# biirving/meant

Hardware: AMD Instinct MI355X
Metric: samples/sec fwd+bwd, MEANT lag=12 d=768 (higher is better)
Workload: dtype bf16; 1 GPU; full MEANT (tweet+image) fwd+CE+bwd, lag=12, d=768, 12 heads, seq=512, 224x224 p=16, E=1, vocab 64001 (BASELINE.json configs[2]/[3]); batch_per_gpu=128, global_batch=128, parallelism=dp1, micro_batches=1, train_mode_dropout=True, activation_checkpointing=False, norm_linear_fold=False, grad_allreduce=False

## Files before the change

### include/meant_hip.h

```cpp
#ifndef MEANT_HIP_H
#define MEANT_HIP_H

#include <stddef.h>
#include <stdint.h>

#ifdef __cplusplus
extern "C" {
#endif

enum meant_dtype { MEANT_F32 = 0, MEANT_BF16 = 1 };
enum meant_raw_dtype { MEANT_RAW_F32 = 0, MEANT_RAW_BF16 = 1, MEANT_RAW_F64 = 2, MEANT_RAW_U8 = 3 };

enum meant_status {
  MEANT_OK = 0,
  MEANT_ERR_ARG = -1,
  MEANT_ERR_UNSUPPORTED = -2,
  MEANT_ERR_LAUNCH = -3,
  MEANT_ERR_WORKSPACE = -4
};

enum meant_epilogue {
  MEANT_EPI_NONE = 0,
  MEANT_EPI_GELU = 1,
  MEANT_EPI_RESIDUAL = 2,
  MEANT_EPI_SIGMOID = 4
};

int meant_version(void);
const char* meant_last_error(void);
int meant_num_cus(void);

int meant_set_option(const char* name, int value);
int meant_get_option(const char* name, int* value);
int64_t meant_route_count(const char* route);
void meant_route_reset(void);
int64_t meant_debug_nt_steals(void);

int meant_rmsnorm_fwd(const void* x, const float* scale, void* y, float* rinv, int64_t rows, int64_t d,
                      float eps, float drop_p, uint64_t seed, int dtype, void* stream);
size_t meant_rmsnorm_bwd_ws(int64_t rows, int64_t d);
int meant_rmsnorm_bwd(const void* dy, const void* x, const float* scale, const float* rinv, void* dx,
                      float* dscale, int64_t rows, int64_t d, float eps, float drop_p, uint64_t seed,
                      const void* dres, const void* gelu_pre, int dtype, void* workspace, size_t workspace_bytes,
                      void* stream);

int meant_rmsnorm_partial_fwd(const void* x, const float* scale, const float* offset, void* y, float* rinv, int64_t rows,
                              int64_t d, int64_t d_part, float eps, int dtype, void* stream);
int meant_rmsnorm_partial_bwd(const void* dy, const void* x, const float* scale, const float* rinv, void* dx, float* dscale,
                              float* doffset, int64_t rows, int64_t d, int64_t d_part, float eps, int dtype, void* workspace,
                              size_t workspace_bytes, void* stream);

int meant_rmsnorm_pooled_ok(int64_t rows, int64_t d, int64_t group_rows);
int meant_rmsnorm_fwd_pooled(const void* x, const float* scale, void* y, float* rinv, float* pooled, int64_t rows,
                             int64_t d, int64_t group_rows, int pool_input, int gelu_input, float eps, float drop_p,
                             uint64_t seed, int dtype, void* stream);
int meant_rmsnorm_bwd_pooled(const void* dy, int dy_pooled, const void* x, const float* scale, const float* rinv,
                             void* dx, float* dscale, int64_t rows, int64_t d, int64_t group_rows, float eps,
                             float drop_p, uint64_t seed, const void* dres, int dres_pooled, const void* gelu_pre,
                             int dtype, void* workspace, size_t workspace_bytes, void* stream);

int meant_rmsnorm_stats(const void* x, float* rinv, int64_t rows, int64_t d, float eps, int dtype, void* stream);
int meant_rmsnorm_bwd_chain(const void* dy, int dy_pooled, const void* x, const float* scale, const float* rinv,
                            void* dx_scaled, float* dscale, int64_t rows, int64_t d, int64_t group_rows, float eps,
                            float drop_p, uint64_t seed, const void* gelu_pre, const float* up_rinv, const float* up_bias,
                            float up_eps, int64_t up_d, float* kcoef, float* dbias_up, int dtype, void* workspace, size_t workspace_bytes,
                            void* stream);
int meant_colscale(const float* w, const float* g, float* out, int64_t N, int64_t K, void* stream);
int meant_colscale_bwd(const float* dwp, const float* w, const float* g, float* dw, float* dg, int64_t N, int64_t K,
                       void* stream);

int meant_layernorm_fwd(const void* x, const float* gamma, const float* beta, void* y, float* stats,
                        int64_t rows, int64_t d, float eps, int dtype, void* stream);
int meant_layernorm_bwd(const void* dy, const void* x, const float* gamma, const float* stats, void* dx,
                        float* dgamma, float* dbeta, int64_t rows, int64_t d, int dtype, void* workspace,
                        size_t workspace_bytes, void* stream);

int meant_linear_fwd(const void* x, int64_t ldx, const void* w, const float* bias, const void* residual,
                     int64_t ldr, void* y, int64_t ldy, void* preact, int64_t M, int64_t N, int64_t K,
                     int epilogue, int dtype, void* stream);
int meant_qkv_proj_fwd(const void* x, int64_t ldx, const void* w, const float* bias, void* qkv, int64_t M,
                       int64_t K, int64_t S, int H, int Dh, int R, const float* qa, const float* qb,
                       const float* ka, const float* kb, int dtype, void* stream);
int meant_linear_fwd_rowscale(const void* x, int64_t ldx, const void* w, const float* bias, const float* row_scale,
                              const void* residual, int64_t ldr, void* y, int64_t ldy, void* preact, int64_t M, int64_t N,
                              int64_t K, int epilogue, int dtype, void* stream);
int meant_linear_bwd_dx_norm(const void* dy_scaled, int64_t lddy, const void* wT, const void* x, int64_t ldx,
                             const float* coef, const void* dres, int64_t lddres, const float* dres_pooled,
                             int64_t group_rows, void* dx, int64_t lddx, int64_t M, int64_t N, int64_t K, int dtype,
                             void* stream);
int meant_linear_bwd_dx(const void* dy, int64_t lddy, const void* wT, void* dx, int64_t lddx, int64_t M,
                        int64_t N, int64_t K, int dtype, void* stream);
size_t meant_linear_bwd_dw_ws(int64_t M, int64_t N, int64_t K, int dtype);
int meant_linear_bwd_dw(const void* dy, int64_t lddy, const void* x, int64_t ldx, float* dw, float* dbias,
                        int64_t M, int64_t N, int64_t K, int dtype, void* workspace, size_t workspace_bytes,
                        void* stream);

int meant_gemm_f32_strided(const float* A, const float* B, float* C, int64_t M, int64_t N, int64_t K,
                           int64_t nb1, int64_t nb2, const int64_t* sA ,
                           const int64_t* sB , const int64_t* sC , float alpha,
                           int accumulate, void* stream);

int meant_rotary_qk(void* qkv, int64_t T, int64_t S, int H, int Dh, int R, const float* qa, const float* qb,
                    const float* ka, const float* kb, int transpose, int dtype, void* stream);

size_t meant_attn_ws(int64_t G, int64_t S, int H, int Dh, int dtype);
size_t meant_attn_fwd_ws(int64_t G, int64_t S, int H, int Dh, int dtype);
int meant_attn_fwd(const void* qkv, void* o, float* lse, const float* key_mask, int64_t G, int64_t S, int H,
                   int Dh, float scale, int causal, int dtype, void* workspace, size_t workspace_bytes,
                   void* stream);
size_t meant_attn_drop_ws(int64_t G, int64_t S, int H, int Dh, int dtype);
int meant_attn_drop_fwd(const void* qkv, void* o, float* lse, const float* key_mask, int64_t G, int64_t S, int H, int Dh,
                        float scale, int causal, float drop_p, uint64_t seed, int dtype, void* workspace,
                        size_t workspace_bytes, void* stream);
int meant_attn_drop_bwd(const void* qkv, const void* o, const void* do_, const float* lse, const float* key_mask, void* dqkv,
                        int64_t G, int64_t S, int H, int Dh, float scale, int causal, float drop_p, uint64_t seed,
                        int dtype, void* workspace, size_t workspace_bytes, void* stream);
int meant_attn_bwd(const void* qkv, const void* o, const void* do_, const float* lse, const float* key_mask,
                   void* dqkv, int64_t G, int64_t S, int H, int Dh, float scale, int causal, const float* qa,
                   const float* qb, const float* ka, const float* kb, int R, int dtype, void* workspace,
                   size_t workspace_bytes, void* stream);

int meant_gather_rows(const void* src, const int32_t* idx, const void* fill, void* dst, int64_t n, int64_t W, int dtype,
                      void* stream);
int meant_gather_rows_rot(const void* src, const int32_t* idx, void* dst, int64_t n, int64_t S, int H, int Dh, int R,
                          const float* qa, const float* qb, const float* ka, const float* kb, int dtype, void* stream);
int meant_group_scatter(const void* ddst, const int32_t* index, void* dsrc, int64_t B, int64_t L, int64_t G, int64_t S,
                        int64_t W, int dtype, void* stream);
int meant_attn_cls_fwd(const void* qkv, void* out, int64_t ld_out, float* stats, const float* key_mask, int64_t B, int64_t L,
                       int H, int Dh, float scale, int dtype, void* stream);
int meant_attn_cls_bwd(const void* qkv, const void* out, int64_t ld_out, const void* dout, int64_t ld_dout,
                       const float* stats, const float* key_mask, void* dqkv, int64_t B, int64_t L, int H, int Dh,
                       float scale, int dtype, void* stream);

int meant_token_shift(const void* x, void* y, int64_t B, int64_t frames, int64_t n, int64_t d, int transpose, int dtype,
                      void* stream);
int meant_dropout(const void* x, void* y, int64_t n, float p, uint64_t seed, int dtype, void* stream);

int meant_temporal_attn_fwd(const void* q, const void* kv, void* o, float* p, int64_t B, int L, int H, int Dh,
                            float scale, int dtype, void* stream);
int meant_temporal_attn_bwd(const void* q, const void* kv, const float* p, const void* do_, void* dq, void* dkv,
                            int64_t B, int L, int H, int Dh, float scale, int dtype, void* stream);

int meant_patchify(const void* images, int images_dtype, void* patches, int64_t G, int C, int Hh, int Ww, int p,
                   int dtype, void* stream);

int meant_patchify_raw(const void* images, int raw_dtype, float mean, float inv_std, void* patches, int64_t G, int C,
                       int Hh, int Ww, int p, int dtype, void* stream);

int meant_meanpool_fwd(const void* x, void* out, int64_t ld_out, int64_t col_off, int64_t G, int64_t S, int64_t d,
                       int dtype, int out_dtype, void* stream);
int meant_meanpool_bwd(const void* dout, int64_t ld_out, int64_t col_off, void* dx, int64_t G, int64_t S, int64_t d,
                       int dtype, int out_dtype, void* stream);

int meant_add_rowvec(const void* x, const float* v, void* y, int64_t rows, int64_t d, int64_t period, int dtype,
                     void* stream);
int meant_add_rowvec_bwd(const void* dy, float* dv, int64_t rows, int64_t d, int64_t period, int dtype, void* stream);
int meant_gelu_bwd(const void* dy, const void* pre, void* dx, int64_t n, int dtype, void* stream);
int meant_sigmoid_bwd(const void* dy, const void* y, void* dx, int64_t n, int dtype, void* stream);
int meant_geglu_fwd(const void* h, void* y, int64_t rows, int64_t w, int dtype, void* stream);
int meant_geglu_bwd(const void* h, const void* dy, void* dh, int64_t rows, int64_t w, int dtype, void* stream);
int meant_add(const void* a, const void* b, void* y, int64_t n, int dtype, void* stream);
int meant_cast(const void* src, int dtype_src, void* dst, int dtype_dst, int64_t n, void* stream);
int meant_transpose2d(const void* src, int dtype_src, void* dst, int dtype_dst, int64_t rows, int64_t cols,
                      void* stream);
int meant_pad_copy2d(const void* src, int64_t ld_src, int64_t cols_src, int dtype_src, void* dst, int64_t ld_dst,
                     int64_t cols_dst, int dtype_dst, int64_t rows, void* stream);
int meant_embedding_fwd(const float* table, const int64_t* ids, void* out, int64_t n, int64_t d, int64_t V, int dtype,
                        void* stream);
int meant_embedding_bwd(const void* dout, const int64_t* ids, float* dtable, int64_t n, int64_t d, int64_t V, int dtype,
                        void* stream);
int meant_embedding_bwd_sorted(const void* dout, const int64_t* sorted_ids, const int64_t* order, float* dtable,
                               int64_t n, int64_t d, int64_t V, int dtype, void* stream);
int meant_embedding_bwd_sorted_range(const void* dout, const int64_t* sorted_ids, const int64_t* order, float* dtable,
                                     int64_t n, int64_t d, int64_t V, int64_t id_lo, int64_t id_hi, int dtype, void* stream);
size_t meant_sort_ids_ws(int64_t n, int64_t V);
int meant_sort_ids(const int64_t* ids, int64_t n, int64_t V, int64_t* sorted_ids, int64_t* order, void* workspace,
                   size_t workspace_bytes, void* stream);
size_t meant_embedding_bwd_seg_ws(int64_t n, int64_t d);
int meant_embedding_bwd_seg(const void* dout, const int64_t* sorted_ids, const int64_t* order, float* dtable, int64_t n,
                            int64_t d, int64_t V, int64_t id_lo, int64_t id_hi, int dtype, void* workspace,
                            size_t workspace_bytes, void* stream);

int meant_ce_probs(const float* probs, const int64_t* target, float* loss_accum, float* dprobs, int64_t B, int C,
                   void* stream);
int meant_softmax_ce_fwd(const void* logits, int64_t ld, const int64_t* target, int64_t T, int64_t V, int64_t ignore_index,
                         float* row_loss, float* lse, int dtype, void* stream);
int meant_softmax_ce_bwd(const void* logits, int64_t ld, const int64_t* target, const float* lse, int64_t T, int64_t V,
                         int64_t ignore_index, const float* gscale, void* dlogits, int dtype, void* stream);
size_t meant_select_rows_ws(int64_t T);
int meant_select_rows(const int64_t* target, int64_t T, int64_t V, int64_t ignore_index, int32_t* idx, int32_t* inv,
                      int64_t* target_sel, int32_t* count, void* workspace, size_t workspace_bytes, void* stream);
int meant_sumsq_f32(const float* x, int64_t n, float* out_accum, void* stream);
int meant_adamw_f32(float* p, const float* g, float* m, float* v, int64_t n, float lr, float beta1, float beta2,
                    float eps, float weight_decay, int64_t step, const float* sumsq, float max_norm,
                    float grad_scale, void* stream);

#ifdef __cplusplus
}
#endif
#endif
```

### meant_amd/_lib.py

```python
from __future__ import annotations

import ctypes as C
import os

import torch

_HERE = os.path.dirname(os.path.abspath(__file__))
LIB_PATH = os.environ.get("MEANT_LIB_PATH") or os.path.join(_HERE, "libmeant_hip.so")

F32, BF16 = 0, 1
RAW_F32, RAW_BF16, RAW_F64, RAW_U8 = 0, 1, 2, 3
EPI_NONE, EPI_GELU, EPI_RESIDUAL, EPI_SIGMOID = 0, 1, 2, 4

_p, _i, _i64, _f, _u64, _sz = C.c_void_p, C.c_int, C.c_int64, C.c_float, C.c_uint64, C.c_size_t

SIGNATURES = {
    "meant_version": (_i, []),
    "meant_last_error": (C.c_char_p, []),
    "meant_num_cus": (_i, []),
    "meant_rmsnorm_fwd": (_i, [_p, _p, _p, _p, _i64, _i64, _f, _f, _u64, _i, _p]),
    "meant_rmsnorm_bwd_ws": (_sz, [_i64, _i64]),
    "meant_rmsnorm_bwd": (_i, [_p, _p, _p, _p, _p, _p, _i64, _i64, _f, _f, _u64, _p, _p, _i, _p, _sz, _p]),
    "meant_rmsnorm_pooled_ok": (_i, [_i64, _i64, _i64]),
    "meant_rmsnorm_fwd_pooled": (_i, [_p, _p, _p, _p, _p, _i64, _i64, _i64, _i, _i, _f, _f, _u64, _i, _p]),
    "meant_rmsnorm_bwd_pooled": (_i, [_p, _i, _p, _p, _p, _p, _p, _i64, _i64, _i64, _f, _f, _u64, _p, _i, _p, _i, _p, _sz, _p]),
    "meant_layernorm_fwd": (_i, [_p, _p, _p, _p, _p, _i64, _i64, _f, _i, _p]),
    "meant_layernorm_bwd": (_i, [_p, _p, _p, _p, _p, _p, _p, _i64, _i64, _i, _p, _sz, _p]),
    "meant_linear_fwd": (_i, [_p, _i64, _p, _p, _p, _i64, _p, _i64, _p, _i64, _i64, _i64, _i, _i, _p]),
    "meant_linear_bwd_dx": (_i, [_p, _i64, _p, _p, _i64, _i64, _i64, _i64, _i, _p]),
    "meant_linear_bwd_dw_ws": (_sz, [_i64, _i64, _i64, _i]),
    "meant_linear_bwd_dw": (_i, [_p, _i64, _p, _i64, _p, _p, _i64, _i64, _i64, _i, _p, _sz, _p]),
    "meant_set_option": (_i, [C.c_char_p, _i]),
    "meant_get_option": (_i, [C.c_char_p, C.POINTER(_i)]),
    "meant_route_count": (_i64, [C.c_char_p]),
    "meant_route_reset": (None, []),
    "meant_debug_nt_steals": (_i64, []),
    "meant_gemm_f32_strided": (_i, [_p, _p, _p, _i64, _i64, _i64, _i64, _i64, _p, _p, _p, _f, _i, _p]),
    "meant_rotary_qk": (_i, [_p, _i64, _i64, _i, _i, _i, _p, _p, _p, _p, _i, _i, _p]),
    "meant_attn_ws": (_sz, [_i64, _i64, _i, _i, _i]),
    "meant_attn_fwd_ws": (_sz, [_i64, _i64, _i, _i, _i]),
    "meant_attn_drop_ws": (_sz, [_i64, _i64, _i, _i, _i]),
    "meant_attn_drop_fwd": (_i, [_p, _p, _p, _p, _i64, _i64, _i, _i, _f, _i, _f, _u64, _i, _p, _sz, _p]),
    "meant_attn_drop_bwd": (_i, [_p, _p, _p, _p, _p, _p, _i64, _i64, _i, _i, _f, _i, _f, _u64, _i, _p, _sz, _p]),
    "meant_attn_fwd": (_i, [_p, _p, _p, _p, _i64, _i64, _i, _i, _f, _i, _i, _p, _sz, _p]),
    "meant_attn_bwd": (_i, [_p, _p, _p, _p, _p, _p, _i64, _i64, _i, _i, _f, _i, _p, _p, _p, _p, _i, _i, _p, _sz, _p]),
    "meant_qkv_proj_fwd": (_i, [_p, _i64, _p, _p, _p, _i64, _i64, _i64, _i, _i, _i, _p, _p, _p, _p, _i, _p]),
    "meant_gather_rows": (_i, [_p, _p, _p, _p, _i64, _i64, _i, _p]),
    "meant_gather_rows_rot": (_i, [_p, _p, _p, _i64, _i64, _i, _i, _i, _p, _p, _p, _p, _i, _p]),
    "meant_group_scatter": (_i, [_p, _p, _p, _i64, _i64, _i64, _i64, _i64, _i, _p]),
    "meant_attn_cls_fwd": (_i, [_p, _p, _i64, _p, _p, _i64, _i64, _i, _i, _f, _i, _p]),
    "meant_attn_cls_bwd": (_i, [_p, _p, _i64, _p, _i64, _p, _p, _p, _i64, _i64, _i, _i, _f, _i, _p]),
    "meant_token_shift": (_i, [_p, _p, _i64, _i64, _i64, _i64, _i, _i, _p]),
    "meant_dropout": (_i, [_p, _p, _i64, _f, _u64, _i, _p]),
    "meant_temporal_attn_fwd": (_i, [_p, _p, _p, _p, _i64, _i, _i, _i, _f, _i, _p]),
    "meant_temporal_attn_bwd": (_i, [_p, _p, _p, _p, _p, _p, _i64, _i, _i, _i, _f, _i, _p]),
    "meant_patchify": (_i, [_p, _i, _p, _i64, _i, _i, _i, _i, _i, _p]),
    "meant_patchify_raw": (_i, [_p, _i, _f, _f, _p, _i64, _i, _i, _i, _i, _i, _p]),
    "meant_meanpool_fwd": (_i, [_p, _p, _i64, _i64, _i64, _i64, _i64, _i, _i, _p]),
    "meant_meanpool_bwd": (_i, [_p, _i64, _i64, _p, _i64, _i64, _i64, _i, _i, _p]),
    "meant_add_rowvec": (_i, [_p, _p, _p, _i64, _i64, _i64, _i, _p]),
    "meant_add_rowvec_bwd": (_i, [_p, _p, _i64, _i64, _i64, _i, _p]),
    "meant_gelu_bwd": (_i, [_p, _p, _p, _i64, _i, _p]),
    "meant_sigmoid_bwd": (_i, [_p, _p, _p, _i64, _i, _p]),
    "meant_geglu_fwd": (_i, [_p, _p, _i64, _i64, _i, _p]),
    "meant_geglu_bwd": (_i, [_p, _p, _p, _i64, _i64, _i, _p]),
    "meant_add": (_i, [_p, _p, _p, _i64, _i, _p]),
    "meant_cast": (_i, [_p, _i, _p, _i, _i64, _p]),
    "meant_transpose2d": (_i, [_p, _i, _p, _i, _i64, _i64, _p]),
    "meant_pad_copy2d": (_i, [_p, _i64, _i64, _i, _p, _i64, _i64, _i, _i64, _p]),
    "meant_embedding_fwd": (_i, [_p, _p, _p, _i64, _i64, _i64, _i, _p]),
    "meant_embedding_bwd": (_i, [_p, _p, _p, _i64, _i64, _i64, _i, _p]),
    "meant_ce_probs": (_i, [_p, _p, _p, _p, _i64, _i, _p]),
    "meant_softmax_ce_fwd": (_i, [_p, _i64, _p, _i64, _i64, _i64, _p, _p, _i, _p]),
    "meant_softmax_ce_bwd": (_i, [_p, _i64, _p, _p, _i64, _i64, _i64, _p, _p, _i, _p]),
    "meant_select_rows_ws": (_sz, [_i64]),
    "meant_select_rows": (_i, [_p, _i64, _i64, _i64, _p, _p, _p, _p, _p, _sz, _p]),
    "meant_sumsq_f32": (_i, [_p, _i64, _p, _p]),
    "meant_adamw_f32": (_i, [_p, _p, _p, _p, _i64, _f, _f, _f, _f, _f, _i64, _p, _f, _f, _p]),
    "meant_embedding_bwd_sorted": (_i, [_p, _p, _p, _p, _i64, _i64, _i64, _i, _p]),
    "meant_embedding_bwd_sorted_range": (_i, [_p, _p, _p, _p, _i64, _i64, _i64, _i64, _i64, _i, _p]),
    "meant_sort_ids_ws": (_sz, [_i64, _i64]),
    "meant_sort_ids": (_i, [_p, _i64, _i64, _p, _p, _p, _sz, _p]),
    "meant_embedding_bwd_seg_ws": (_sz, [_i64, _i64]),
    "meant_embedding_bwd_seg": (_i, [_p, _p, _p, _p, _i64, _i64, _i64, _i64, _i64, _i, _p, _sz, _p]),
    "meant_rmsnorm_partial_fwd": (_i, [_p, _p, _p, _p, _p, _i64, _i64, _i64, _f, _i, _p]),
    "meant_rmsnorm_partial_bwd": (_i, [_p, _p, _p, _p, _p, _p, _p, _i64, _i64, _i64, _f, _i, _p, _sz, _p]),
    "meant_rmsnorm_stats": (_i, [_p, _p, _i64, _i64, _f, _i, _p]),
    "meant_rmsnorm_bwd_chain": (_i, [_p, _i, _p, _p, _p, _p, _p, _i64, _i64, _i64, _f, _f, _u64, _p, _p, _p, _f, _i64, _p, _p, _i, _p, _sz, _p]),
    "meant_colscale": (_i, [_p, _p, _p, _i64, _i64, _p]),
    "meant_colscale_bwd": (_i, [_p, _p, _p, _p, _p, _i64, _i64, _p]),
    "meant_linear_fwd_rowscale": (_i, [_p, _i64, _p, _p, _p, _p, _i64, _p, _i64, _p, _i64, _i64, _i64, _i, _i, _p]),
    "meant_linear_bwd_dx_norm": (_i, [_p, _i64, _p, _p, _i64, _p, _p, _i64, _p, _i64, _p, _i64, _i64, _i64, _i64, _i, _p]),
}


class MeantLibraryMissing(ImportError):
    pass


def _load():
    if not os.path.exists(LIB_PATH):
        raise MeantLibraryMissing(
            f"{LIB_PATH} not found: build it with `python -c 'import __graft_entry__ as g; g.build()'` "
            f"(or `make -C meant_amd/csrc`).  meant_amd has no CPU / eager fallback.")
    lib = C.CDLL(LIB_PATH)
    for name, (res, args) in SIGNATURES.items():
        fn = getattr(lib, name)
        fn.restype = res
        fn.argtypes = args
    return lib


lib = _load()


def set_option(name: str, value: int) -> None:
    check(lib.meant_set_option(name.encode(), int(value)), "set_option")


def get_option(name: str) -> int:
    v = _i(0)
    check(lib.meant_get_option(name.encode(), C.byref(v)), "get_option")
    return v.value


def route_count(route: str) -> int:
    n = lib.meant_route_count(route.encode())
    if n < 0:
        raise KeyError(route)
    return n


def route_reset() -> None:
    lib.meant_route_reset()


class MeantHipError(RuntimeError):
    pass


def check(rc: int, what: str = "") -> None:
    if rc != 0:
        msg = lib.meant_last_error().decode("utf-8", "replace")
        raise MeantHipError(f"{what or 'libmeant_hip'} failed (status {rc}): {msg}")
```

### meant_amd/csrc/common.h

```cpp
#pragma once
#include <hip/hip_runtime.h>
#include <stdint.h>
#include <stdio.h>
#include <math.h>
#include "../../include/meant_hip.h"

typedef __bf16 bf16;
typedef __attribute__((ext_vector_type(2))) float f32x2;
typedef __attribute__((ext_vector_type(4))) float f32x4;
typedef __attribute__((ext_vector_type(16))) float f32x16;
typedef __attribute__((ext_vector_type(4))) __bf16 bf16x4;
typedef __attribute__((ext_vector_type(8))) __bf16 bf16x8;
typedef __attribute__((ext_vector_type(4))) unsigned int u32x4;
typedef __attribute__((ext_vector_type(2))) unsigned int u32x2;

#define WAVE 64

void meant_set_error(const char* fmt, ...);

#define MEANT_REQUIRE(cond, code, ...)      \
  do {                                      \
    if (!(cond)) {                          \
      meant_set_error(__VA_ARGS__);         \
      return (code);                        \
    }                                       \
  } while (0)

#define MEANT_LAUNCH_CHECK(name)                                                     \
  do {                                                                               \
    hipError_t e__ = hipGetLastError();                                              \
    if (e__ != hipSuccess) {                                                         \
      meant_set_error("%s: launch failed: %s", name, hipGetErrorString(e__));        \
      return MEANT_ERR_LAUNCH;                                                       \
    }                                                                                \
  } while (0)

#define MEANT_MAX_DEVICES 64
int meant_current_device(void);
int meant_raise_dyn_lds(const void* kernel, int bytes);
#define MEANT_RAISE_LDS(kernel, bytes)                                        \
  do {                                                                        \
    int rc__ = meant_raise_dyn_lds((const void*)(kernel), (int)(bytes));      \
    if (rc__) return rc__;                                                    \
  } while (0)

enum meant_option_id {
  MEANT_OPT_NT_STREAM = 0, MEANT_OPT_NT_DYNAMIC, MEANT_OPT_DETERMINISTIC, MEANT_OPT_NT_GRID_CAP, MEANT_OPT_ATTN_SHORT, MEANT_OPT_NT_RAGGED, MEANT_OPT_ATTN_BWD1, MEANT_OPT_TEMPORAL_LONG, MEANT_OPT_COUNT
};
int meant_opt(int id);

enum meant_route_id {
  ROUTE_NT128 = 0, ROUTE_NT256, ROUTE_NT256S, ROUTE_NT256S_ROT, ROUTE_NT_SPLIT, ROUTE_TN128, ROUTE_TN256, ROUTE_TN256_DET, ROUTE_TN_TAIL,
  ROUTE_GEMM_F32, ROUTE_ATTN_FWD, ROUTE_ATTN_FWD_D128, ROUTE_ATTN_FWD_D96, ROUTE_ATTN_BWD,
  ROUTE_ATTN_BWD_D128, ROUTE_ATTN_BWD_D96, ROUTE_ATTN_GENERIC, ROUTE_ATTN_CLS, ROUTE_ATTN_SHORT, ROUTE_NT_OVERLAP, ROUTE_ATTN_BWD1,
  ROUTE_ATTN_FWD_D160, ROUTE_ATTN_FWD_D192, ROUTE_ATTN_FWD_D256, ROUTE_ATTN_BWD_D160, ROUTE_ATTN_BWD_D192, ROUTE_ATTN_BWD_D256, ROUTE_TEMPORAL_LONG,
  ROUTE_EMB_SEG, ROUTE_SORT_IDS, ROUTE_NT128K, ROUTE_NT256K, ROUTE_SELECT_ROWS, ROUTE_ROTARY_QK, ROUTE_ROTARY_PAIRS, ROUTE_NT_ROT,
  MEANT_ROUTE_COUNT
};
void meant_route_hit(int route);

static inline bool meant_aligned16(const void* p) { return (reinterpret_cast<uintptr_t>(p) & 15) == 0; }
static inline int64_t ceil_div(int64_t a, int64_t b) { return (a + b - 1) / b; }

template <typename T> struct Vec8;
template <> struct Vec8<float> {
  f32x4 lo, hi;
  __device__ __forceinline__ float get(int i) const { return i < 4 ? lo[i] : hi[i - 4]; }
  __device__ __forceinline__ void set(int i, float v) { if (i < 4) lo[i] = v; else hi[i - 4] = v; }
};
template <> struct Vec8<bf16> {
  bf16x8 v;
  __device__ __forceinline__ float get(int i) const { return (float)v[i]; }
  __device__ __forceinline__ void set(int i, float x) { v[i] = (bf16)x; }
  __device__ __forceinline__ unsigned raw(int i) const {
    typedef __attribute__((ext_vector_type(4))) unsigned uvec4;
    return (__builtin_bit_cast(uvec4, v)[i >> 1] >> ((i & 1) * 16)) & 0xffffu;
  }
};

__device__ __forceinline__ void rotary_pair(float t0, float t1, float a0, float a1, float b0, float b1, float& o0, float& o1) {
  o0 = __builtin_fmaf(t0, a0, -(t1 * b0));
  o1 = __builtin_fmaf(t1, a1, t0 * b1);
}

template <typename T> __device__ __forceinline__ Vec8<T> load8(const T* p);
template <> __device__ __forceinline__ Vec8<float> load8<float>(const float* p) {
  Vec8<float> r; r.lo = *reinterpret_cast<const f32x4*>(p); r.hi = *reinterpret_cast<const f32x4*>(p + 4); return r;
}
template <> __device__ __forceinline__ Vec8<bf16> load8<bf16>(const bf16* p) {
  Vec8<bf16> r; r.v = *reinterpret_cast<const bf16x8*>(p); return r;
}
template <typename T> __device__ __forceinline__ Vec8<T> load8s(const T* p);
template <> __device__ __forceinline__ Vec8<float> load8s<float>(const float* p) {
  Vec8<float> r;
  r.lo = __builtin_nontemporal_load(reinterpret_cast<const f32x4*>(p));
  r.hi = __builtin_nontemporal_load(reinterpret_cast<const f32x4*>(p + 4));
  return r;
}
template <> __device__ __forceinline__ Vec8<bf16> load8s<bf16>(const bf16* p) {
  Vec8<bf16> r; r.v = __builtin_nontemporal_load(reinterpret_cast<const bf16x8*>(p)); return r;
}
template <typename T> __device__ __forceinline__ void store8s(T* p, const Vec8<T>& v);
template <> __device__ __forceinline__ void store8s<float>(float* p, const Vec8<float>& v) {
  __builtin_nontemporal_store(v.lo, reinterpret_cast<f32x4*>(p)); __builtin_nontemporal_store(v.hi, reinterpret_cast<f32x4*>(p + 4));
}
template <> __device__ __forceinline__ void store8s<bf16>(bf16* p, const Vec8<bf16>& v) {
  __builtin_nontemporal_store(v.v, reinterpret_cast<bf16x8*>(p));
}
template <typename T> __device__ __forceinline__ void store8(T* p, const Vec8<T>& v);
template <> __device__ __forceinline__ void store8<float>(float* p, const Vec8<float>& v) {
  *reinterpret_cast<f32x4*>(p) = v.lo; *reinterpret_cast<f32x4*>(p + 4) = v.hi;
}
template <> __device__ __forceinline__ void store8<bf16>(bf16* p, const Vec8<bf16>& v) {
  *reinterpret_cast<bf16x8*>(p) = v.v;
}

__device__ __forceinline__ float to_f(float x) { return x; }
__device__ __forceinline__ float to_f(bf16 x) { return (float)x; }
template <typename T> __device__ __forceinline__ T from_f(float x);
template <> __device__ __forceinline__ float from_f<float>(float x) { return x; }
template <> __device__ __forceinline__ bf16 from_f<bf16>(float x) { return (bf16)x; }

__device__ __forceinline__ float wave_sum(float v) {
#pragma unroll
  for (int o = 32; o > 0; o >>= 1) v += __shfl_xor(v, o, 64);
  return v;
}
__device__ __forceinline__ float wave_max(float v) {
#pragma unroll
  for (int o = 32; o > 0; o >>= 1) v = fmaxf(v, __shfl_xor(v, o, 64));
  return v;
}

#define MEANT_DPP_ADD(v, CTRL) ((v) + __builtin_bit_cast(float, __builtin_amdgcn_update_dpp(0, __builtin_bit_cast(int, (v)), (CTRL), 0xf, 0xf, true)))
__device__ __forceinline__ float wave_sum_dpp(float v) {
  v = MEANT_DPP_ADD(v, 0xB1);
  v = MEANT_DPP_ADD(v, 0x4E);
  v = MEANT_DPP_ADD(v, 0x141);
  v = MEANT_DPP_ADD(v, 0x140);
  const int b = __builtin_bit_cast(int, v);
  const float r0 = __builtin_bit_cast(float, __builtin_amdgcn_readlane(b, 0)), r1 = __builtin_bit_cast(float, __builtin_amdgcn_readlane(b, 16));
  const float r2 = __builtin_bit_cast(float, __builtin_amdgcn_readlane(b, 32)), r3 = __builtin_bit_cast(float, __builtin_amdgcn_readlane(b, 48));
  return (r0 + r1) + (r2 + r3);
}
__device__ __forceinline__ float rms_rinv(float sumsq, float inv_sqrt_d, float eps) {
  return 1.0f / (sqrtf(sumsq) * inv_sqrt_d + eps);
}

__device__ __forceinline__ float gelu_erf(float x) { return 0.5f * x * (1.0f + erff(x * 0.70710678118654752f)); }
__device__ __forceinline__ float gelu_erf_fast(float x) {
  const float z = fabsf(x) * 0.70710678118654752f;
  const float t = __builtin_amdgcn_rcpf(fmaf(0.3275911f, z, 1.0f));
  float p = fmaf(1.061405429f, t, -1.453152027f);
  p = fmaf(p, t, 1.421413741f);
  p = fmaf(p, t, -0.284496736f);
  p = fmaf(p, t, 0.254829592f);
  const float half_erfc = 0.5f * p * t * __builtin_amdgcn_exp2f(-1.4426950408889634f * z * z);
  const float phi = x < 0.f ? half_erfc : 1.0f - half_erfc;
  return x * phi;
}
__device__ __forceinline__ float gelu_phi_fast(float x) {
  const float z = fabsf(x) * 0.70710678118654752f;
  const float t = __builtin_amdgcn_rcpf(fmaf(0.3275911f, z, 1.0f));
  float p = fmaf(1.061405429f, t, -1.453152027f);
  p = fmaf(p, t, 1.421413741f);
  p = fmaf(p, t, -0.284496736f);
  p = fmaf(p, t, 0.254829592f);
  const float half_erfc = 0.5f * p * t * __builtin_amdgcn_exp2f(-1.4426950408889634f * z * z);
  return x < 0.f ? half_erfc : 1.0f - half_erfc;
}
constexpr unsigned PHI_LO = 0x3A80u, PHI_HI = 0x40FFu, PHI_N = PHI_HI - PHI_LO + 1;
__device__ __forceinline__ unsigned phi_slot(unsigned bits) {
  unsigned m = bits & 0x7FFFu;
  m = m < PHI_LO ? PHI_LO : m;
  m = m > PHI_HI ? PHI_HI : m;
  return (m - PHI_LO) + ((bits >> 15) & 1u) * PHI_N;
}
__device__ __forceinline__ float gelu_erf_grad(float x) {
  const float cdf = 0.5f * (1.0f + erff(x * 0.70710678118654752f));
  const float pdf = 0.39894228040143268f * __expf(-0.5f * x * x);
  return cdf + x * pdf;
}

__device__ __forceinline__ float gelu_erf_grad_fast(float x) {
  const float z = fabsf(x) * 0.70710678118654752f;
  const float t = __builtin_amdgcn_rcpf(fmaf(0.3275911f, z, 1.0f));
  float p = fmaf(1.061405429f, t, -1.453152027f);
  p = fmaf(p, t, 1.421413741f);
  p = fmaf(p, t, -0.284496736f);
  p = fmaf(p, t, 0.254829592f);
  const float e = __builtin_amdgcn_exp2f(-0.72134752044448170f * x * x);
  const float half_erfc = 0.5f * p * t * e;
  const float phi = x < 0.f ? half_erfc : 1.0f - half_erfc;
  return fmaf(x * 0.39894228040143268f, e, phi);
}

__device__ __forceinline__ float hash_uniform(uint64_t seed, uint64_t idx) {
  uint64_t z = seed + idx * 0x9E3779B97F4A7C15ull;
  z = (z ^ (z >> 30)) * 0xBF58476D1CE4E5B9ull;
  z = (z ^ (z >> 27)) * 0x94D049BB133111EBull;
  z = z ^ (z >> 31);
  return (float)(z >> 40) * (1.0f / 16777216.0f);
}
#ifndef DROP_HASH32
#define DROP_HASH32 1
#endif
__device__ __forceinline__ uint32_t mix32(uint32_t h) {
  h ^= h >> 16; h *= 0x85EBCA6Bu; h ^= h >> 13; h *= 0xC2B2AE35u; h ^= h >> 16;
  return h;
}
__device__ __forceinline__ uint32_t draw32(uint64_t seed, uint64_t blk, uint32_t j) {
  const uint32_t hi = (uint32_t)(blk >> 32);
  const uint32_t k = (uint32_t)blk ^ ((hi << 17) | (hi >> 15));
  const uint32_t s = ((uint32_t)seed + 0x9E3779B9u * (j + 1)) ^ ((uint32_t)(seed >> 32) * 0x7FEB352Du);
  return mix32(k ^ s);
}
__device__ __forceinline__ void keep_scale8(float p, uint64_t seed, uint64_t base, float (&m)[8]) {
  const unsigned thr = (unsigned)(p * 65536.0f);
  const float sc = 65536.0f / (float)(65536u - thr);
  if ((thr & 0xffu) == 0) {
    const unsigned thr8 = thr >> 8;
#if DROP_HASH32
#pragma unroll
    for (int h = 0; h < 2; ++h) {
      const uint32_t z = draw32(seed, base >> 3, (uint32_t)h);
#pragma unroll
      for (int q = 0; q < 4; ++q) m[4 * h + q] = ((z >> (8 * q)) & 0xffu) >= thr8 ? sc : 0.0f;
    }
#else
    uint64_t z = seed + ((base >> 3) | (1ull << 62)) * 0x9E3779B97F4A7C15ull;
    z = (z ^ (z >> 30)) * 0xBF58476D1CE4E5B9ull;
    z = (z ^ (z >> 27)) * 0x94D049BB133111EBull;
    z = z ^ (z >> 31);
#pragma unroll
    for (int q = 0; q < 8; ++q) m[q] = ((unsigned)(z >> (8 * q)) & 0xffu) >= thr8 ? sc : 0.0f;
#endif
    return;
  }
#if DROP_HASH32
#pragma unroll
  for (int h = 0; h < 4; ++h) {
    const uint32_t z = draw32(seed, base >> 3, 2u + (uint32_t)h);
#pragma unroll
    for (int q = 0; q < 2; ++q) m[2 * h + q] = ((z >> (16 * q)) & 0xffffu) >= thr ? sc : 0.0f;
  }
#else
#pragma unroll
  for (int h = 0; h < 2; ++h) {
    uint64_t z = seed + ((base >> 2) + h) * 0x9E3779B97F4A7C15ull;
    z = (z ^ (z >> 30)) * 0xBF58476D1CE4E5B9ull;
    z = (z ^ (z >> 27)) * 0x94D049BB133111EBull;
    z = z ^ (z >> 31);
#pragma unroll
    for (int q = 0; q < 4; ++q) m[4 * h + q] = ((unsigned)(z >> (16 * q)) & 0xffffu) >= thr ? sc : 0.0f;
  }
#endif
}

__device__ __forceinline__ unsigned lds_addr(const void* p) {
  return (unsigned)(unsigned long long)(const __attribute__((address_space(3))) char*)p;
}
template <int OFF>
__device__ __forceinline__ u32x2 lds_read_tr16(unsigned addr) {
  u32x2 r;
  asm volatile("ds_read_b64_tr_b16 %0, %1 offset:%2" : "=v"(r) : "v"(addr), "n"(OFF));
  return r;
}
__device__ __forceinline__ void lds_wait_all() {
  asm volatile("s_waitcnt lgkmcnt(0)" ::: "memory");
  __builtin_amdgcn_sched_barrier(0);
}
template <int N>
__device__ __forceinline__ void lds_wait_upto() {
  asm volatile("s_waitcnt lgkmcnt(%0)" ::"n"(N) : "memory");
  __builtin_amdgcn_sched_barrier(0);
}
__device__ __forceinline__ bf16x8 pack_tr(u32x2 lo, u32x2 hi) {
  u32x4 v = {lo[0], lo[1], hi[0], hi[1]};
  return __builtin_bit_cast(bf16x8, v);
}

#define DISPATCH_DTYPE(dtype, T, ...)                                           \
  do {                                                                          \
    if ((dtype) == MEANT_F32) { using T = float; __VA_ARGS__; }                 \
    else if ((dtype) == MEANT_BF16) { using T = bf16; __VA_ARGS__; }            \
    else { meant_set_error("unknown dtype %d", (int)(dtype)); return MEANT_ERR_ARG; } \
  } while (0)
```

### meant_amd/csrc/core.hip

```cpp
#include "common.h"
#include <stdarg.h>
#include <string.h>
#include <stdlib.h>
#include <atomic>
#include <mutex>
#include <unordered_map>

static thread_local char g_err[512] = "";

void meant_set_error(const char* fmt, ...) {
  va_list ap;
  va_start(ap, fmt);
  vsnprintf(g_err, sizeof(g_err), fmt, ap);
  va_end(ap);
}

extern "C" const char* meant_last_error(void) { return g_err; }

extern "C" int meant_version(void) { return 200;  }

namespace {
struct DeviceState {
  int cus = -1;
  std::unordered_map<const void*, int> lds_raised;
};
std::mutex g_dev_mu;
DeviceState g_dev[MEANT_MAX_DEVICES];
}

int meant_current_device(void) {
  int dev = 0;
  if (hipGetDevice(&dev) != hipSuccess || dev < 0 || dev >= MEANT_MAX_DEVICES) return -1;
  return dev;
}

extern "C" int meant_num_cus(void) {
  const int dev = meant_current_device();
  if (dev < 0) return 0;
  std::lock_guard<std::mutex> lock(g_dev_mu);
  DeviceState& st = g_dev[dev];
  if (st.cus < 0) {
    hipDeviceProp_t p;
    st.cus = hipGetDeviceProperties(&p, dev) == hipSuccess ? p.multiProcessorCount : 0;
  }
  return st.cus;
}

int meant_raise_dyn_lds(const void* kernel, int bytes) {
  const int dev = meant_current_device();
  MEANT_REQUIRE(dev >= 0, MEANT_ERR_LAUNCH, "no current HIP device (or device index >= %d)", MEANT_MAX_DEVICES);
  std::lock_guard<std::mutex> lock(g_dev_mu);
  DeviceState& st = g_dev[dev];
  const auto it = st.lds_raised.find(kernel);
  if (it != st.lds_raised.end() && it->second >= bytes) return MEANT_OK;
  const hipError_t e = hipFuncSetAttribute(kernel, hipFuncAttributeMaxDynamicSharedMemorySize, bytes);
  MEANT_REQUIRE(e == hipSuccess, MEANT_ERR_LAUNCH, "hipFuncSetAttribute(%d bytes of LDS) failed on device %d: %s", bytes, dev,
                hipGetErrorString(e));
  st.lds_raised[kernel] = bytes;
  return MEANT_OK;
}

namespace {
struct OptionDef { const char* name; const char* env; int dflt; };
const OptionDef k_options[MEANT_OPT_COUNT] = {
    {"nt_stream", "MEANT_NT_STREAM", 1},
    {"nt_dynamic", "MEANT_NT_DYNAMIC", 1},
    {"deterministic", "MEANT_DETERMINISTIC", 0},
    {"nt_grid_cap", "MEANT_NT_GRID_CAP", 0},
    {"attn_short", "MEANT_ATTN_SHORT", 1},
    {"nt_ragged", "MEANT_NT_RAGGED", 1},
    {"attn_bwd1", "MEANT_ATTN_BWD1", 1},
    {"temporal_long", "MEANT_TEMPORAL_LONG", 0},
};
bool is_nt_pp(const char* name) { return name && !strcmp(name, "nt_pp"); }
std::atomic<int> g_opt[MEANT_OPT_COUNT];
std::once_flag g_opt_once;
void options_init() {
  std::call_once(g_opt_once, [] {
    for (int i = 0; i < MEANT_OPT_COUNT; ++i) {
      const char* v = getenv(k_options[i].env);
      g_opt[i].store(v && *v ? atoi(v) : k_options[i].dflt, std::memory_order_relaxed);
    }
  });
}
int option_index(const char* name) {
  if (!name) return -1;
  for (int i = 0; i < MEANT_OPT_COUNT; ++i)
    if (!strcmp(name, k_options[i].name)) return i;
  return -1;
}
}

int meant_opt(int id) {
  options_init();
  return g_opt[id].load(std::memory_order_relaxed);
}

extern "C" int meant_set_option(const char* name, int value) {
  options_init();
  if (is_nt_pp(name)) {
    MEANT_REQUIRE(value == 1, MEANT_ERR_UNSUPPORTED, "meant_set_option: nt_pp is always 1 (the lock-step kernel was removed)");
    return MEANT_OK;
  }
  const int i = option_index(name);
  MEANT_REQUIRE(i >= 0, MEANT_ERR_ARG, "meant_set_option: unknown option '%s'", name ? name : "(null)");
  g_opt[i].store(value, std::memory_order_relaxed);
  return MEANT_OK;
}

extern "C" int meant_get_option(const char* name, int* value) {
  options_init();
  if (is_nt_pp(name) && value) { *value = 1; return MEANT_OK; }
  const int i = option_index(name);
  MEANT_REQUIRE(i >= 0 && value, MEANT_ERR_ARG, "meant_get_option: unknown option '%s'", name ? name : "(null)");
  *value = g_opt[i].load(std::memory_order_relaxed);
  return MEANT_OK;
}

namespace {
const char* const k_routes[MEANT_ROUTE_COUNT] = {
    "nt128", "nt256", "nt256s", "nt256s_rot", "nt_split", "tn128", "tn256", "tn256_det", "tn_tail", "gemm_f32",
    "attn_fwd", "attn_fwd_d128", "attn_fwd_d96", "attn_bwd", "attn_bwd_d128", "attn_bwd_d96",
    "attn_generic", "attn_cls", "attn_short", "nt_overlap", "attn_bwd1",
    "attn_fwd_d160", "attn_fwd_d192", "attn_fwd_d256", "attn_bwd_d160", "attn_bwd_d192", "attn_bwd_d256",
    "temporal_long", "emb_seg", "sort_ids", "nt128k", "nt256k", "select_rows",
    "rotary_qk", "rotary_pairs",
    "nt_rot",
};
std::atomic<long long> g_route[MEANT_ROUTE_COUNT];
}

void meant_route_hit(int route) { g_route[route].fetch_add(1, std::memory_order_relaxed); }

extern "C" int64_t meant_route_count(const char* route) {
  if (!route) return -1;
  for (int i = 0; i < MEANT_ROUTE_COUNT; ++i)
    if (!strcmp(route, k_routes[i])) return (int64_t)g_route[i].load(std::memory_order_relaxed);
  return -1;
}

extern "C" void meant_route_reset(void) {
  for (int i = 0; i < MEANT_ROUTE_COUNT; ++i) g_route[i].store(0, std::memory_order_relaxed);
}
```

### meant_amd/csrc/embedding.hip

```cpp
#include "common.h"

#define EMB_REQ(c, ...) MEANT_REQUIRE(c, MEANT_ERR_ARG, __VA_ARGS__)

namespace {

constexpr int SORT_TILE = 2048, SORT_WAVE_SPAN = 512, SORT_ROUNDS = 8;

__device__ __forceinline__ uint32_t sort_key(int64_t id, int64_t V) {
  return (uint32_t)(id < 0 ? 0 : (id >= V ? V - 1 : id));
}

__global__ __launch_bounds__(256) void sort_hist_kernel(const int64_t* __restrict__ ids, int64_t n, int64_t V, int passes,
                                                         uint32_t* __restrict__ ghist, uint32_t* __restrict__ tile_hist, int64_t ntiles) {
  __shared__ uint32_t h[4][256];
  const int tid = threadIdx.x;
#pragma unroll
  for (int p = 0; p < 4; ++p) h[p][tid] = 0;
  __syncthreads();
  const int64_t base = (int64_t)blockIdx.x * SORT_TILE;
  for (int i = 0; i < SORT_TILE / 256; ++i) {
    const int64_t j = base + i * 256 + tid;
    if (j < n) {
      const uint32_t key = sort_key(ids[j], V);
      for (int p = 0; p < passes; ++p) atomicAdd(&h[p][(key >> (8 * p)) & 255u], 1u);
    }
  }
  __syncthreads();
  tile_hist[(int64_t)tid * ntiles + blockIdx.x] = h[0][tid];
  for (int p = 0; p < passes; ++p)
    if (h[p][tid]) atomicAdd(&ghist[p * 256 + tid], h[p][tid]);
}

__global__ __launch_bounds__(256) void sort_count_kernel(const uint32_t* __restrict__ keys, int64_t n, int shift,
                                                          uint32_t* __restrict__ tile_hist, int64_t ntiles) {
  __shared__ uint32_t h[256];
  const int tid = threadIdx.x;
  h[tid] = 0;
  __syncthreads();
  const int64_t base = (int64_t)blockIdx.x * SORT_TILE;
  for (int i = 0; i < SORT_TILE / 256; ++i) {
    const int64_t j = base + i * 256 + tid;
    if (j < n) atomicAdd(&h[(keys[j] >> shift) & 255u], 1u);
  }
  __syncthreads();
  tile_hist[(int64_t)tid * ntiles + blockIdx.x] = h[tid];
}

__device__ __forceinline__ uint32_t block_scan_incl(uint32_t x, uint32_t* wsum, uint32_t* total) {
  const int lane = threadIdx.x & 63, wave = threadIdx.x >> 6;
#pragma unroll
  for (int o = 1; o < 64; o <<= 1) {
    const uint32_t y = __shfl_up(x, o, 64);
    if (lane >= o) x += y;
  }
  __syncthreads();
  if (lane == 63) wsum[wave] = x;
  __syncthreads();
  uint32_t pre = 0, tot = 0;
#pragma unroll
  for (int w = 0; w < 4; ++w) {
    const uint32_t s = wsum[w];
    if (w < wave) pre += s;
    tot += s;
  }
  *total = tot;
  return x + pre;
}

__global__ __launch_bounds__(256) void sort_scan_kernel(const uint32_t* __restrict__ ghist, uint32_t* __restrict__ tile_hist, int64_t ntiles) {
  __shared__ uint32_t wsum[4];
  const int tid = threadIdx.x, digit = blockIdx.x;
  uint32_t carry;
  block_scan_incl(tid < digit ? ghist[tid] : 0u, wsum, &carry);
  uint32_t* row = tile_hist + (int64_t)digit * ntiles;
  for (int64_t t0 = 0; t0 < ntiles; t0 += 256) {
    const int64_t t = t0 + tid;
    const uint32_t x = t < ntiles ? row[t] : 0u;
    uint32_t total;
    const uint32_t incl = block_scan_incl(x, wsum, &total);
    if (t < ntiles) row[t] = carry + incl - x;
    carry += total;
  }
}

template <bool FIRST, bool LAST>
__global__ __launch_bounds__(256) void sort_scatter_kernel(const int64_t* __restrict__ ids, const uint32_t* __restrict__ kin,
                                                            const uint32_t* __restrict__ vin, int64_t n, int64_t V, int shift,
                                                            const uint32_t* __restrict__ tile_off, int64_t ntiles,
                                                            uint32_t* __restrict__ kout, uint32_t* __restrict__ vout,
                                                            int64_t* __restrict__ sorted_ids, int64_t* __restrict__ order) {
  __shared__ uint32_t cnt[4][256];
  const int tid = threadIdx.x, lane = tid & 63, wave = tid >> 6;
#pragma unroll
  for (int w = 0; w < 4; ++w) cnt[w][tid] = 0;
  __syncthreads();
  const int64_t base = (int64_t)blockIdx.x * SORT_TILE + wave * SORT_WAVE_SPAN;
  uint32_t key[SORT_ROUNDS], val[SORT_ROUNDS], rk[SORT_ROUNDS];
#pragma unroll
  for (int r = 0; r < SORT_ROUNDS; ++r) {
    const int64_t j = base + r * 64 + lane;
    const bool valid = j < n;
    key[r] = valid ? (FIRST ? sort_key(ids[j], V) : kin[j]) : 0u;
    val[r] = valid ? (FIRST ? (uint32_t)j : vin[j]) : 0u;
    const uint32_t dig = (key[r] >> shift) & 255u;
    unsigned long long m = __ballot(valid);
#pragma unroll
    for (int b = 0; b < 8; ++b) {
      const bool bit = (dig >> b) & 1u;
      const unsigned long long bal = __ballot(valid && bit);
      m &= bit ? bal : ~bal;
    }
    const unsigned long long below = m & ((1ull << lane) - 1ull);
    rk[r] = valid ? cnt[wave][dig] + (uint32_t)__popcll(below) : 0u;
    __syncthreads();
    if (valid && below == 0) cnt[wave][dig] += (uint32_t)__popcll(m);
    __syncthreads();
  }
  {
    uint32_t o = tile_off[(int64_t)tid * ntiles + blockIdx.x];
#pragma unroll
    for (int w = 0; w < 4; ++w) {
      const uint32_t c = cnt[w][tid];
      cnt[w][tid] = o;
      o += c;
    }
  }
  __syncthreads();
#pragma unroll
  for (int r = 0; r < SORT_ROUNDS; ++r) {
    const int64_t j = base + r * 64 + lane;
    if (j >= n) continue;
    const int64_t pos = (int64_t)cnt[wave][(key[r] >> shift) & 255u] + rk[r];
    if (pos >= n) continue;
    if (LAST) {
      sorted_ids[pos] = (int64_t)key[r];
      order[pos] = (int64_t)val[r];
    } else {
      kout[pos] = key[r];
      vout[pos] = val[r];
    }
  }
}

int sort_passes(int64_t V) {
  int bits = 0;
  for (uint64_t m = (uint64_t)(V - 1); m; m >>= 1) ++bits;
  const int p = (bits + 7) / 8;
  return p < 1 ? 1 : p;
}
size_t align256(size_t x) { return (x + 255) & ~(size_t)255; }
struct SortWs { size_t ghist, tile_hist, buf[2], total; int nbuf; };
SortWs sort_ws_layout(int64_t n, int64_t V) {
  SortWs w;
  const int64_t ntiles = ceil_div(n, SORT_TILE);
  const int passes = sort_passes(V);
  w.nbuf = passes - 1 < 2 ? passes - 1 : 2;
  size_t off = 0;
  w.ghist = off; off += align256(4 * 256 * sizeof(uint32_t));
  w.tile_hist = off; off += align256((size_t)ntiles * 256 * sizeof(uint32_t));
  for (int i = 0; i < 2; ++i) {
    w.buf[i] = off;
    if (i < w.nbuf) off += 2 * align256((size_t)n * sizeof(uint32_t));
  }
  w.total = off;
  return w;
}

constexpr int SEG = 256;
template <typename T>
__global__ __launch_bounds__(256) void emb_seg_kernel(const T* __restrict__ dout, const int64_t* __restrict__ sorted_ids,
                                                       const int64_t* __restrict__ order, float* __restrict__ dtable,
                                                       float* __restrict__ part, int64_t n, int64_t d, int64_t V, int64_t id_lo,
                                                       int64_t id_hi, int cb_chunks) {
  const int lane = threadIdx.x & 63, wave = threadIdx.x >> 6;
  const int64_t s = (int64_t)blockIdx.x * 4 + wave;
  const int64_t j0 = s * SEG;
  if (j0 >= n) return;
  const int64_t j1 = j0 + SEG < n ? j0 + SEG : n;
  if (sorted_ids[j1 - 1] < id_lo || sorted_ids[j0] >= id_hi) return;
  const int c0 = blockIdx.y * cb_chunks;
  const int left = (int)(d >> 3) - c0;
  const int nch = left < cb_chunks ? left : cb_chunks;
  const bool has0 = lane < nch, has1 = lane + 64 < nch;
  const int64_t col0 = (int64_t)(c0 + lane) * 8, col1 = (int64_t)(c0 + lane + 64) * 8;
  float acc0[8], acc1[8];
#pragma unroll
  for (int e = 0; e < 8; ++e) acc0[e] = acc1[e] = 0.f;
  int64_t cur = sorted_ids[j0];
  bool open_left = j0 > 0 && sorted_ids[j0 - 1] == cur;

  auto flush = [&](int64_t id, int slot) {
    if (id < 0 || id >= V || id < id_lo || id >= id_hi) return;
    if (slot >= 0) {
      float* row = part + (s * 2 + slot) * d;
      Vec8<float> v;
      if (has0) {
#pragma unroll
        for (int e = 0; e < 8; ++e) v.set(e, acc0[e]);
        store8<float>(row + col0, v);
      }
      if (has1) {
#pragma unroll
        for (int e = 0; e < 8; ++e) v.set(e, acc1[e]);
        store8<float>(row + col1, v);
      }
      return;
    }
    float* row = dtable + id * d;
    if (has0) {
      Vec8<float> v = load8<float>(row + col0);
#pragma unroll
      for (int e = 0; e < 8; ++e) v.set(e, v.get(e) + acc0[e]);
      store8<float>(row + col0, v);
    }
    if (has1) {
      Vec8<float> v = load8<float>(row + col1);
#pragma unroll
      for (int e = 0; e < 8; ++e) v.set(e, v.get(e) + acc1[e]);
      store8<float>(row + col1, v);
    }
  };

  for (int64_t jb = j0; jb < j1; jb += 64) {
    const int64_t jl = jb + lane < j1 ? jb + lane : j1 - 1;
    const long long my_id = sorted_ids[jl], my_ord = order[jl];
    const int cnt = (int)(j1 - jb < 64 ? j1 - jb : 64);
    for (int t0 = 0; t0 < cnt; t0 += 4) {
      Vec8<T> r0[4], r1[4];
      long long ids4[4];
#pragma unroll
      for (int u = 0; u < 4; ++u) {
        const int t = t0 + u < cnt ? t0 + u : cnt - 1;
        ids4[u] = __shfl(my_id, t, 64);
        const long long ord = __shfl(my_ord, t, 64);
        const bool row_ok = ord >= 0 && ord < n;
        const T* src = dout + (row_ok ? ord : 0) * d;
        r0[u] = Vec8<T>{};
        r1[u] = Vec8<T>{};
        if (has0 && row_ok) r0[u] = load8s<T>(src + col0);
        if (has1 && row_ok) r1[u] = load8s<T>(src + col1);
      }
#pragma unroll
      for (int u = 0; u < 4; ++u) {
        if (t0 + u >= cnt) break;
        const int64_t id = ids4[u];
        if (id != cur) {
          flush(cur, open_left ? 0 : -1);
#pragma unroll
          for (int e = 0; e < 8; ++e) acc0[e] = acc1[e] = 0.f;
          cur = id;
          open_left = false;
        }
#pragma unroll
        for (int e = 0; e < 8; ++e) {
          if (has0) acc0[e] += r0[u].get(e);
          if (has1) acc1[e] += r1[u].get(e);
        }
      }
    }
  }
  const bool open_right = j1 < n && sorted_ids[j1] == cur;
  flush(cur, open_left ? 0 : (open_right ? 1 : -1));
}

constexpr int SEG_SHORT = 16;
__global__ __launch_bounds__(256) void emb_seg_cross_kernel(const int64_t* __restrict__ sorted_ids, const float* __restrict__ part,
                                                             int* __restrict__ longk, float* __restrict__ dtable, int64_t n, int64_t d,
                                                             int64_t V, int64_t id_lo, int64_t id_hi) {
  const int lane = threadIdx.x & 63, wave = threadIdx.x >> 6;
  const int64_t s = (int64_t)blockIdx.x * 4 + wave, j0 = s * SEG, j1 = j0 + SEG;
  if (j1 >= n) return;
  const int64_t id = sorted_ids[j1 - 1];
  const bool owner = sorted_ids[j1] == id && !(j0 > 0 && sorted_ids[j0 - 1] == id)
                     && id >= 0 && id < V && id >= id_lo && id < id_hi;
  int64_t K = 0;
  if (owner) {
    const int64_t nst = (n + SEG - 1) / SEG;
    int64_t follow = 0;
    for (int64_t t0 = s + 1;; t0 += 64) {
      const int64_t t = t0 + lane;
      const int k = __popcll(__ballot(t < nst && sorted_ids[t * SEG] == id));
      follow += k;
      if (k < 64) break;
    }
    K = follow + 1;
  }
  if (blockIdx.y == 0 && lane == 0) longk[s] = K > SEG_SHORT ? (int)K : 0;
  if (K == 0 || K > SEG_SHORT) return;
  const int64_t col = (int64_t)blockIdx.y * 256 + lane * 4;
  if (col >= d) return;
  f32x4 acc = *reinterpret_cast<const f32x4*>(part + (s * 2 + 1) * d + col);
  for (int64_t k = 1; k < K; ++k) acc += *reinterpret_cast<const f32x4*>(part + (s + k) * 2 * d + col);
  f32x4* dst = reinterpret_cast<f32x4*>(dtable + id * d + col);
  *dst = *dst + acc;
}

__global__ __launch_bounds__(256) void emb_seg_long_kernel(const int64_t* __restrict__ sorted_ids, const float* __restrict__ part,
                                                            const int* __restrict__ longk, float* __restrict__ dtable, int64_t d) {
  __shared__ f32x4 red[16][16];
  const int tid = threadIdx.x;
  const int64_t s = blockIdx.x;
  const int64_t K = longk[s];
  if (K == 0) return;
  const int64_t id = sorted_ids[s * SEG + SEG - 1];
  const int p = tid >> 4;
  const int64_t col = (int64_t)blockIdx.y * 64 + (tid & 15) * 4;
  const bool active = col < d;
  const int64_t piece = (K + 15) / 16, k0 = p * piece, k1 = k0 + piece < K ? k0 + piece : K;
  f32x4 acc = {0.f, 0.f, 0.f, 0.f};
  if (active) {
#pragma unroll 4
    for (int64_t k = k0; k < k1; ++k) {
      const float* row = k == 0 ? part + (s * 2 + 1) * d : part + (s + k) * 2 * d;
      acc += *reinterpret_cast<const f32x4*>(row + col);
    }
  }
  red[p][tid & 15] = acc;
  __syncthreads();
#pragma unroll
  for (int h = 8; h > 0; h >>= 1) {
    if (p < h) red[p][tid & 15] += red[p + h][tid & 15];
    __syncthreads();
  }
  if (p == 0 && active) {
    f32x4* dst = reinterpret_cast<f32x4*>(dtable + id * d + col);
    *dst = *dst + red[0][tid & 15];
  }
}

size_t seg_part_bytes(int64_t n, int64_t d) { return (size_t)ceil_div(n, SEG) * 2 * (size_t)d * sizeof(float); }

template <typename T>
__global__ __launch_bounds__(256) void embedding_fwd_kernel(const float* __restrict__ table, const int64_t* __restrict__ ids,
                                                             T* __restrict__ out, int64_t n, int d, int64_t V) {
  const int lane = threadIdx.x & 63, wave = threadIdx.x >> 6;
  const int nch = d >> 3;
  for (int64_t r = (int64_t)blockIdx.x * 4 + wave; r < n; r += (int64_t)gridDim.x * 4) {
    int64_t id = ids[r];
    id = id < 0 ? 0 : (id >= V ? V - 1 : id);
    const float* src = table + id * d;
    for (int ch = lane; ch < nch; ch += 64) {
      const Vec8<float> v = load8<float>(src + ch * 8);
      Vec8<T> o;
#pragma unroll
      for (int k = 0; k < 8; ++k) o.set(k, v.get(k));
      store8s<T>(out + r * d + ch * 8, o);
    }
  }
}
template <typename T>
__global__ __launch_bounds__(256) void embedding_bwd_kernel(const T* __restrict__ dout, const int64_t* __restrict__ ids,
                                                             float* __restrict__ dtable, int64_t n, int d, int64_t V) {
  const int lane = threadIdx.x & 63, wave = threadIdx.x >> 6;
  for (int64_t r = (int64_t)blockIdx.x * 4 + wave; r < n; r += (int64_t)gridDim.x * 4) {
    int64_t id = ids[r];
    id = id < 0 ? 0 : (id >= V ? V - 1 : id);
    float* dst = dtable + id * d;
    for (int e = lane; e < d; e += 64) atomicAdd(dst + e, to_f(dout[r * d + e]));
  }
}

constexpr int EMB_SEG = 256;
template <typename T>
__global__ __launch_bounds__(256) void embedding_bwd_sorted_kernel(const T* __restrict__ dout, const int64_t* __restrict__ sorted_ids,
                                                                    const int64_t* __restrict__ order, float* __restrict__ dtable,
                                                                    int64_t n, int d, int64_t V, int det, int64_t id_lo, int64_t id_hi) {
  const int lane = threadIdx.x & 63, wave = threadIdx.x >> 6;
  int64_t j0 = ((int64_t)blockIdx.x * 4 + wave) * EMB_SEG;
  if (j0 >= n) return;
  int64_t j1 = j0 + EMB_SEG < n ? j0 + EMB_SEG : n;
  if (sorted_ids[j1 - 1] < id_lo || sorted_ids[j0] >= id_hi) return;
  if (det) {
    if (j0 > 0) {
      const int64_t prev = sorted_ids[j0 - 1];
      while (j0 < j1 && sorted_ids[j0] == prev) ++j0;
      if (j0 == j1) return;
    }
    const int64_t last = sorted_ids[j1 - 1];
    while (j1 < n && sorted_ids[j1] == last) ++j1;
  }
  const int nch = d >> 3;
  const bool has1 = lane + 64 < nch, has0 = lane < nch;
  float acc0[8], acc1[8];
#pragma unroll
  for (int e = 0; e < 8; ++e) acc0[e] = acc1[e] = 0.f;
  int64_t cur = sorted_ids[j0];
  bool shared = !det && j0 > 0 && sorted_ids[j0 - 1] == cur;

  auto flush = [&](int64_t id, bool atomic) {
    if (id < 0 || id >= V || id < id_lo || id >= id_hi) return;
    float* row = dtable + id * d;
    if (atomic) {
#pragma unroll
      for (int e = 0; e < 8; ++e) {
        if (has0) atomicAdd(row + lane * 8 + e, acc0[e]);
        if (has1) atomicAdd(row + (lane + 64) * 8 + e, acc1[e]);
      }
    } else {
      if (has0) {
        Vec8<float> v = load8<float>(row + lane * 8);
#pragma unroll
        for (int e = 0; e < 8; ++e) v.set(e, v.get(e) + acc0[e]);
        store8<float>(row + lane * 8, v);
      }
      if (has1) {
        Vec8<float> v = load8<float>(row + (lane + 64) * 8);
#pragma unroll
        for (int e = 0; e < 8; ++e) v.set(e, v.get(e) + acc1[e]);
        store8<float>(row + (lane + 64) * 8, v);
      }
    }
  };

  for (int64_t jb = j0; jb < j1; jb += 64) {
    const int64_t jl = jb + lane < j1 ? jb + lane : j1 - 1;
    const long long my_id = sorted_ids[jl], my_ord = order[jl];
    const int cnt = (int)(j1 - jb < 64 ? j1 - jb : 64);
    for (int t0 = 0; t0 < cnt; t0 += 4) {
      Vec8<T> r0[4], r1[4];
      long long ids4[4];
#pragma unroll
      for (int u = 0; u < 4; ++u) {
        const int t = t0 + u < cnt ? t0 + u : cnt - 1;
        ids4[u] = __shfl(my_id, t, 64);
        const long long ord = __shfl(my_ord, t, 64);
        const T* src = dout + ord * d;
        if (has0) r0[u] = load8s<T>(src + lane * 8);
        if (has1) r1[u] = load8s<T>(src + (lane + 64) * 8);
      }
#pragma unroll
      for (int u = 0; u < 4; ++u) {
        if (t0 + u >= cnt) break;
        const int64_t id = ids4[u];
        if (id != cur) {
          flush(cur, shared);
#pragma unroll
          for (int e = 0; e < 8; ++e) acc0[e] = acc1[e] = 0.f;
          cur = id;
          shared = false;
        }
#pragma unroll
        for (int e = 0; e < 8; ++e) {
          if (has0) acc0[e] += r0[u].get(e);
          if (has1) acc1[e] += r1[u].get(e);
        }
      }
    }
  }
  flush(cur, !det && (shared || (j1 < n && sorted_ids[j1] == cur)));
}

}

extern "C" size_t meant_sort_ids_ws(int64_t n, int64_t V) {
  if (n <= 0 || V <= 0 || n >= (1ll << 31) || V >= (1ll << 31)) return 0;
  return sort_ws_layout(n, V).total;
}

extern "C" int meant_sort_ids(const int64_t* ids, int64_t n, int64_t V, int64_t* sorted_ids, int64_t* order, void* workspace,
                              size_t workspace_bytes, void* stream) {
  EMB_REQ(ids && sorted_ids && order && n > 0 && V > 0, "sort_ids: bad argument");
  MEANT_REQUIRE(n < (1ll << 31) && V < (1ll << 31), MEANT_ERR_UNSUPPORTED, "sort_ids: n=%lld and V=%lld must be below 2^31", (long long)n,
                (long long)V);
  {
    const char *a = (const char*)ids, *o1 = (const char*)sorted_ids, *o2 = (const char*)order;
    const size_t len = (size_t)n * sizeof(int64_t);
    const auto overlap = [len](const char* x, const char* y) { return x < y + len && y < x + len; };
    EMB_REQ(!overlap(a, o1) && !overlap(a, o2) && !overlap(o1, o2), "sort_ids: ids, sorted_ids and order must not overlap");
  }
  const SortWs w = sort_ws_layout(n, V);
  MEANT_REQUIRE(workspace && workspace_bytes >= w.total, MEANT_ERR_WORKSPACE, "sort_ids: workspace of %zu bytes needed, %zu given", w.total, workspace_bytes);
  EMB_REQ((reinterpret_cast<uintptr_t>(workspace) & 3) == 0, "sort_ids: 4-byte workspace alignment");
  hipStream_t st = (hipStream_t)stream;
  char* base = (char*)workspace;
  uint32_t* ghist = (uint32_t*)(base + w.ghist);
  uint32_t* tile_hist = (uint32_t*)(base + w.tile_hist);
  uint32_t* bk[2] = {nullptr, nullptr};
  uint32_t* bv[2] = {nullptr, nullptr};
  for (int i = 0; i < w.nbuf; ++i) {
    bk[i] = (uint32_t*)(base + w.buf[i]);
    bv[i] = (uint32_t*)(base + w.buf[i] + align256((size_t)n * sizeof(uint32_t)));
  }
  const int64_t ntiles = ceil_div(n, SORT_TILE);
  const int passes = sort_passes(V);
  const dim3 grid((unsigned)ntiles), block(256);
  const hipError_t e = hipMemsetAsync(ghist, 0, 4 * 256 * sizeof(uint32_t), st);
  MEANT_REQUIRE(e == hipSuccess, MEANT_ERR_LAUNCH, "sort_ids: clearing the digit counters failed: %s", hipGetErrorString(e));
  hipLaunchKernelGGL(sort_hist_kernel, grid, block, 0, st, ids, n, V, passes, ghist, tile_hist, ntiles);
  for (int p = 0; p < passes; ++p) {
    const bool first = p == 0, last = p == passes - 1;
    const uint32_t* kin = first ? nullptr : bk[(p - 1) & 1];
    const uint32_t* vin = first ? nullptr : bv[(p - 1) & 1];
    uint32_t* kout = last ? nullptr : bk[p & 1];
    uint32_t* vout = last ? nullptr : bv[p & 1];
    const int shift = 8 * p;
    if (!first) hipLaunchKernelGGL(sort_count_kernel, grid, block, 0, st, kin, n, shift, tile_hist, ntiles);
    hipLaunchKernelGGL(sort_scan_kernel, dim3(256), block, 0, st, (const uint32_t*)(ghist + p * 256), tile_hist, ntiles);
#define SORT_SCATTER(F, L)                                                                                                     \
  hipLaunchKernelGGL((sort_scatter_kernel<F, L>), grid, block, 0, st, ids, kin, vin, n, V, shift, (const uint32_t*)tile_hist, \
                     ntiles, kout, vout, sorted_ids, order)
    if (first && last) SORT_SCATTER(true, true);
    else if (first) SORT_SCATTER(true, false);
    else if (last) SORT_SCATTER(false, true);
    else SORT_SCATTER(false, false);
#undef SORT_SCATTER
  }
  MEANT_LAUNCH_CHECK("sort_ids");
  meant_route_hit(ROUTE_SORT_IDS);
  return MEANT_OK;
}

extern "C" size_t meant_embedding_bwd_seg_ws(int64_t n, int64_t d) {
  if (n <= 0 || d <= 0) return 0;
  return seg_part_bytes(n, d) + align256((size_t)ceil_div(n, SEG) * sizeof(int));
}

extern "C" int meant_embedding_bwd_seg(const void* dout, const int64_t* sorted_ids, const int64_t* order, float* dtable, int64_t n,
                                       int64_t d, int64_t V, int64_t id_lo, int64_t id_hi, int dtype, void* workspace,
                                       size_t workspace_bytes, void* stream) {
  EMB_REQ(dout && sorted_ids && order && dtable && n > 0 && d > 0 && V > 0 && 0 <= id_lo && id_lo <= id_hi && id_hi <= V,
          "embedding_bwd_seg: bad argument");
  MEANT_REQUIRE(d % 8 == 0, MEANT_ERR_UNSUPPORTED, "embedding_bwd_seg: d=%lld must be a multiple of 8", (long long)d);
  MEANT_REQUIRE(d < (1ll << 22), MEANT_ERR_UNSUPPORTED, "embedding_bwd_seg: d=%lld is beyond the launch grid (d < 2^22)", (long long)d);
  const size_t need = meant_embedding_bwd_seg_ws(n, d);
  MEANT_REQUIRE(workspace && workspace_bytes >= need, MEANT_ERR_WORKSPACE, "embedding_bwd_seg: workspace of %zu bytes needed, %zu given", need, workspace_bytes);
  EMB_REQ(meant_aligned16(dout) && meant_aligned16(dtable) && meant_aligned16(workspace), "embedding_bwd_seg: 16-byte alignment");
  if (id_lo == id_hi) return MEANT_OK;
  const int64_t nst = ceil_div(n, SEG);
  const int chunks = (int)(d >> 3);
  const int ncb = (int)ceil_div(chunks, 128);
  const int cb_chunks = (int)ceil_div(chunks, ncb);
  hipStream_t st = (hipStream_t)stream;
  DISPATCH_DTYPE(dtype, T,
                 hipLaunchKernelGGL(emb_seg_kernel<T>, dim3((unsigned)ceil_div(nst, 4), (unsigned)ncb), dim3(256), 0, st, (const T*)dout,
                                    sorted_ids, order, dtable, (float*)workspace, n, d, V, id_lo, id_hi, cb_chunks));
  if (nst > 1) {
    int* longk = (int*)((char*)workspace + seg_part_bytes(n, d));
    hipLaunchKernelGGL(emb_seg_cross_kernel, dim3((unsigned)ceil_div(nst - 1, 4), (unsigned)ceil_div(d, 256)), dim3(256), 0, st, sorted_ids,
                       (const float*)workspace, longk, dtable, n, d, V, id_lo, id_hi);
    hipLaunchKernelGGL(emb_seg_long_kernel, dim3((unsigned)(nst - 1), (unsigned)ceil_div(d, 64)), dim3(256), 0, st, sorted_ids,
                       (const float*)workspace, (const int*)longk, dtable, d);
  }
  MEANT_LAUNCH_CHECK("embedding_bwd_seg");
  meant_route_hit(ROUTE_EMB_SEG);
  return MEANT_OK;
}

extern "C" int meant_embedding_fwd(const float* table, const int64_t* ids, void* out, int64_t n, int64_t d, int64_t V, int dtype, void* stream) {
  EMB_REQ(table && ids && out && n > 0 && d > 0 && d % 8 == 0 && V > 0, "embedding_fwd: bad argument");
  int64_t nb = ceil_div(n, 4); if (nb > 8192) nb = 8192;
  DISPATCH_DTYPE(dtype, T,
                 hipLaunchKernelGGL(embedding_fwd_kernel<T>, dim3((unsigned)nb), dim3(256), 0, (hipStream_t)stream, table, ids, (T*)out, n, (int)d, V));
  MEANT_LAUNCH_CHECK("embedding_fwd");
  return MEANT_OK;
}
extern "C" int meant_embedding_bwd_sorted(const void* dout, const int64_t* sorted_ids, const int64_t* order, float* dtable, int64_t n,
                                          int64_t d, int64_t V, int dtype, void* stream) {
  EMB_REQ(dout && sorted_ids && order && dtable && n > 0 && d > 0 && V > 0, "embedding_bwd_sorted: bad argument");
  MEANT_REQUIRE(d <= 1024 && d % 8 == 0, MEANT_ERR_UNSUPPORTED, "embedding_bwd_sorted: d=%lld must be a multiple of 8 and <= 1024", (long long)d);
  EMB_REQ(meant_aligned16(dout) && meant_aligned16(dtable), "embedding_bwd_sorted: 16-byte alignment");
  const int64_t nb = ceil_div(n, 4 * EMB_SEG);
  DISPATCH_DTYPE(dtype, T,
                 hipLaunchKernelGGL(embedding_bwd_sorted_kernel<T>, dim3((unsigned)nb), dim3(256), 0, (hipStream_t)stream, (const T*)dout,
                                    sorted_ids, order, dtable, n, (int)d, V, meant_opt(MEANT_OPT_DETERMINISTIC) != 0, (int64_t)0, V));
  MEANT_LAUNCH_CHECK("embedding_bwd_sorted");
  return MEANT_OK;
}

extern "C" int meant_embedding_bwd_sorted_range(const void* dout, const int64_t* sorted_ids, const int64_t* order, float* dtable, int64_t n,
                                                int64_t d, int64_t V, int64_t id_lo, int64_t id_hi, int dtype, void* stream) {
  EMB_REQ(dout && sorted_ids && order && dtable && n > 0 && d > 0 && V > 0 && 0 <= id_lo && id_lo <= id_hi && id_hi <= V,
         "embedding_bwd_sorted_range: bad argument");
  MEANT_REQUIRE(d <= 1024 && d % 8 == 0, MEANT_ERR_UNSUPPORTED, "embedding_bwd_sorted_range: d=%lld must be a multiple of 8 and <= 1024", (long long)d);
  EMB_REQ(meant_aligned16(dout) && meant_aligned16(dtable), "embedding_bwd_sorted_range: 16-byte alignment");
  if (id_lo == id_hi) return MEANT_OK;
  const int64_t nb = ceil_div(n, 4 * EMB_SEG);
  DISPATCH_DTYPE(dtype, T,
                 hipLaunchKernelGGL(embedding_bwd_sorted_kernel<T>, dim3((unsigned)nb), dim3(256), 0, (hipStream_t)stream, (const T*)dout,
                                    sorted_ids, order, dtable, n, (int)d, V, meant_opt(MEANT_OPT_DETERMINISTIC) != 0, id_lo, id_hi));
  MEANT_LAUNCH_CHECK("embedding_bwd_sorted_range");
  return MEANT_OK;
}

extern "C" int meant_embedding_bwd(const void* dout, const int64_t* ids, float* dtable, int64_t n, int64_t d, int64_t V, int dtype, void* stream) {
  EMB_REQ(dout && ids && dtable && n > 0 && d > 0 && V > 0, "embedding_bwd: bad argument");
  int64_t nb = ceil_div(n, 4); if (nb > 8192) nb = 8192;
  DISPATCH_DTYPE(dtype, T,
                 hipLaunchKernelGGL(embedding_bwd_kernel<T>, dim3((unsigned)nb), dim3(256), 0, (hipStream_t)stream, (const T*)dout, ids, dtable, n, (int)d, V));
  MEANT_LAUNCH_CHECK("embedding_bwd");
  return MEANT_OK;
}
```

### meant_amd/csrc/internal.h

```cpp
#pragma once
#include "common.h"

struct GemmF32Args {
  const void* A; const void* B; void* C;
  int in_dtype = MEANT_F32;
  int out_dtype = MEANT_F32;
  int64_t M, N, K, nb1, nb2;
  int64_t sA[4];
  int64_t sB[4];
  int64_t sC[4];
  float alpha;
  int accumulate;
  const float* bias;
  const void* residual;
  void* preact;
  int epilogue;
  int ksplit = 0;
};
int gemm_f32_launch(const GemmF32Args& a, hipStream_t stream);

struct GemmBf16Args {
  const bf16* A; int64_t lda;
  const bf16* B; int64_t ldb;
  bf16* C; int64_t ldc;
  int64_t M, N, K;
  const float* bias;
  const bf16* residual; int64_t ldr;
  bf16* preact;
  int epilogue;
  const float* rot_qa; const float* rot_qb; const float* rot_ka; const float* rot_kb;
  int rot_S, rot_D, rot_Dh, rot_R;
  const float* row_scale = nullptr;
  const bf16* sub = nullptr; int64_t ldsub = 0;
  const float* sub_coef = nullptr;
  const float* bres = nullptr;
  int bres_rows = 1; float bres_scale = 1.f;
};
int gemm_bf16_nt_launch(const GemmBf16Args& a, hipStream_t stream);
int gemm_bf16_tn_launch(const bf16* dY, int64_t lddy, const bf16* X, int64_t ldx, float* dW, float* dbias,
                        int64_t M, int64_t N, int64_t K, void* ws, size_t ws_bytes, hipStream_t stream);
size_t gemm_bf16_tn_ws(int64_t M, int64_t N, int64_t K);

int colsum_launch(const void* x, int64_t ldx, float* out, int64_t M, int64_t N, int dtype, int accumulate, hipStream_t stream);

int attn_f32_fwd(const float* qkv, float* o, float* lse, const float* key_mask, int64_t G, int64_t S, int H, int Dh,
                 float scale, int causal, void* ws, size_t ws_bytes, hipStream_t stream, float drop_p = 0.f, uint64_t seed = 0);
int attn_f32_bwd(const float* qkv, const float* o, const float* dout, const float* lse, const float* key_mask, float* dqkv,
                 int64_t G, int64_t S, int H, int Dh, float scale, int causal, void* ws, size_t ws_bytes, hipStream_t stream, float drop_p = 0.f,
                 uint64_t seed = 0);
size_t attn_drop_ws(int64_t G, int64_t S, int H, int Dh, int dtype);
int attn_drop_bf16(bool backward, const bf16* qkv, const bf16* o, const bf16* dout, bf16* o_out, float* lse, const float* key_mask, bf16* dqkv,
                   int64_t G, int64_t S, int H, int Dh, float scale, int causal, float drop_p, uint64_t seed, void* ws, size_t ws_bytes,
                   hipStream_t stream);
size_t attn_f32_ws(int64_t G, int64_t S, int H, int Dh);
int attn_bf16_fwd(const bf16* qkv, bf16* o, float* lse, const float* key_mask, int64_t G, int64_t S, int H, int Dh,
                  float scale, int causal, void* ws, size_t ws_bytes, hipStream_t stream);
struct RotTables { const float* qa; const float* qb; const float* ka; const float* kb; int R; };
int attn_bf16_bwd(const bf16* qkv, const bf16* o, const bf16* dout, const float* lse, const float* key_mask, bf16* dqkv,
                  int64_t G, int64_t S, int H, int Dh, float scale, int causal, RotTables rot, void* ws, size_t ws_bytes,
                  hipStream_t stream);
size_t attn_bf16_ws(int64_t G, int64_t S, int H, int Dh);
size_t attn_bf16_fwd_ws(int64_t G, int64_t S, int H, int Dh);
bool attn_short_ok(int64_t S, int Dh);
int attn_short_fwd(const bf16* qkv, bf16* o, float* lse, const float* key_mask, int64_t G, int64_t S, int H, int Dh, float scale,
                   int causal, hipStream_t stream);
int attn_short_bwd(const bf16* qkv, const bf16* dout, const float* lse, const float* key_mask, bf16* dqkv, int64_t G, int64_t S, int H,
                   int Dh, float scale, int causal, RotTables rot, hipStream_t stream);
bool attn_bwd1_ok(int64_t S, int Dh, int causal);
size_t attn_bwd1_ws(int64_t G, int64_t S, int H, int Dh);
int attn_bwd1_launch(const bf16* qkv, const bf16* o, const bf16* dout, const float* lse, const float* bias2, const int* flags,
                     const uint64_t* masks, bf16* dqkv, void* ws1, int64_t G, int64_t S, int H, float scale, int causal, RotTables rot,
                     hipStream_t stream);
```

### meant_amd/csrc/norm.hip

```cpp
#include <type_traits>
#include "internal.h"

namespace {

constexpr int MAXC = 4;
constexpr int NORM_THREADS = 256;
constexpr int NORM_MAX_BLOCKS = 1024;
constexpr int NORM_PACKED_BLOCKS = 2048;

template <typename T> __device__ __forceinline__ float gelu_grad_t(float x);
template <> __device__ __forceinline__ float gelu_grad_t<float>(float x) { return gelu_erf_grad(x); }
template <> __device__ __forceinline__ float gelu_grad_t<bf16>(float x) { return gelu_erf_grad_fast(x); }

__device__ const float g_phi_tab[2 * PHI_N] = {
#include "phi_table.inc"
};
template <typename T> constexpr bool PHI_TABLE = sizeof(T) == 2;
__device__ __forceinline__ void phi_tab_to_lds(float* dst) {
  for (int j = threadIdx.x; j < (int)(2 * PHI_N); j += NORM_THREADS) dst[j] = g_phi_tab[j];
  __syncthreads();
}


template <typename T>
// ... 872 lines not shown
        if (col < d) {
          wide_load<T, V>(xr + col, v[c]);
#pragma unroll
          for (int i = 0; i < V; ++i) sm += v[c][i];
        }
      }
    }
    const float mean = block_sum(sm, red) / (float)d;
    float q = 0.f;
    for (int s = 0; s < ns; ++s) {
#pragma unroll
      for (int c = 0; c < CPT; ++c) {
        const int col = wide_col<V>(s, c);
        if (col < d) {
          if (ns > 1) wide_load<T, V>(xr + col, v[c]);
#pragma unroll
          for (int i = 0; i < V; ++i) { const float t = v[c][i] - mean; q += t * t; }
        }
      }
    }
    const float rstd = rsqrtf(block_sum(q, red) / (float)d + eps);
    if (threadIdx.x == 0) { stats[row * 2] = mean; stats[row * 2 + 1] = rstd; }
    for (int s = 0; s < ns; ++s) {
#pragma unroll
      for (int c = 0; c < CPT; ++c) {
        const int col = wide_col<V>(s, c);
        if (col < d) {
          if (ns > 1) wide_load<T, V>(xr + col, v[c]);
          float g[V], b[V], o[V];
          wide_param<V>(gamma + col, g);
          wide_param<V>(beta + col, b);
#pragma unroll
          for (int i = 0; i < V; ++i) o[i] = (v[c][i] - mean) * rstd * g[i] + b[i];
          wide_store<T, V>(yr + col, o);
        }
      }
    }
  }
}

template <typename T, int V>
__device__ __forceinline__ void ln_bwd_in(const T* dy, const T* x, const float* gamma, int64_t off, int col, float mean, float rstd,
                                          float (&xh)[V], float (&dyv)[V], float (&gd)[V]) {
  float xv[V], g[V];
  wide_load<T, V>(x + off + col, xv);
  wide_load<T, V>(dy + off + col, dyv);
  wide_param<V>(gamma + col, g);
#pragma unroll
  for (int i = 0; i < V; ++i) { xh[i] = (xv[i] - mean) * rstd; gd[i] = dyv[i] * g[i]; }
}

template <typename T, int V>
__global__ __launch_bounds__(NORM_THREADS) void layernorm_bwd_wide_kernel(const T* __restrict__ dy, const T* __restrict__ x,
                                                                           const float* __restrict__ gamma, const float* __restrict__ stats,
                                                                           T* __restrict__ dx, float* __restrict__ partial, int64_t rows,
                                                                           int d) {
  __shared__ float red[4];
  constexpr int CPT = WIDE_CPT<V>;
  const int ns = (d + WIDE_SLICE - 1) / WIDE_SLICE;
  const bool resident = ns == 1;
  float* grow = partial + (int64_t)blockIdx.x * d;
  float* brow = partial + ((int64_t)gridDim.x + blockIdx.x) * d;
  float ga[CPT][V], ba[CPT][V];
#pragma unroll
  for (int c = 0; c < CPT; ++c)
#pragma unroll
    for (int i = 0; i < V; ++i) { ga[c][i] = 0.f; ba[c][i] = 0.f; }
  if (!resident) {
    for (int s = 0; s < ns; ++s)
#pragma unroll
      for (int c = 0; c < CPT; ++c) {
        const int col = wide_col<V>(s, c);
        if (col < d) {
#pragma unroll
          for (int i = 0; i < V; ++i) { grow[col + i] = 0.f; brow[col + i] = 0.f; }
        }
      }
  }
  for (int64_t row = blockIdx.x; row < rows; row += gridDim.x) {
    const int64_t off = row * d;
    const float mean = stats[row * 2], rstd = stats[row * 2 + 1];
    float xh[CPT][V], gd[CPT][V];
    float s1 = 0.f, s2 = 0.f;
    for (int s = 0; s < ns; ++s) {
#pragma unroll
      for (int c = 0; c < CPT; ++c) {
        const int col = wide_col<V>(s, c);
        if (col < d) {
          float dyv[V];
          ln_bwd_in<T, V>(dy, x, gamma, off, col, mean, rstd, xh[c], dyv, gd[c]);
#pragma unroll
          for (int i = 0; i < V; ++i) {
            s1 += gd[c][i];
            s2 += gd[c][i] * xh[c][i];
            if (resident) { ga[c][i] += dyv[i] * xh[c][i]; ba[c][i] += dyv[i]; }
            else { grow[col + i] += dyv[i] * xh[c][i]; brow[col + i] += dyv[i]; }
          }
        }
      }
    }
    s1 = block_sum(s1, red) / (float)d;
    s2 = block_sum(s2, red) / (float)d;
    for (int s = 0; s < ns; ++s) {
#pragma unroll
      for (int c = 0; c < CPT; ++c) {
        const int col = wide_col<V>(s, c);
        if (col < d) {
          if (!resident) {
            float dyv[V];
            ln_bwd_in<T, V>(dy, x, gamma, off, col, mean, rstd, xh[c], dyv, gd[c]);
          }
          float o[V];
#pragma unroll
          for (int i = 0; i < V; ++i) o[i] = rstd * (gd[c][i] - s1 - xh[c][i] * s2);
          wide_store<T, V>(dx + off + col, o);
        }
      }
    }
  }
  if (resident) {
#pragma unroll
    for (int c = 0; c < CPT; ++c) {
      const int col = wide_col<V>(0, c);
      if (col < d) {
#pragma unroll
        for (int i = 0; i < V; ++i) { grow[col + i] = ga[c][i]; brow[col + i] = ba[c][i]; }
      }
    }
  }
}

inline int clamp_blocks(int64_t b, int64_t cap) { return (int)(b < 1 ? 1 : (b > cap ? cap : b)); }
inline int packed_blocks(int64_t groups) { return clamp_blocks(ceil_div(groups, 4), NORM_PACKED_BLOCKS); }
inline int packed_blocks_bwd(int64_t groups) { return clamp_blocks(ceil_div(groups, 4), 2 * (int64_t)meant_num_cus()); }
inline int norm_blocks(int64_t rows) { return clamp_blocks(ceil_div(rows, 4), NORM_MAX_BLOCKS); }
inline size_t dtype_bytes(int dtype) { return dtype == MEANT_BF16 ? 2 : 4; }

enum NormKind { NORM_PACKED, NORM_ROW, NORM_WIDE };
struct NormRoute { NormKind kind; int R, C, V; };
inline NormRoute norm_route(int64_t rows, int64_t d, bool may_pack = true) {
  if (d % 8 != 0 || d > MAXC * 512) return {NORM_WIDE, 0, 0, d % 8 == 0 ? 8 : 1};
  const int nchunk = (int)(d >> 3);
  for (int R = 1; may_pack && rows > 0 && d > 0 && R <= 4; R *= 2)
    if ((R * nchunk) % 64 == 0 && R * nchunk / 64 <= 3 && rows % R == 0) return {NORM_PACKED, R, R * nchunk / 64, 8};
  return {NORM_ROW, 0, 0, 8};
}
inline bool norm_aligned(const NormRoute& nr, const void* p, size_t elt) {
  return nr.V == 8 ? meant_aligned16(p) : (reinterpret_cast<uintptr_t>(p) % elt) == 0;
}

template <int N> using Int = std::integral_constant<int, N>;
template <typename F> inline int switch_c(int C, F&& f) { return C == 1 ? f(Int<1>{}) : C == 2 ? f(Int<2>{}) : f(Int<3>{}); }
template <typename F> inline int switch_v(int V, F&& f) { return V == 8 ? f(Int<8>{}) : f(Int<1>{}); }

inline int norm_colsums(const float* partial, int nb, int64_t d, float* out1, float* out2, int accumulate2, void* stream) {
  int rc = colsum_launch(partial, d, out1, nb, d, MEANT_F32, 0, (hipStream_t)stream);
  if (rc || !out2) return rc;
  return colsum_launch(partial + (size_t)nb * d, d, out2, nb, d, MEANT_F32, accumulate2, (hipStream_t)stream);
}

inline int launched(const char* name) { MEANT_LAUNCH_CHECK(name); return MEANT_OK; }
int launch_fwd_unpacked(const char* name, const NormRoute& nr, const void* x, const float* scale, void* y, float* rinv, int64_t rows, int64_t d,
                        float eps, float drop_p, uint64_t seed, int64_t d_part, const float* offset, int dtype, void* stream) {
  if (nr.kind == NORM_ROW) {
    DISPATCH_DTYPE(dtype, T, hipLaunchKernelGGL(rmsnorm_fwd_kernel<T>, dim3(norm_blocks(rows)), dim3(NORM_THREADS), 0, (hipStream_t)stream,
                                                (const T*)x, scale, (T*)y, rinv, rows, (int)d, eps, drop_p, seed, (int)d_part, offset));
    return launched(name);
  }
  return switch_v(nr.V, [&](auto v) -> int {
    DISPATCH_DTYPE(dtype, T, hipLaunchKernelGGL((rmsnorm_fwd_wide_kernel<T, v.value>), dim3(norm_blocks(rows)), dim3(NORM_THREADS), 0,
                                                (hipStream_t)stream, (const T*)x, scale, (T*)y, rinv, rows, (int)d, eps, drop_p, seed,
                                                (int)d_part, offset));
    return launched(name);
  });
}

int launch_fwd_packed(const char* name, const NormRoute& nr, const void* x, const float* scale, void* y, float* rinv, int64_t rows, int64_t d,
                      float eps, float drop_p, uint64_t seed, int dtype, void* stream) {
  return switch_c(nr.C, [&](auto c) -> int {
    DISPATCH_DTYPE(dtype, T, hipLaunchKernelGGL((rmsnorm_fwd_packed_kernel<T, c.value>), dim3(packed_blocks(rows / nr.R)), dim3(NORM_THREADS), 0,
                                                (hipStream_t)stream, (const T*)x, scale, (T*)y, rinv, rows, (int)d, nr.R, eps, drop_p, seed));
    return launched(name);
  });
}

int launch_stats_packed(const char* name, const NormRoute& nr, const void* x, float* rinv, int64_t rows, int64_t d, float eps, int dtype,
                        void* stream) {
  return switch_c(nr.C, [&](auto c) -> int {
    DISPATCH_DTYPE(dtype, T, hipLaunchKernelGGL((rmsnorm_stats_packed_kernel<T, c.value>), dim3(packed_blocks(rows / nr.R)), dim3(NORM_THREADS), 0,
                                                (hipStream_t)stream, (const T*)x, rinv, rows, (int)d, nr.R, eps));
    return launched(name);
  });
}

template <int POOL, bool GELU_IN>
int launch_fwd_pooled(const char* name, const NormRoute& nr, const void* x, const float* scale, void* y, float* rinv, float* pooled,
                      int64_t ngroups, int64_t d, int64_t group_rows, float eps, float drop_p, uint64_t seed, int dtype, void* stream) {
  const int nb = (int)(ngroups < NORM_PACKED_BLOCKS ? ngroups : NORM_PACKED_BLOCKS);
  return switch_c(nr.C, [&](auto c) -> int {
    DISPATCH_DTYPE(dtype, T, hipLaunchKernelGGL((rmsnorm_fwd_pooled_kernel<T, c.value, POOL, GELU_IN>), dim3(nb), dim3(NORM_THREADS), 0,
                                                (hipStream_t)stream, (const T*)x, scale, (T*)y, rinv, ngroups, (int)d, nr.R, eps, drop_p, seed,
                                                pooled, (int)group_rows));
    return launched(name);
  });
}

template <int BC, bool CHAIN>
int launch_bwd_packed(const char* name, const NormRoute& nr, int nbp, const void* dy, const void* x, const float* scale, const float* rinv,
                      void* dx, float* partial, int64_t rows, int64_t d, float eps, float drop_p, uint64_t seed, const void* dres,
                      const void* gelu_pre, int64_t group_rows, const NormChain& ch, int dtype, void* stream) {
  return switch_c(nr.C, [&](auto c) -> int {
    DISPATCH_DTYPE(dtype, T, hipLaunchKernelGGL((rmsnorm_bwd_packed_kernel<T, c.value, BC, CHAIN>), dim3(nbp), dim3(NORM_THREADS), 0,
                                                (hipStream_t)stream, (const T*)dy, (const T*)x, scale, rinv, (T*)dx, partial, rows, (int)d, nr.R,
                                                eps, drop_p, seed, (const T*)dres, (const T*)gelu_pre, (int)group_rows, ch));
    return launched(name);
  });
}

int launch_bwd_unpacked(const char* name, const NormRoute& nr, int nb, const void* dy, const void* x, const float* scale, const float* rinv,
                        void* dx, float* partial, int64_t rows, int64_t d, float eps, float drop_p, uint64_t seed, const void* dres,
                        const void* gelu_pre, int64_t d_part, float* partial_off, int dtype, void* stream) {
  if (nr.kind == NORM_ROW) {
    DISPATCH_DTYPE(dtype, T, hipLaunchKernelGGL(rmsnorm_bwd_kernel<T>, dim3(nb), dim3(NORM_THREADS), 0, (hipStream_t)stream, (const T*)dy,
                                                (const T*)x, scale, rinv, (T*)dx, partial, rows, (int)d, eps, drop_p, seed, (const T*)dres,
                                                (const T*)gelu_pre, (int)d_part, partial_off));
    return launched(name);
  }
  auto wide = [&](auto v, auto off) -> int {
    DISPATCH_DTYPE(dtype, T, hipLaunchKernelGGL((rmsnorm_bwd_wide_kernel<T, v.value, off.value>), dim3(nb), dim3(NORM_THREADS), 0,
                                                (hipStream_t)stream, (const T*)dy, (const T*)x, scale, rinv, (T*)dx, partial, rows, (int)d, eps,
                                                drop_p, seed, (const T*)dres, (const T*)gelu_pre, (int)d_part, partial_off));
    return launched(name);
  };
  return switch_v(nr.V, [&](auto v) -> int { return partial_off ? wide(v, std::true_type{}) : wide(v, std::false_type{}); });
}

int launch_ln_fwd(const char* name, const NormRoute& nr, const void* x, const float* gamma, const float* beta, void* y, float* stats,
                  int64_t rows, int64_t d, float eps, int dtype, void* stream) {
  if (nr.kind == NORM_ROW) {
    DISPATCH_DTYPE(dtype, T, hipLaunchKernelGGL(layernorm_fwd_kernel<T>, dim3(norm_blocks(rows)), dim3(NORM_THREADS), 0, (hipStream_t)stream,
                                                (const T*)x, gamma, beta, (T*)y, stats, rows, (int)d, eps));
    return launched(name);
  }
  return switch_v(nr.V, [&](auto v) -> int {
    DISPATCH_DTYPE(dtype, T, hipLaunchKernelGGL((layernorm_fwd_wide_kernel<T, v.value>), dim3(norm_blocks(rows)), dim3(NORM_THREADS), 0,
                                                (hipStream_t)stream, (const T*)x, gamma, beta, (T*)y, stats, rows, (int)d, eps));
    return launched(name);
  });
}

int launch_ln_bwd(const char* name, const NormRoute& nr, int nb, const void* dy, const void* x, const float* gamma, const float* stats, void* dx,
                  float* partial, int64_t rows, int64_t d, int dtype, void* stream) {
  if (nr.kind == NORM_ROW) {
    DISPATCH_DTYPE(dtype, T, hipLaunchKernelGGL(layernorm_bwd_kernel<T>, dim3(nb), dim3(NORM_THREADS), 0, (hipStream_t)stream, (const T*)dy,
                                                (const T*)x, gamma, stats, (T*)dx, partial, rows, (int)d));
    return launched(name);
  }
  return switch_v(nr.V, [&](auto v) -> int {
    DISPATCH_DTYPE(dtype, T, hipLaunchKernelGGL((layernorm_bwd_wide_kernel<T, v.value>), dim3(nb), dim3(NORM_THREADS), 0, (hipStream_t)stream,
                                                (const T*)dy, (const T*)x, gamma, stats, (T*)dx, partial, rows, (int)d));
    return launched(name);
  });
}

int rmsnorm_fwd_any(const char* name, bool may_pack, const void* x, const float* scale, const float* offset, void* y, float* rinv, int64_t rows,
                    int64_t d, int64_t d_part, float eps, float drop_p, uint64_t seed, int dtype, void* stream) {
  MEANT_REQUIRE(x && scale && y && rinv, MEANT_ERR_ARG, "%s: null pointer", name);
  MEANT_REQUIRE(rows >= 0 && d > 0 && d <= NORM_MAX_D && d_part >= 1 && d_part <= d, MEANT_ERR_UNSUPPORTED,
                "%s: unsupported d=%lld, d_part=%lld: need 1 <= d_part <= d", name, (long long)d, (long long)d_part);
  MEANT_REQUIRE(drop_p >= 0.f && drop_p < 1.f, MEANT_ERR_ARG, "%s: drop_p out of range", name);
  const NormRoute nr = norm_route(rows, d, may_pack);
  const size_t eb = dtype_bytes(dtype);
  MEANT_REQUIRE(norm_aligned(nr, x, eb) && norm_aligned(nr, y, eb) && norm_aligned(nr, scale, 4), MEANT_ERR_ARG, "%s: alignment", name);
  if (rows == 0) return MEANT_OK;
  if (nr.kind == NORM_PACKED) return launch_fwd_packed(name, nr, x, scale, y, rinv, rows, d, eps, drop_p, seed, dtype, stream);
  return launch_fwd_unpacked(name, nr, x, scale, y, rinv, rows, d, eps, drop_p, seed, d_part, offset, dtype, stream);
}

int rmsnorm_bwd_any(const char* name, bool may_pack, const void* dy, const void* x, const float* scale, const float* rinv, void* dx, float* dscale,
                    float* doffset, int64_t rows, int64_t d, int64_t d_part, float eps, float drop_p, uint64_t seed, const void* dres,
                    const void* gelu_pre, int dtype, void* workspace, size_t workspace_bytes, void* stream) {
  MEANT_REQUIRE(dy && x && scale && rinv && dx && dscale && workspace, MEANT_ERR_ARG, "%s: null pointer", name);
  MEANT_REQUIRE(rows > 0 && d > 0 && d <= NORM_MAX_D && d_part >= 1 && d_part <= d, MEANT_ERR_UNSUPPORTED,
                "%s: unsupported d=%lld, d_part=%lld: need 1 <= d_part <= d", name, (long long)d, (long long)d_part);
  MEANT_REQUIRE(workspace_bytes >= meant_rmsnorm_bwd_ws(rows, d), MEANT_ERR_WORKSPACE, "%s: workspace too small", name);
  const NormRoute nr = norm_route(rows, d, may_pack);
  float* part1 = (float*)workspace;
  if (nr.kind == NORM_PACKED) {
    const int nbp = packed_blocks_bwd(rows / nr.R);
    const int rc = launch_bwd_packed<0, false>(name, nr, nbp, dy, x, scale, rinv, dx, part1, rows, d, eps, drop_p, seed, dres, gelu_pre, 1,
                                                NormChain{}, dtype, stream);
    return rc ? rc : norm_colsums(part1, nbp, d, dscale, nullptr, 0, stream);
  }
  const size_t eb = dtype_bytes(dtype);
  MEANT_REQUIRE(nr.kind != NORM_WIDE || (norm_aligned(nr, dy, eb) && norm_aligned(nr, x, eb) && norm_aligned(nr, dx, eb) && norm_aligned(nr, scale, 4) &&
                                         (!dres || norm_aligned(nr, dres, eb)) && (!gelu_pre || norm_aligned(nr, gelu_pre, eb))),
                MEANT_ERR_ARG, "%s: alignment", name);
  const int nb = norm_blocks(rows);
  const int rc = launch_bwd_unpacked(name, nr, nb, dy, x, scale, rinv, dx, part1, rows, d, eps, drop_p, seed, dres, gelu_pre, d_part,
                                     doffset ? part1 + (size_t)nb * d : nullptr, dtype, stream);
  return rc ? rc : norm_colsums(part1, nb, d, dscale, doffset, 0, stream);
}

}

extern "C" size_t meant_rmsnorm_bwd_ws(int64_t rows, int64_t d) {
  const int64_t nb = norm_blocks(rows) > packed_blocks(rows) ? norm_blocks(rows) : packed_blocks(rows);
  return (size_t)nb * d * sizeof(float) * 2;
}

extern "C" int meant_rmsnorm_fwd(const void* x, const float* scale, void* y, float* rinv, int64_t rows, int64_t d,
                                 float eps, float drop_p, uint64_t seed, int dtype, void* stream) {
  return rmsnorm_fwd_any("rmsnorm_fwd", true, x, scale, nullptr, y, rinv, rows, d, d, eps, drop_p, seed, dtype, stream);
}

extern "C" int meant_rmsnorm_bwd(const void* dy, const void* x, const float* scale, const float* rinv, void* dx,
                                 float* dscale, int64_t rows, int64_t d, float eps, float drop_p, uint64_t seed,
                                 const void* dres, const void* gelu_pre, int dtype, void* workspace, size_t workspace_bytes,
                                 void* stream) {
  return rmsnorm_bwd_any("rmsnorm_bwd", true, dy, x, scale, rinv, dx, dscale, nullptr, rows, d, d, eps, drop_p, seed, dres, gelu_pre, dtype,
                         workspace, workspace_bytes, stream);
}

extern "C" int meant_rmsnorm_partial_fwd(const void* x, const float* scale, const float* offset, void* y, float* rinv, int64_t rows,
                                         int64_t d, int64_t d_part, float eps, int dtype, void* stream) {
  return rmsnorm_fwd_any("rmsnorm_partial_fwd", false, x, scale, offset, y, rinv, rows, d, d_part, eps, 0.f, 0, dtype, stream);
}

extern "C" int meant_rmsnorm_partial_bwd(const void* dy, const void* x, const float* scale, const float* rinv, void* dx, float* dscale,
                                         float* doffset, int64_t rows, int64_t d, int64_t d_part, float eps, int dtype, void* workspace,
                                         size_t workspace_bytes, void* stream) {
  return rmsnorm_bwd_any("rmsnorm_partial_bwd", false, dy, x, scale, rinv, dx, dscale, doffset, rows, d, d_part, eps, 0.f, 0, nullptr, nullptr,
                         dtype, workspace, workspace_bytes, stream);
}

extern "C" int meant_rmsnorm_pooled_ok(int64_t rows, int64_t d, int64_t group_rows) {
  if (group_rows <= 0 || rows % group_rows) return 0;
  const NormRoute nr = norm_route(rows, d);
  return nr.kind == NORM_PACKED && group_rows % nr.R == 0;
}

extern "C" int meant_rmsnorm_fwd_pooled(const void* x, const float* scale, void* y, float* rinv, float* pooled, int64_t rows, int64_t d,
                                        int64_t group_rows, int pool_input, int gelu_input, float eps, float drop_p, uint64_t seed,
                                        int dtype, void* stream) {
  const char* name = "rmsnorm_fwd_pooled";
  MEANT_REQUIRE(x && scale && rinv && pooled, MEANT_ERR_ARG, "rmsnorm_fwd_pooled: null pointer");
  MEANT_REQUIRE(!(pool_input && gelu_input), MEANT_ERR_UNSUPPORTED, "rmsnorm_fwd_pooled: gelu_input goes with pool_input == 0");
  MEANT_REQUIRE(meant_rmsnorm_pooled_ok(rows, d, group_rows), MEANT_ERR_UNSUPPORTED,
                "rmsnorm_fwd_pooled: rows=%lld d=%lld group_rows=%lld is not a packed shape (see meant_rmsnorm_pooled_ok)", (long long)rows,
                (long long)d, (long long)group_rows);
  const NormRoute nr = norm_route(rows, d);
  const size_t eb = dtype_bytes(dtype);
  MEANT_REQUIRE(norm_aligned(nr, x, eb) && norm_aligned(nr, scale, 4) && (!y || norm_aligned(nr, y, eb)), MEANT_ERR_ARG,
                "rmsnorm_fwd_pooled: 16-byte alignment");
  MEANT_REQUIRE(drop_p >= 0.f && drop_p < 1.f, MEANT_ERR_ARG, "rmsnorm_fwd_pooled: drop_p out of range");
  const int64_t ngroups = rows / group_rows;
  if (pool_input) return launch_fwd_pooled<2, false>(name, nr, x, scale, y, rinv, pooled, ngroups, d, group_rows, eps, drop_p, seed, dtype, stream);
  if (gelu_input) return launch_fwd_pooled<1, true>(name, nr, x, scale, y, rinv, pooled, ngroups, d, group_rows, eps, drop_p, seed, dtype, stream);
  return launch_fwd_pooled<1, false>(name, nr, x, scale, y, rinv, pooled, ngroups, d, group_rows, eps, drop_p, seed, dtype, stream);
}

extern "C" int meant_rmsnorm_bwd_pooled(const void* dy, int dy_pooled, const void* x, const float* scale, const float* rinv, void* dx,
                                        float* dscale, int64_t rows, int64_t d, int64_t group_rows, float eps, float drop_p, uint64_t seed,
                                        const void* dres, int dres_pooled, const void* gelu_pre, int dtype, void* workspace,
                                        size_t workspace_bytes, void* stream) {
  MEANT_REQUIRE(dy && (x || gelu_pre) && scale && rinv && dx && dscale && workspace, MEANT_ERR_ARG, "rmsnorm_bwd_pooled: null pointer");
  MEANT_REQUIRE((dy_pooled || dres_pooled) && (!dres_pooled || dres), MEANT_ERR_ARG, "rmsnorm_bwd_pooled: nothing pooled (use meant_rmsnorm_bwd)");
  MEANT_REQUIRE(meant_rmsnorm_pooled_ok(rows, d, group_rows) && rows < 2147483647LL, MEANT_ERR_UNSUPPORTED, "rmsnorm_bwd_pooled: not a packed shape");
  MEANT_REQUIRE(workspace_bytes >= meant_rmsnorm_bwd_ws(rows, d), MEANT_ERR_WORKSPACE, "rmsnorm_bwd_pooled: workspace too small");
  const NormRoute nr = norm_route(rows, d);
  const int nbp = packed_blocks_bwd(rows / nr.R);
  const int bc = (dy_pooled ? 1 : 0) | (dres_pooled ? 2 : 0) | (x ? 0 : 4);
  MEANT_REQUIRE(bc == 1 || bc == 2 || bc == 3 || bc == 5, MEANT_ERR_UNSUPPORTED, "rmsnorm_bwd_pooled: unsupported combination");
  auto launch = [&](auto b) -> int {
    return launch_bwd_packed<decltype(b)::value, false>("rmsnorm_bwd_pooled", nr, nbp, dy, x, scale, rinv, dx, (float*)workspace, rows, d, eps,
                                                        drop_p, seed, dres, gelu_pre, group_rows, NormChain{}, dtype, stream);
  };
  const int rc = bc == 1 ? launch(Int<1>{}) : bc == 2 ? launch(Int<2>{}) : bc == 3 ? launch(Int<3>{}) : launch(Int<5>{});
  return rc ? rc : norm_colsums((const float*)workspace, nbp, d, dscale, nullptr, 0, stream);
}

extern "C" int meant_rmsnorm_stats(const void* x, float* rinv, int64_t rows, int64_t d, float eps, int dtype, void* stream) {
  MEANT_REQUIRE(x && rinv, MEANT_ERR_ARG, "rmsnorm_stats: null pointer");
  const NormRoute nr = norm_route(rows, d);
  MEANT_REQUIRE(nr.kind == NORM_PACKED, MEANT_ERR_UNSUPPORTED,
                "rmsnorm_stats: rows=%lld d=%lld is not a packed shape (see meant_rmsnorm_pooled_ok)", (long long)rows, (long long)d);
  MEANT_REQUIRE(norm_aligned(nr, x, dtype_bytes(dtype)), MEANT_ERR_ARG, "rmsnorm_stats: 16-byte alignment");
  return launch_stats_packed("rmsnorm_stats", nr, x, rinv, rows, d, eps, dtype, stream);
}

extern "C" int meant_rmsnorm_bwd_chain(const void* dy, int dy_pooled, const void* x, const float* scale, const float* rinv, void* dx_scaled,
                                       float* dscale, int64_t rows, int64_t d, int64_t group_rows, float eps, float drop_p, uint64_t seed,
                                       const void* gelu_pre, const float* up_rinv, const float* up_bias, float up_eps, int64_t up_d,
                                       float* kcoef, float* dbias_up, int dtype, void* workspace, size_t workspace_bytes, void* stream) {
  const char* name = "rmsnorm_bwd_chain";
  MEANT_REQUIRE(dy && gelu_pre && scale && rinv && dx_scaled && dscale && up_rinv && up_bias && kcoef && dbias_up && workspace, MEANT_ERR_ARG,
                "rmsnorm_bwd_chain: null pointer");
  MEANT_REQUIRE((x != nullptr) != (dy_pooled != 0), MEANT_ERR_UNSUPPORTED,
                "rmsnorm_bwd_chain: either token-level dy with the stored activation x, or pooled dy with x formed from gelu_pre");
  const NormRoute nr = norm_route(rows, d);
  MEANT_REQUIRE(nr.kind == NORM_PACKED && rows < 2147483647LL && (!dy_pooled || meant_rmsnorm_pooled_ok(rows, d, group_rows)),
                MEANT_ERR_UNSUPPORTED, "rmsnorm_bwd_chain: rows=%lld d=%lld is not a packed shape (see meant_rmsnorm_pooled_ok)", (long long)rows,
                (long long)d);
  MEANT_REQUIRE(workspace_bytes >= meant_rmsnorm_bwd_ws(rows, d), MEANT_ERR_WORKSPACE, "rmsnorm_bwd_chain: workspace too small");
  const int nbp = packed_blocks_bwd(rows / nr.R);
  float* part1 = (float*)workspace;
  MEANT_REQUIRE(up_d > 0 && up_d < (1LL << 30), MEANT_ERR_ARG, "rmsnorm_bwd_chain: bad up_d");
  const NormChain ch{up_rinv, up_bias, kcoef, part1 + (size_t)nbp * d, up_eps, (int)up_d};
  const int rc = dy_pooled ? launch_bwd_packed<5, true>(name, nr, nbp, dy, x, scale, rinv, dx_scaled, part1, rows, d, eps, drop_p, seed, nullptr,
                                                        gelu_pre, group_rows, ch, dtype, stream)
                           : launch_bwd_packed<0, true>(name, nr, nbp, dy, x, scale, rinv, dx_scaled, part1, rows, d, eps, drop_p, seed, nullptr,
                                                        gelu_pre, 1, ch, dtype, stream);
  return rc ? rc : norm_colsums(part1, nbp, d, dscale, dbias_up, 1, stream);
}

extern "C" int meant_layernorm_fwd(const void* x, const float* gamma, const float* beta, void* y, float* stats,
                                   int64_t rows, int64_t d, float eps, int dtype, void* stream) {
  MEANT_REQUIRE(x && gamma && beta && y && stats, MEANT_ERR_ARG, "layernorm_fwd: null pointer");
  MEANT_REQUIRE(rows > 0 && d > 0 && d <= NORM_MAX_D, MEANT_ERR_UNSUPPORTED, "layernorm_fwd: unsupported d=%lld", (long long)d);
  const NormRoute nr = norm_route(rows, d, false);
  const size_t eb = dtype_bytes(dtype);
  MEANT_REQUIRE(nr.kind != NORM_WIDE || (norm_aligned(nr, x, eb) && norm_aligned(nr, y, eb) && norm_aligned(nr, gamma, 4) && norm_aligned(nr, beta, 4)),
                MEANT_ERR_ARG, "layernorm_fwd: alignment");
  return launch_ln_fwd("layernorm_fwd", nr, x, gamma, beta, y, stats, rows, d, eps, dtype, stream);
}

extern "C" int meant_layernorm_bwd(const void* dy, const void* x, const float* gamma, const float* stats, void* dx,
                                   float* dgamma, float* dbeta, int64_t rows, int64_t d, int dtype, void* workspace,
                                   size_t workspace_bytes, void* stream) {
  MEANT_REQUIRE(dy && x && gamma && stats && dx && dgamma && dbeta && workspace, MEANT_ERR_ARG, "layernorm_bwd: null pointer");
  MEANT_REQUIRE(rows > 0 && d > 0 && d <= NORM_MAX_D, MEANT_ERR_UNSUPPORTED, "layernorm_bwd: unsupported d=%lld", (long long)d);
  MEANT_REQUIRE(workspace_bytes >= meant_rmsnorm_bwd_ws(rows, d), MEANT_ERR_WORKSPACE, "layernorm_bwd: workspace too small");
  const NormRoute nr = norm_route(rows, d, false);
  const size_t eb = dtype_bytes(dtype);
  MEANT_REQUIRE(nr.kind != NORM_WIDE || (norm_aligned(nr, dy, eb) && norm_aligned(nr, x, eb) && norm_aligned(nr, dx, eb) && norm_aligned(nr, gamma, 4)),
                MEANT_ERR_ARG, "layernorm_bwd: alignment");
  const int nb = norm_blocks(rows);
  const int rc = launch_ln_bwd("layernorm_bwd", nr, nb, dy, x, gamma, stats, dx, (float*)workspace, rows, d, dtype, stream);
  return rc ? rc : norm_colsums((const float*)workspace, nb, d, dgamma, dbeta, 0, stream);
}
```

### meant_amd/modules.py

```python
from __future__ import annotations

import math
from typing import Optional

import torch
from torch import nn

from . import ops
from ._lib import EPI_NONE, EPI_GELU, EPI_SIGMOID


COMPOSE_PRE_LINEAR = True

POOL_LAST_LINEAR = True

import os as _os
TWO_STREAMS = _os.environ.get("MEANT_TWO_STREAMS", "1") != "0"
_SIDE = {}


def _side_stream(device):
    key = (device.type, device.index)
    if key not in _SIDE:
        _SIDE[key] = torch.cuda.Stream(device=device)
# ... 8 lines not shown
def _hi_stream(device):
    key = (device.type, device.index)
    if key not in _HI:
        _HI[key] = torch.cuda.Stream(device=device, priority=-1)
    return _HI[key]


def resolve_compute_dtype(module: nn.Module, like: Optional[torch.Tensor]) -> torch.dtype:
    forced = getattr(module, "compute_dtype", None)
    if forced is not None:
        return forced
    if torch.is_autocast_enabled():
        return torch.bfloat16
    if like is not None and like.dtype in (torch.bfloat16, torch.float16):
        return torch.bfloat16
    return torch.float32


class RMSNorm(nn.Module):

    def __init__(self, d, p=-1., eps=1e-8, bias=False):
        super().__init__()
        self.eps, self.d, self.p, self.bias = eps, d, p, bias
        self.scale = nn.Parameter(torch.ones(d))
        if bias:
            self.offset = nn.Parameter(torch.zeros(d))

    def forward(self, x, drop_p: float = 0.0, seed: int = 0):
        partial = 0. <= self.p <= 1.
        if partial or self.bias:
            d_part = int(self.d * self.p) if partial else self.d
            if d_part < 1:
                raise ValueError(f"meant_amd.RMSNorm: p = {self.p} leaves no element to take the statistics over (d = {self.d})")
            y = ops.rmsnorm_partial(x, self.scale, self.offset if self.bias else None, d_part, self.eps, any_width=True)
            return ops.dropout(y, drop_p, seed) if drop_p > 0.0 else y
        return ops.rmsnorm(x, self.scale, self.eps, drop_p, seed, any_width=True)


class LayerNorm(nn.LayerNorm):
    def forward(self, x):
        return ops.layernorm(x, self.weight, self.bias, self.eps, any_width=True)


class Linear(nn.Linear):
    def forward(self, x, residual=None, epilogue=EPI_NONE):
        return ops.linear(x, self.weight, self.bias, residual, epilogue)


class RotaryEmbedding(nn.Module):

    def __init__(self, dim, custom_freqs=None, freqs_for='lang', theta=10000, max_freq=10, num_freqs=1,
                 learned_freq=False, use_xpos=False, xpos_scale_base=512):
        super().__init__()
        if custom_freqs is not None:
            freqs = custom_freqs
        elif freqs_for == 'lang':
            freqs = 1. / (theta ** (torch.arange(0, dim, 2)[:(dim // 2)].float() / dim))
        elif freqs_for == 'pixel':
            freqs = torch.linspace(1., max_freq / 2, dim // 2) * math.pi
        elif freqs_for == 'constant':
            freqs = torch.ones(num_freqs).float()
        else:
            raise ValueError(f'unknown modality {freqs_for}')
        self.learned_freq = bool(learned_freq)
        self.freqs = nn.Parameter(freqs, requires_grad=self.learned_freq)
        self.use_xpos = use_xpos
        self.scale_base = xpos_scale_base
        if use_xpos:
            self.register_buffer('scale', (torch.arange(0, dim, 2) + 0.4 * dim) / (1.4 * dim))
        else:
            self.register_buffer('scale', None)
        self._tables = {}

    def __getstate__(self):
        st = self.__dict__.copy()
        st['_tables'] = {}
        return st

    @property
    def rot_dim(self) -> int:
        return 2 * self.freqs.numel()

    def tables_autograd(self, seq_len: int) -> tuple:
        f = self.freqs.float()
        pos = torch.arange(seq_len, device=f.device, dtype=f.dtype)
        ang = torch.repeat_interleave(pos[:, None] * f[None, :], 2, dim=-1)
        cos, sin = ang.cos(), ang.sin()
        if not self.use_xpos:
            return cos, sin, cos, sin
        power = (torch.arange(seq_len, device=f.device) - seq_len // 2) / self.scale_base
        s = self.scale.float()[None, :] ** power[:, None]
        s = torch.cat((s, s), dim=-1)
        si = s ** -1
        return cos * s, sin * s, cos * si, sin * si

    def tables(self, seq_len: int, device, head_dim: Optional[int] = None) -> tuple:
        key = (seq_len, str(device), self.freqs._version, self.freqs.data_ptr())
        hit = self._tables.get(key)
        if hit is not None:
            if head_dim is None:
                return hit
            pkey = ("pad", head_dim) + key
            padded = self._tables.get(pkey)
            if padded is None:
                padded = self._tables[pkey] = ops.pad_rotary_tables(hit, head_dim)
            return padded
        with torch.no_grad():
            f = self.freqs.detach().float().cpu()
            pos = torch.arange(seq_len)
            ang = torch.repeat_interleave(pos.to(f.dtype)[:, None] * f[None, :], 2, dim=-1)
            cos, sin = ang.cos(), ang.sin()
            if self.use_xpos:
                power = (pos - seq_len // 2) / self.scale_base
                s = self.scale.detach().float().cpu()[None, :] ** power[:, None]
                s = torch.cat((s, s), dim=-1)
                si = s ** -1
                t = (cos * s, sin * s, cos * si, sin * si)
            else:
                t = (cos, sin, cos, sin)
            t = tuple(x.contiguous().to(device) for x in t)
            if not self.use_xpos:
                t = (t[0], t[1], t[0], t[1])
        self._tables = {k: v for k, v in self._tables.items() if k[-2:] == key[-2:]}
        self._tables[key] = t
        return t if head_dim is None else self.tables(seq_len, device, head_dim)


def _rotate_pairs(t, a, b):
    R = a.shape[1]
    tr = t[..., :R].float()
    pr = tr.reshape(*tr.shape[:-1], R // 2, 2)
    rot = torch.stack((-pr[..., 1], pr[..., 0]), dim=-1).reshape(tr.shape)
    out = tr * a[None, :, None, :] + rot * b[None, :, None, :]
    return torch.cat((out.to(t.dtype), t[..., R:]), dim=-1)


def learned_rotary_attention(x, mod, rot: RotaryEmbedding, key_mask, causal: bool, pre=None):
    G, S, d = x.shape
    H = mod.num_heads
    wqkv = torch.cat([mod.q.weight, mod.v.weight, mod.k.weight], dim=0)
    bqkv = torch.cat([mod.q.bias, mod.v.bias, mod.k.bias], dim=0)
    if pre is not None:
        wqkv, bqkv = ops.compose_linear(pre.weight, pre.bias, wqkv, bqkv)
    D = wqkv.shape[0] // 3
    qkv = ops.linear(x.reshape(G * S, d), wqkv, bqkv).view(G, S, 3, H, D // H)
    qa, qb, ka, kb = rot.tables_autograd(S)
    q, k = _rotate_pairs(qkv[:, :, 0], qa, qb), _rotate_pairs(qkv[:, :, 1], ka, kb)
    packed = torch.stack((q, k, qkv[:, :, 2]), dim=2).reshape(G * S, 3 * D)
    return ops.attention_core(packed, G, S, H, 1.0 / math.sqrt(D), None, causal, key_mask).view(G, S, D)


def score_dropout_attention(x, mod, rot: RotaryEmbedding, key_mask, causal: bool, p: float, seed: int, pre=None):
    G, S, d = x.shape
    H = mod.num_heads
    wqkv = torch.cat([mod.q.weight, mod.v.weight, mod.k.weight], dim=0)
    bqkv = torch.cat([mod.q.bias, mod.v.bias, mod.k.bias], dim=0)
    if pre is not None:
        wqkv, bqkv = ops.compose_linear(pre.weight, pre.bias, wqkv, bqkv)
    D = wqkv.shape[0] // 3
    qkv = ops.linear(x.reshape(G * S, d), wqkv, bqkv)
    tables = None
    if rot is not None and getattr(rot, 'learned_freq', False):
        q5 = qkv.view(G, S, 3, H, D // H)
        qa, qb, ka, kb = rot.tables_autograd(S)
        qkv = torch.stack((_rotate_pairs(q5[:, :, 0], qa, qb), _rotate_pairs(q5[:, :, 1], ka, kb), q5[:, :, 2]), dim=2).reshape(G * S, 3 * D)
    elif rot is not None:
        tables = rot.tables(S, x.device)
    return ops.attention_core_score_dropout(qkv, G, S, H, 1.0 / math.sqrt(D), p, seed, tables, causal, key_mask).view(G, S, D)


class attention(nn.Module):

    def __init__(self, num_heads, dim, pos_emb: RotaryEmbedding, mask=False, droput=0.):
        super().__init__()
        self.num_heads, self.dim = num_heads, dim
        self.Dh = int(dim / num_heads)
        self.dropout = nn.Dropout(droput)
        self.pos_emb = pos_emb
        self.mask = mask
        self.softmax = nn.Softmax(dim=-1)
        self.multi_mad = Linear(self.num_heads * self.Dh, self.dim)
        self.q = Linear(self.dim, self.Dh * self.num_heads)
        self.v = Linear(self.dim, self.Dh * self.num_heads)
        self.k = Linear(self.dim, self.Dh * self.num_heads)

    def core(self, x, pre=None):
        if self.pos_emb is not None and getattr(self.pos_emb, 'learned_freq', False):
            return learned_rotary_attention(x, self, self.pos_emb, None, bool(self.mask), pre)
        tables = self.pos_emb.tables(x.shape[1], x.device, ops.run_head_dim(self.Dh, x.dtype)) if self.pos_emb is not None else None
        prew = (pre.weight, pre.bias) if pre is not None else None
        return ops.qkv_attention(x, self.q.weight, self.q.bias, self.v.weight, self.v.bias, self.k.weight, self.k.bias,
                                 tables, None, bool(self.mask), self.num_heads, pre=prew)

    def forward(self, input):
        out = self.multi_mad(self.core(input))
        if self.training and self.dropout.p > 0:
            out = self.dropout(out)
        return out


class xPosAttention(nn.Module):

    def __init__(self, num_heads, dim, xPos: RotaryEmbedding, mask=True, droput=0.):
        super().__init__()
        self.num_heads, self.dim = num_heads, dim
        self.Dh = int(dim / num_heads)
        self.dropout = nn.Dropout(droput)
        self.xPos = xPos
        self.mask = mask
        self.softmax = nn.Softmax(dim=-1)
        self.multi_mad = Linear(self.num_heads * self.Dh, self.dim)
        self.q = Linear(self.dim, self.Dh * self.num_heads)
        self.v = Linear(self.dim, self.Dh * self.num_heads)
        self.k = Linear(self.dim, self.Dh * self.num_heads)

    def core(self, x, attention_mask=None, pre=None):
        if self.training and self.dropout.p > 0:
            return score_dropout_attention(x, self, self.xPos, attention_mask, bool(self.mask), float(self.dropout.p), _seed(), pre)
        if getattr(self.xPos, 'learned_freq', False):
            return learned_rotary_attention(x, self, self.xPos, attention_mask, bool(self.mask), pre)
        tables = self.xPos.tables(x.shape[1], x.device, ops.run_head_dim(self.Dh, x.dtype))
        prew = (pre.weight, pre.bias) if pre is not None else None
        return ops.qkv_attention(x, self.q.weight, self.q.bias, self.v.weight, self.v.bias, self.k.weight, self.k.bias,
                                 tables, attention_mask, bool(self.mask), self.num_heads, pre=prew)

    def forward(self, input, attention_mask=None):
        return self.multi_mad(self.core(input, attention_mask))


class temporal(nn.Module):

    def __init__(self, num_heads, dim, mask=False, droput=0.):
        super().__init__()
        self.num_heads, self.dim = num_heads, dim
        self.Dh = int(dim / num_heads)
        self.dropout = nn.Dropout(droput)
        self.mask = mask
        self.softmax = nn.Softmax(dim=-1)
        self.multi_mad = Linear(self.num_heads * self.Dh, self.dim)
        self.atten_size = self.Dh * self.num_heads
        self.q = Linear(self.dim, self.atten_size)
        self.v = Linear(self.dim, self.atten_size)
        self.k = Linear(self.dim, self.atten_size)

    def forward(self, input):
        o = ops.temporal_attention(input, self.q.weight, self.q.bias, self.v.weight, self.v.bias, self.k.weight, self.k.bias,
                                   self.num_heads)
        return self.multi_mad(o)


def _seed() -> int:
    return int(torch.randint(0, 2 ** 62, (1,)).item())


class visionEncoder(nn.Module):

    def __init__(self, dim, num_heads, flash=False):
        super().__init__()
        self.dim, self.num_heads = dim, num_heads
        self.posEmbed = RotaryEmbedding(dim=math.floor(dim / num_heads / 2), freqs_for='pixel')
        atten = attention(num_heads, dim, self.posEmbed)
        self.encode = nn.ModuleList([RMSNorm(dim), Linear(dim, dim), atten, RMSNorm(dim), Linear(dim, dim)])
        self.encode2 = nn.ModuleList([RMSNorm(dim), Linear(dim, dim), nn.GELU(), RMSNorm(dim), Linear(dim, dim)])

    def forward(self, input, pool: bool = False, fold=None):
        e, e2 = self.encode, self.encode2
        n, res = ops.rmsnorm_fork(input, e[0].scale, e[0].eps)
        if COMPOSE_PRE_LINEAR and e[1].bias is not None:
            h = e[2].multi_mad(e[2].core(n, pre=e[1]))
        else:
            h = e[2](e[1](n))
        h = e[3](h)
        x1 = e[4](h, residual=res)
        fold = ops.norm_linear_ok(x1, e2[1].weight, fold)
        if pool and ops.pooled_norm_ok(x1, x1.shape[1]):
            if fold:
                return ops.norm_linear_gelu_norm_pooled(x1, e2[0].scale, e2[0].eps, e2[1].weight, e2[1].bias, e2[3].scale, e2[3].eps)
            n, xm = ops.rmsnorm_fork_pooled(x1, e2[0].scale, e2[0].eps)
            return ops.linear_gelu_rmsnorm_pooled(n, e2[1].weight, e2[1].bias, e2[3].scale, e2[3].eps), xm
        if fold:
            h, res = ops.norm_linear_gelu_norm(x1, e2[0].scale, e2[0].eps, e2[1].weight, e2[1].bias, e2[3].scale, e2[3].eps)
        else:
            n, res = ops.rmsnorm_fork(x1, e2[0].scale, e2[0].eps)
            h = ops.linear_gelu_rmsnorm(n, e2[1].weight, e2[1].bias, e2[3].scale, e2[3].eps)
        if pool:
            return h, res
        return e2[4](h, residual=res)


class languageEncoder(nn.Module):

    def __init__(self, dim, num_heads, dropout=0.0, flash=False):
        super().__init__()
        self.dim, self.num_heads = dim, num_heads
        self.xPos = RotaryEmbedding(dim=48, use_xpos=True)
        att = xPosAttention(num_heads, dim, self.xPos)
        self.encode = nn.ModuleList([RMSNorm(dim), Linear(dim, dim), att, RMSNorm(dim), nn.Dropout(dropout), Linear(dim, dim)])
        self.encode2 = nn.ModuleList([RMSNorm(dim), Linear(dim, dim), nn.GELU(), RMSNorm(dim), nn.Dropout(), Linear(dim, dim)])

    def forward(self, input, attention_mask=None, pool: bool = False, fold=None):
        e, e2 = self.encode, self.encode2
        p1 = e[4].p if self.training else 0.0
        p2 = e2[4].p if self.training else 0.0
        n, res = ops.rmsnorm_fork(input, e[0].scale, e[0].eps)
        if COMPOSE_PRE_LINEAR and e[1].bias is not None:
            h = e[2].multi_mad(e[2].core(n, attention_mask, pre=e[1]))
        else:
            h = e[2](e[1](n), attention_mask)
        h = e[3](h, drop_p=p1, seed=_seed() if p1 > 0 else 0)
        x1 = e[5](h, residual=res)
        fold = ops.norm_linear_ok(x1, e2[1].weight, fold)
        seed2 = _seed() if p2 > 0 else 0
        if pool and ops.pooled_norm_ok(x1, x1.shape[1]):
            if fold:
                return ops.norm_linear_gelu_norm_pooled(x1, e2[0].scale, e2[0].eps, e2[1].weight, e2[1].bias, e2[3].scale, e2[3].eps, p2, seed2)
            n, xm = ops.rmsnorm_fork_pooled(x1, e2[0].scale, e2[0].eps)
            return ops.linear_gelu_rmsnorm_pooled(n, e2[1].weight, e2[1].bias, e2[3].scale, e2[3].eps, p2, seed2), xm
        if fold:
            h, res = ops.norm_linear_gelu_norm(x1, e2[0].scale, e2[0].eps, e2[1].weight, e2[1].bias, e2[3].scale, e2[3].eps, p2, seed2)
        else:
            n, res = ops.rmsnorm_fork(x1, e2[0].scale, e2[0].eps)
            h = ops.linear_gelu_rmsnorm(n, e2[1].weight, e2[1].bias, e2[3].scale, e2[3].eps, p2, seed2)
        if pool:
            return h, res
        return e2[5](h, residual=res)


class temporalEncoder(nn.Module):

    def __init__(self, dim, num_heads, lag, norms=True):
        super().__init__()
        self.dim, self.num_heads, self.lag = dim, num_heads, lag
        self.temp_embedding = nn.Parameter(torch.randn(1, lag, dim))
        if norms:
            mods = [RMSNorm(dim), Linear(dim, dim), temporal(num_heads, dim), RMSNorm(dim), Linear(dim, dim)]
        else:
            mods = [Linear(dim, dim), temporal(num_heads, dim), Linear(dim, dim)]
        self.temp_encode = nn.ModuleList(mods)

    def forward(self, x):
        x = ops.add_rowvec(x, self.temp_embedding)
        for mod in self.temp_encode:
            x = mod(x)
        return x


class _Patchify(nn.Module):

    def __init__(self, p):
        super().__init__()
        self.p = p
        self.out_dtype = torch.float32
        self.norm_mean, self.norm_std = 0.0, 1.0

    def set_normalization(self, mean: float, std: float):
        self.norm_mean, self.norm_std = float(mean), float(std)

    def forward(self, images):
        return ops.patchify(images, self.p, self.out_dtype, self.norm_mean, self.norm_std)


class _PatchEmbed(nn.Sequential):
    def __init__(self, patch_dim, dim, p):
        super().__init__(_Patchify(p), Linear(patch_dim, dim))

    def forward(self, images, dtype=torch.float32):
        self[0].out_dtype = dtype
        return self[1](self[0](images))


def _run_encoder(enc, x, *args, checkpoint: bool = False, **kw):
    if checkpoint and torch.is_grad_enabled() and x.requires_grad:
        from torch.utils.checkpoint import checkpoint as _ckpt
        return _ckpt(enc, x, *args, use_reentrant=False, preserve_rng_state=True, **kw)
    return enc(x, *args, **kw)


def _ckpt_setting(model):
    v = getattr(model, "activation_checkpointing", False)
    return v if isinstance(v, bool) else int(v)


def _run_stack(encoders, x, *args, checkpoint=False):
    n = len(encoders)
    fold = ops.stack_fold(n, x.numel() // x.shape[-1], x.shape[-1])
    for i, enc in enumerate(encoders):
        ck = checkpoint if isinstance(checkpoint, bool) else i < checkpoint
        last = enc.encode2[-1]
        if POOL_LAST_LINEAR and i == n - 1 and isinstance(last, Linear):
            h, res = _run_encoder(enc, x, *args, checkpoint=ck, pool=True, fold=fold)
            return (h, res, last.weight, last.bias)
        x = _run_encoder(enc, x, *args, checkpoint=ck, fold=fold)
    return x


def _pool_parts(compute_dtype, *stacks):
    if all(isinstance(st, tuple) for st in stacks):
        if all(st[0].dim() == 3 for st in stacks):
            return ops.pool_linear_cat(list(stacks))
        parts = [st if st[0].dim() == 2 else (ops.meanpool_f32(st[0]), ops.meanpool_f32(st[1]), st[2], st[3]) for st in stacks]
        return ops.pooled_linear_cat(parts, compute_dtype)
    toks = []
    for st in stacks:
        if isinstance(st, tuple):
            h, res, w, b = st
            if h.dim() == 2:
                raise RuntimeError("meant_amd: one stack pooled its last layer, the other did not")
            st = ops.linear(h, w, b, residual=res)
        toks.append(st)
    return ops.meanpool_cat(*toks)


POOL_OWN_STREAM = _os.environ.get("MEANT_POOL_OWN_STREAM", "1") == "1"


def _pool_own_stream(compute_dtype, st):
    if not POOL_OWN_STREAM or not (isinstance(st, tuple) and st[0].dim() == 2):
        return st
    return ops.pooled_linear_cat([st], compute_dtype)


def _embed(mods, ids, dtype):
    x = ids
    for mod in mods:
        if isinstance(mod, nn.Embedding) and mod.max_norm is None and not mod.sparse and x.dtype in (torch.int64, torch.int32):
            x = ops.embedding(x, mod.weight, dtype)
        else:
            x = mod(x)
    if x.dtype != dtype:
        x = x.to(dtype)
    return x


HEAD_F32_MAX_CLASSES = 64


def _head(mods, x):
    x = mods[0](x)
    if x.dtype != torch.float32 and mods[1].weight.shape[0] <= HEAD_F32_MAX_CLASSES:
        x = x.float()
    if isinstance(mods[2], nn.Sigmoid):
        return mods[1](x, epilogue=EPI_SIGMOID)
    return mods[2](mods[1](x))


class meant(nn.Module):

    def __init__(self, text_dim, image_dim, price_dim, height, width, patch_res, lag, num_classes, embedding, flash=False,
                 num_heads=8, num_encoders=1, channels=4):
        super().__init__()
        self.lag, self.text_dim, self.image_dim = lag, text_dim, image_dim
        self.dim = text_dim + image_dim
        self.num_heads = num_heads
        self.channels = channels
        self.patch_dim = channels * patch_res * patch_res
        self.n = int((height * width) / (patch_res ** 2))
        self.embedding = nn.ModuleList([embedding])
        self.patchEmbed = _PatchEmbed(self.patch_dim, image_dim, patch_res)
        self.visionEncoders = nn.ModuleList([visionEncoder(image_dim, num_heads, flash=flash) for _ in range(num_encoders)])
        self.languageEncoders = nn.ModuleList([languageEncoder(text_dim, num_heads, flash=flash) for _ in range(num_encoders)])
        self.temporal_encoding = nn.ModuleList([temporalEncoder(self.dim, num_heads, lag)])
        self.mlpHead = nn.ModuleList([RMSNorm(self.dim), Linear(self.dim, num_classes), nn.Sigmoid()])
        self.compute_dtype = None

    def forward(self, tweets, images, attention_mask=None):
        dt = resolve_compute_dtype(self, images)
        B = images.shape[0]
        if images.is_cuda and TWO_STREAMS:
            ops.set_index_stream(images.device, _side_stream(images.device))
        words = _embed(self.embedding, tweets.reshape(B * self.lag, tweets.shape[2]), dt)
        if attention_mask is not None:
            attention_mask = attention_mask.reshape(B * self.lag, attention_mask.shape[2])
        ck = _ckpt_setting(self)
        side = _side_stream(images.device) if (TWO_STREAMS and images.is_cuda and not ck) else None
        if side is not None:
            main = torch.cuda.current_stream()
            side.wait_stream(main)
            with torch.cuda.stream(side):
                img = self.patchEmbed(images.reshape(B * self.lag, *images.shape[2:]), dt)
                img = _run_stack(self.visionEncoders, img, checkpoint=ck)
                img = _pool_own_stream(dt, img)
        if side is not None and LANG_PRIORITY:
            hi = _hi_stream(images.device)
            hi.wait_stream(main)
            with torch.cuda.stream(hi):
                words = _run_stack(self.languageEncoders, words, attention_mask, checkpoint=ck)
                words = _pool_own_stream(dt, words)
            main.wait_stream(hi)
            for tt in (words if isinstance(words, tuple) else (words,)):
                if tt is not None and tt.is_cuda:
                    tt.record_stream(main)
        else:
            words = _run_stack(self.languageEncoders, words, attention_mask, checkpoint=ck)
        if side is not None:
            main.wait_stream(side)
            for tt in (img if isinstance(img, tuple) else (img,)):
                if tt is not None and tt.is_cuda:
                    tt.record_stream(main)
        else:
            img = self.patchEmbed(images.reshape(B * self.lag, *images.shape[2:]), dt)
            img = _run_stack(self.visionEncoders, img, checkpoint=ck)
        done = [torch.is_tensor(st) and st.dim() == 2 for st in (words, img)]
        if any(done):
            fused = torch.cat([st if d_ else _pool_parts(dt, st) for st, d_ in zip((words, img), done)], dim=1).view(B, self.lag, self.dim)
        else:
            fused = _pool_parts(dt, words, img).view(B, self.lag, self.dim)
        for enc in self.temporal_encoding:
            fused = enc(fused)
        return _head(self.mlpHead, fused).squeeze(dim=1).float()


class meant_vision(nn.Module):

    def __init__(self, image_dim, price_dim, height, width, patch_res, lag, num_classes, flash=False, num_heads=8,
                 num_encoders=1, channels=4):
        super().__init__()
        self.dim = image_dim
        self.num_heads = num_heads
        self.channels = channels
        self.patch_dim = channels * patch_res * patch_res
        self.n = int((height * width) / (patch_res ** 2))
        self.patchEmbed = _PatchEmbed(self.patch_dim, image_dim, patch_res)
        self.visionEncoders = nn.ModuleList([visionEncoder(image_dim, num_heads, flash=flash) for _ in range(num_encoders)])
        self.temporal_encoding = nn.ModuleList([temporalEncoder(self.dim, num_heads, lag, norms=False)])
        self.mlpHead = nn.ModuleList([LayerNorm(self.dim), Linear(self.dim, num_classes), nn.Sigmoid()])
        self.compute_dtype = None

    def forward(self, images):
        dt = resolve_compute_dtype(self, images)
        B, L = images.shape[0], images.shape[1]
        img = self.patchEmbed(images.reshape(B * L, *images.shape[2:]), dt)
        img = _run_stack(self.visionEncoders, img)
        fused = _pool_parts(dt, img).view(B, L, self.dim)
        for enc in self.temporal_encoding:
            fused = enc(fused)
        return _head(self.mlpHead, fused).squeeze(dim=1).float()


class meant_tweet(nn.Module):

    def __init__(self, text_dim, price_dim, lag, num_classes, embedding, flash=False, num_heads=8, num_encoders=1, channels=4):
        super().__init__()
        self.dim = text_dim
        self.num_heads = num_heads
        self.embedding = nn.ModuleList([embedding])
        self.languageEncoders = nn.ModuleList([languageEncoder(text_dim, num_heads, flash=flash) for _ in range(num_encoders)])
        self.temporal_encoding = nn.ModuleList([temporalEncoder(self.dim, num_heads, lag, norms=False)])
        self.mlpHead = nn.ModuleList([LayerNorm(self.dim), Linear(self.dim, num_classes), nn.Sigmoid()])
        self.lag = lag
        self.compute_dtype = None

    def forward(self, tweets, attention_mask=None):
        dt = resolve_compute_dtype(self, None)
        B = tweets.shape[0]
        words = _embed(self.embedding, tweets.reshape(B * self.lag, tweets.shape[2]), dt)
        attention_mask = attention_mask.reshape(B * self.lag, attention_mask.shape[2])
        words = _run_stack(self.languageEncoders, words, attention_mask)
        fused = _pool_parts(dt, words).view(B, self.lag, self.dim)
        for enc in self.temporal_encoding:
            fused = enc(fused)
        return _head(self.mlpHead, fused).squeeze(dim=1).float()


class meant_vqa(nn.Module):

    def __init__(self, text_dim, image_dim, price_dim, height, width, patch_res, lag, num_classes, embedding, flash=False,
                 num_heads=8, num_encoders=1, channels=4):
        super().__init__()
        self.lag, self.text_dim, self.image_dim = lag, text_dim, image_dim
        self.dim = text_dim + image_dim
        self.num_heads = num_heads
        self.channels = channels
        self.patch_dim = channels * patch_res * patch_res
        self.n = int((height * width) / (patch_res ** 2))
        self.embedding = nn.ModuleList([embedding])
        self.patchEmbed = _PatchEmbed(self.patch_dim, image_dim, patch_res)
        self.visionEncoders = nn.ModuleList([visionEncoder(image_dim, num_heads, flash=flash) for _ in range(num_encoders)])
        self.languageEncoders = nn.ModuleList([languageEncoder(text_dim, num_heads, flash=flash) for _ in range(num_encoders)])
        self.multimodal_embedding = nn.Sequential(nn.Linear(1, self.dim), nn.GELU(), RMSNorm(self.dim), nn.Linear(self.dim, self.dim))
        self.multimodal_encoding = nn.ModuleList([visionEncoder(self.dim, num_heads, flash=flash)])
        self.mlpHead = nn.ModuleList([RMSNorm(self.dim), Linear(self.dim, num_classes), nn.Sigmoid()])
        self.compute_dtype = None

    def forward(self, tweets, images, attention_mask=None):
        dt = resolve_compute_dtype(self, images)
        words = _embed(self.embedding, tweets, dt)
        words = _run_stack(self.languageEncoders, words, attention_mask)
        img = self.patchEmbed(images, dt)
        img = _run_stack(self.visionEncoders, img)
        fused = _pool_parts(dt, words, img)
        return _head(self.mlpHead, fused).float()


flash_attention = attention
xPosAttention_flash = xPosAttention


MLM_LABELLED_ONLY = _os.environ.get("MEANT_MLM_LABELLED_ONLY", "1") != "0"


def _is_roberta_lm_head(h) -> bool:
    return all(hasattr(h, a) for a in ("dense", "layer_norm", "decoder")) and isinstance(getattr(h, "decoder"), nn.Linear)


class meant_language_pretrainer(nn.Module):

    def __init__(self, num_encoders, mlm_input_dim, embedding, lm_head, flash=False, lag=5, text_dim=768, num_heads=8):
        super().__init__()
        self.embedding = nn.ModuleList([embedding])
        self.languageEncoders = nn.ModuleList([languageEncoder(text_dim, num_heads, flash=flash) for _ in range(num_encoders)])
        self.mlm_head = lm_head
        self.lag = lag
        self.labelled_only = MLM_LABELLED_ONLY
        self.last_head_rows = None

    def _encode(self, words, attention_mask):
        dt = resolve_compute_dtype(self, None)
        x = _embed(self.embedding, words, dt)
        fold = ops.stack_fold(len(self.languageEncoders), x.numel() // x.shape[-1], x.shape[-1])
        for enc in self.languageEncoders:
            x = enc(x, attention_mask=attention_mask, fold=fold)
        return x

    def _head_features(self, x):
        h = self.mlm_head
        y = ops.linear(x, h.dense.weight, h.dense.bias, None, EPI_GELU)
        return ops.layernorm(y, h.layer_norm.weight, h.layer_norm.bias, h.layer_norm.eps)

    def forward(self, words, attention_mask=None):
        x = self._encode(words, attention_mask)
        h = self.mlm_head
        if _is_roberta_lm_head(h):
            return ops.vocab_linear(self._head_features(x), h.decoder.weight, h.decoder.bias)
        return h(x)

    def loss(self, words, attention_mask, labels, ignore_index: int = -100, labelled_only=None):
        h = self.mlm_head
        roberta = _is_roberta_lm_head(h)
        T = labels.numel()
        sel, m = None, T
        if roberta and (self.labelled_only if labelled_only is None else labelled_only):
            sel = ops.select_rows(labels, h.decoder.weight.shape[0], ignore_index)
            m = ops.padded_rows(sel.n)
            if m >= T:
                sel, m = None, T
        x = self._encode(words, attention_mask)
        self.last_head_rows = m
        if sel is None and not labels.is_cuda:
            labels = labels.to(x.device)
        if not roberta:
            return ops.softmax_cross_entropy(h(x), labels, ignore_index)
        if sel is not None:
            x = ops.take_rows(x.reshape(T, x.shape[-1]), sel.idx, sel.inv, m)
            labels = sel.target_sel[:m]
        return ops.vocab_linear_cross_entropy(self._head_features(x), h.decoder.weight, h.decoder.bias, labels, ignore_index)


def _is_vit_mim_decoder(dec) -> bool:
    return (isinstance(dec, nn.Sequential) and len(dec) == 2 and isinstance(dec[0], nn.Conv2d) and dec[0].kernel_size == (1, 1)
            and dec[0].stride == (1, 1) and dec[0].groups == 1 and isinstance(dec[1], nn.PixelShuffle))


class meant_vision_pretrainer(nn.Module):

    def __init__(self, num_encoders, decoder, mlm_input_dim, patch_res=16, channels=4, height=224, width=224, image_dim=768, num_heads=8):
        super().__init__()
        self.channels = channels
        self.patch_dim = channels * patch_res * patch_res
        self.n = int((height * width) / (patch_res ** 2))
        self.patchEmbed = _PatchEmbed(self.patch_dim, image_dim, patch_res)
        self.visionEncoders = nn.ModuleList([visionEncoder(image_dim, num_heads, flash=True)])
        self.decoder = decoder

    def forward(self, images):
        dt = resolve_compute_dtype(self, images)
        x = self.patchEmbed(images, dt)
        fold = ops.stack_fold(len(self.visionEncoders), x.numel() // x.shape[-1], x.shape[-1])
        for enc in self.visionEncoders:
            x = enc(x, fold=fold)
        b, n, c = x.shape
        hw = math.floor(n ** 0.5)
        dec = self.decoder
        if _is_vit_mim_decoder(dec):
            conv, r = dec[0], dec[1].upscale_factor
            y = ops.linear(x, conv.weight.view(conv.out_channels, c), conv.bias)
            co = conv.out_channels // (r * r)
            y = y.view(b, hw, hw, co, r, r).permute(0, 3, 1, 4, 2, 5).reshape(b, co, hw * r, hw * r)
            return y
        return dec(x.permute(0, 2, 1).reshape(b, c, hw, hw))


class _TSAttention(nn.Module):

    def __init__(self, dim, dim_head=64, heads=8):
        super().__init__()
        self.heads, self.dim_head, self.scale = heads, dim_head, dim_head ** -0.5
        inner = dim_head * heads
        self.to_qkv = Linear(dim, inner * 3, bias=False)
        self.to_out = nn.Sequential(Linear(inner, dim), nn.Identity())

    def forward(self, x, plan, tables, group_mask=None, cls_mask=None, residual=None, drop_p=0.0):
        H, Dh = self.heads, self.dim_head
        Dp = ops.divided_head_dim(Dh, x.dtype)
        if Dp != Dh:
            w = self.to_qkv.weight
            wp = torch.nn.functional.pad(w.view(3 * H, Dh, w.shape[1]), (0, 0, 0, Dp - Dh)).reshape(3 * H * Dp, w.shape[1])
            qkv = ops.linear(x, wp)
            out = ops.divided_attention(qkv, plan, tables, H, self.scale, group_mask, cls_mask)
            out = out.view(*out.shape[:-1], H, Dp)[..., :Dh].reshape(*out.shape[:-1], H * Dh)
        else:
            qkv = self.to_qkv(x)
            out = ops.divided_attention(qkv, plan, tables, H, self.scale, group_mask, cls_mask)
        if drop_p > 0.0:
            return ops.dropout(self.to_out[0](out), drop_p, _seed()) + residual
        return self.to_out[0](out, residual=residual)


class _TSPreNorm(nn.Module):
    def __init__(self, dim, fn):
        super().__init__()
        self.fn, self.norm = fn, LayerNorm(dim)


class _TSPreTokenShift(nn.Module):

    def __init__(self, frames, fn):
        super().__init__()
        self.frames, self.fn = frames, fn

    def forward(self, x, *args, **kw):
        return self.fn(ops.token_shift(x, self.frames, (x.shape[1] - 1) // self.frames), *args, **kw)


class _TSFeedForward(nn.Module):
    def __init__(self, dim, mult=4):
        super().__init__()
        self.net = nn.Sequential(Linear(dim, dim * mult * 2), nn.Identity(), nn.Identity(), Linear(dim * mult, dim))

    def forward(self, x, residual=None, drop_p=0.0):
        h = ops.geglu(self.net[0](x))
        if drop_p > 0.0:
            h = ops.dropout(h, drop_p, _seed())
        return self.net[3](h, residual=residual)


class TimeSformer(nn.Module):

    def __init__(self, *, dim, num_frames, num_classes, image_size=224, patch_size=16, channels=3, depth=12, heads=8, dim_head=64,
                 attn_dropout=0., ff_dropout=0., rotary_emb=True, shift_tokens=False):
        super().__init__()
        self.use_rotary_emb = bool(rotary_emb)
        self.shift_tokens, self.attn_dropout, self.ff_dropout = bool(shift_tokens), float(attn_dropout), float(ff_dropout)
        assert image_size % patch_size == 0, "Image dimensions must be divisible by the patch size."
        self.heads, self.patch_size, self.dim_head, self.num_frames = heads, patch_size, dim_head, num_frames
        self.to_patch_embedding = Linear(channels * patch_size ** 2, dim)
        self.cls_token = nn.Parameter(torch.randn(1, dim))
        if rotary_emb:
            self.frame_rot_emb = nn.Module()
            self.frame_rot_emb.register_buffer("inv_freqs", 1.0 / (10000 ** (torch.arange(0, dim_head, 2).float() / dim_head)))
            self.image_rot_emb = nn.Module()
            self.image_rot_emb.register_buffer("scales", torch.logspace(0., math.log(10 / 2) / math.log(2), dim_head // 4, base=2))
        else:
            self.pos_emb = nn.Embedding(num_frames * (image_size // patch_size) ** 2 + 1, dim)
        wrap = (lambda fn: _TSPreTokenShift(num_frames, fn)) if shift_tokens else (lambda fn: fn)
        self.layers = nn.ModuleList([nn.ModuleList([_TSPreNorm(dim, wrap(_TSAttention(dim, dim_head, heads))),
                                                    _TSPreNorm(dim, wrap(_TSAttention(dim, dim_head, heads))),
                                                    _TSPreNorm(dim, wrap(_TSFeedForward(dim)))]) for _ in range(depth)])
        self.to_out = nn.Sequential(LayerNorm(dim), Linear(dim, num_classes))
        self._cache = {}

    def _plan(self, b, f, hp, wp, device):
        key = (b, f, hp, wp, str(device))
        hit = self._cache.get(key)
        if hit is not None:
            return hit
        n = hp * wp
        L = 1 + f * n
        with torch.no_grad():
            fr = ang = None
            if self.use_rotary_emb:
                inv = self.frame_rot_emb.inv_freqs.detach().float().cpu()
                fr = torch.arange(f).float()[:, None] * inv[None, :]
                fr = torch.cat((fr, fr), dim=-1)
                sc = self.image_rot_emb.scales.detach().float().cpu()[None, :]
                hs = torch.linspace(-1., 1., hp)[:, None] * sc * math.pi
                ws = torch.linspace(-1., 1., wp)[:, None] * sc * math.pi
                ang = torch.cat((hs[:, None, :].expand(hp, wp, -1), ws[None, :, :].expand(hp, wp, -1)), dim=-1).reshape(n, -1)
                ang = ang.repeat_interleave(2, dim=-1)

            def tabs(a):
                if a is None:
                    return None
                cos = torch.cat((torch.ones(1, a.shape[1]), a.cos())).contiguous().to(device)
                sin = torch.cat((torch.zeros(1, a.shape[1]), a.sin())).contiguous().to(device)
                return ops.pad_rotary_tables((cos, sin, cos, sin), (self.dim_head + 7) & ~7)

            def tables_of(index):
                G, S = index.shape
                boff = (torch.arange(b) * L)[:, None, None]
                idx_in = (boff + index[None]).reshape(-1)
                idx_dog = (boff + index[None]).clone()
                idx_dog[:, :, 0] = -1
                pos = torch.full((L,), -1, dtype=torch.long)
                pos[index[:, 1:].reshape(-1)] = (torch.arange(G)[:, None] * S + torch.arange(1, S)[None, :]).reshape(-1)
                idx_out = (torch.arange(b) * (G * S))[:, None] + pos[None, :]
                idx_out[:, 0] = -1
                i32 = lambda t: t.to(torch.int32).contiguous().to(device)
                return (i32(index), i32(idx_in), i32(idx_out.reshape(-1)), i32(idx_dog.reshape(-1)))
            tok = 1 + torch.arange(f * n).view(f, n)
            zero = torch.zeros(1, dtype=torch.long)
            idx_time = torch.stack([torch.cat((zero, tok[:, j])) for j in range(n)])
            idx_space = torch.stack([torch.cat((zero, tok[i, :])) for i in range(f)])
            cat_fwd = torch.cat((torch.full((b, 1), -2, dtype=torch.long), torch.arange(b * f * n).view(b, f * n)), dim=1)
            cat_bwd = (torch.arange(b) * L)[:, None] + 1 + torch.arange(f * n)[None, :]
            plan = (tabs(fr), tabs(ang), tables_of(idx_time), tables_of(idx_space),
                    cat_fwd.reshape(-1).to(torch.int32).to(device), cat_bwd.reshape(-1).to(torch.int32).to(device))
        self._cache = {key: plan}
        return plan

    def meant_forward(self, video, mask=None):
        b, f, c, hh, ww = video.shape
        p = self.patch_size
        assert hh % p == 0 and ww % p == 0, f"height {hh} and width {ww} of video must be divisible by the patch size {p}"
        hp, wp = hh // p, ww // p
        n = hp * wp
        dt = resolve_compute_dtype(self, video)
        tokens = self.to_patch_embedding(ops.patchify(video.reshape(b * f, c, hh, ww), p, dt)).view(b, f * n, -1)
        t_time, t_space, p_time, p_space, cat_fwd, cat_bwd = self._plan(b, f, hp, wp, video.device)
        x = ops.cls_concat(self.cls_token, tokens, cat_fwd, cat_bwd)
        if not self.use_rotary_emb:
            x = ops.add_rowvec(x, self.pos_emb.weight[:x.shape[1]].view(1, x.shape[1], -1))
        time_mask = cls_mask = None
        if mask is not None:
            m = mask.to(video.device).float()
            one = torch.ones(b, 1, device=video.device)
            time_mask = torch.cat((one, m), dim=1).repeat_interleave(n, dim=0)
            cls_mask = torch.cat((one, m.repeat_interleave(n, dim=1)), dim=1)
        pa = self.attn_dropout if self.training else 0.0
        pf = self.ff_dropout if self.training else 0.0
        for ta, sa, ff in self.layers:
            x = ta.fn(ta.norm(x), p_time, t_time, time_mask, cls_mask, residual=x, drop_p=pa)
            x = sa.fn(sa.norm(x), p_space, t_space, None, cls_mask, residual=x, drop_p=pa)
            x = ff.fn(ff.norm(x), residual=x, drop_p=pf)
        return x

    def forward(self, video, mask=None):
        return self.to_out(self.meant_forward(video, mask=mask)[:, 0])
```

### meant_amd/ops.py

```python
from __future__ import annotations

import math
import os
import threading
import weakref
from typing import NamedTuple, Optional

import torch

from . import _lib
from ._lib import lib, check, F32, BF16, EPI_NONE, EPI_GELU, EPI_RESIDUAL, EPI_SIGMOID


def _dt(t: torch.Tensor) -> int:
    if t.dtype == torch.float32:
        return F32
    if t.dtype == torch.bfloat16:
        return BF16
    raise TypeError(f"meant_amd: activations must be float32 or bfloat16, got {t.dtype}")


def _need_gpu(*ts):
    cur = None
    for t in ts:
# ... 952 lines not shown
            check(lib.meant_meanpool_bwd(_p(dout), ld, sa[2], _p(db), sb[0], sb[1], sb[2], dti, dto, _stream()), "meanpool_bwd")
        return da, db, None


TAIL_FP32 = os.environ.get("MEANT_TAIL_FP32") == "1"


def meanpool_cat(a, b=None):
    return _MeanPoolCat.apply(a, b, torch.float32 if TAIL_FP32 else a.dtype)


def meanpool_f32(a):
    return _MeanPoolCat.apply(a, None, torch.float32)


class _PoolLinearCat(torch.autograd.Function):

    @staticmethod
    def forward(ctx, out_dtype, *flat):
        parts = [flat[i:i + 4] for i in range(0, len(flat), 4)]
        _need_gpu(*[t for p in parts for t in p])
        G = parts[0][0].shape[0]
        widths = [p[2].shape[0] for p in parts]
        Dt = sum(widths)
        dev = parts[0][0].device
        out = torch.empty((G, Dt), device=dev, dtype=torch.float32)
        xm = torch.empty((G, Dt), device=dev, dtype=torch.float32)
        saved, off = [], 0
        for (h, x, W, b), N in zip(parts, widths):
            h, x = _c(h), _c(x)
            assert h.shape[0] == G and x.shape == h.shape[:2] + (N,) and h.dtype == x.dtype
            S, K = h.shape[1], h.shape[2]
            hm = torch.empty((G, K), device=dev, dtype=torch.float32)
            check(lib.meant_meanpool_fwd(_p(h), _p(hm), K, 0, G, S, K, _dt(h), F32, _stream()), "meanpool_fwd")
            check(lib.meant_meanpool_fwd(_p(x), _p(xm), Dt, off, G, S, N, _dt(x), F32, _stream()), "meanpool_fwd")
            w_f = _c(W.detach().float())
            bias_f = _c(b.detach().float()) if b is not None else None
            check(lib.meant_linear_fwd(_p(hm), K, _p(w_f), _p(bias_f), xm.data_ptr() + off * 4, Dt, out.data_ptr() + off * 4, Dt, None,
                                       G, N, K, EPI_RESIDUAL, F32, _stream()), "linear_fwd")
            saved.append((hm, W, b is not None, h.shape, h.dtype, off))
            off += N
        ctx.parts = saved
        return cast(out, out_dtype)

    @staticmethod
    def backward(ctx, dout):
        dout = cast(_c(dout), torch.float32)
        G, Dt = dout.shape
        grads = [None]
        for hm, W, has_b, hshape, hdt, off in ctx.parts:
            N, K = W.shape
            S = hshape[1]
            dy_ptr = dout.data_ptr() + off * 4
            dti = F32 if hdt == torch.float32 else BF16
            wT = weights.get((W,), torch.float32, True)
            dhm = torch.empty((G, K), device=dout.device, dtype=torch.float32)
            check(lib.meant_linear_bwd_dx(dy_ptr, Dt, _p(wT), _p(dhm), K, G, N, K, F32, _stream()), "linear_bwd_dx")
            dw = torch.zeros((N, K), device=dout.device, dtype=torch.float32)
            db = torch.zeros(N, device=dout.device, dtype=torch.float32) if has_b else None
            check(lib.meant_linear_bwd_dw(dy_ptr, Dt, _p(hm), K, _p(dw), _p(db), G, N, K, F32, None, 0, _stream()), "linear_bwd_dw")
            dh = torch.empty(hshape, device=dout.device, dtype=hdt)
            check(lib.meant_meanpool_bwd(_p(dhm), K, 0, _p(dh), G, S, K, dti, F32, _stream()), "meanpool_bwd")
            dx = torch.empty(hshape[:2] + (N,), device=dout.device, dtype=hdt)
            check(lib.meant_meanpool_bwd(_p(dout), Dt, off, _p(dx), G, S, N, dti, F32, _stream()), "meanpool_bwd")
            grads += [dh, dx, dw, db]
        return tuple(grads)


class _PooledLinearCat(torch.autograd.Function):

    @staticmethod
    def forward(ctx, out_dtype, *flat):
        parts = [flat[i:i + 4] for i in range(0, len(flat), 4)]
        _need_gpu(*[t for p in parts for t in p])
        G = parts[0][0].shape[0]
        widths = [p[2].shape[0] for p in parts]
        Dt = sum(widths)
        dev = parts[0][0].device
        out = torch.empty((G, Dt), device=dev, dtype=torch.float32)
        xs = _c(parts[0][1]) if len(parts) == 1 else torch.cat([p[1] for p in parts], dim=1)
        saved, off = [], 0
        for (hm, xm, W, b), N in zip(parts, widths):
            hm = _c(hm)
            K = hm.shape[1]
            w_f = _c(W.detach().float())
            bias_f = _c(b.detach().float()) if b is not None else None
            check(lib.meant_linear_fwd(_p(hm), K, _p(w_f), _p(bias_f), xs.data_ptr() + off * 4, Dt, out.data_ptr() + off * 4, Dt, None,
                                       G, N, K, EPI_RESIDUAL, F32, _stream()), "linear_fwd")
            saved.append((hm, W, b is not None, off))
            off += N
        ctx.parts = saved
        return cast(out, out_dtype)

    @staticmethod
    def backward(ctx, dout):
        dout = cast(_c(dout), torch.float32)
        G, Dt = dout.shape
        grads = [None]
        for hm, W, has_b, off in ctx.parts:
            N, K = W.shape
            dy_ptr = dout.data_ptr() + off * 4
            wT = weights.get((W,), torch.float32, True)
            dhm = torch.empty((G, K), device=dout.device, dtype=torch.float32)
            check(lib.meant_linear_bwd_dx(dy_ptr, Dt, _p(wT), _p(dhm), K, G, N, K, F32, _stream()), "linear_bwd_dx")
            dw = torch.zeros((N, K), device=dout.device, dtype=torch.float32)
            db = torch.zeros(N, device=dout.device, dtype=torch.float32) if has_b else None
            check(lib.meant_linear_bwd_dw(dy_ptr, Dt, _p(hm), K, _p(dw), _p(db), G, N, K, F32, None, 0, _stream()), "linear_bwd_dw")
            dxm = dout[:, off:off + N] if Dt == N else dout[:, off:off + N].contiguous()
            grads += [dhm, dxm, dw, db]
        return tuple(grads)


def pool_linear_cat(parts):
    flat = [t for p in parts for t in p]
    out_dtype = torch.float32 if TAIL_FP32 else parts[0][0].dtype
    return _PoolLinearCat.apply(out_dtype, *flat)


def pooled_linear_cat(parts, compute_dtype):
    out_dtype = torch.float32 if TAIL_FP32 else compute_dtype
    return _PooledLinearCat.apply(out_dtype, *[t for p in parts for t in p])


class _AddRowVec(torch.autograd.Function):

    @staticmethod
    def forward(ctx, x, v):
        _need_gpu(x, v)
        x = _c(x)
        B, L, d = x.shape
        vf = _c(v.detach().float()).view(L, d)
        y = torch.empty_like(x)
        check(lib.meant_add_rowvec(_p(x), _p(vf), _p(y), B * L, d, L, _dt(x), _stream()), "add_rowvec")
        ctx.meta = (B, L, d, v.shape)
        return y

    @staticmethod
    def backward(ctx, dy):
        B, L, d, vshape = ctx.meta
        dy = _c(dy)
        dv = torch.empty((L, d), device=dy.device, dtype=torch.float32)
        check(lib.meant_add_rowvec_bwd(_p(dy), _p(dv), B * L, d, L, _dt(dy), _stream()), "add_rowvec_bwd")
        return dy, dv.view(vshape)


def add_rowvec(x, v):
    return _AddRowVec.apply(x, v)


_RAW_DTYPES = {torch.float32: 0, torch.bfloat16: 1, torch.float64: 2, torch.uint8: 3}


def patchify(images, p: int, dtype: torch.dtype, mean: float = 0.0, std: float = 1.0):
    _need_gpu(images)
    if images.dtype not in _RAW_DTYPES:
        images = images.float()
    images = _c(images)
    G, Cc, Hh, Ww = images.shape
    n = (Hh // p) * (Ww // p)
    out = torch.empty((G, n, p * p * Cc), device=images.device, dtype=dtype)
    odt = F32 if dtype == torch.float32 else BF16
    if images.dtype in (torch.float32, torch.bfloat16) and mean == 0.0 and std == 1.0:
        check(lib.meant_patchify(_p(images), _dt(images), _p(out), G, Cc, Hh, Ww, p, odt, _stream()), "patchify")
    else:
        check(lib.meant_patchify_raw(_p(images), _RAW_DTYPES[images.dtype], float(mean), 1.0 / float(std), _p(out), G, Cc, Hh, Ww, p,
                                     odt, _stream()), "patchify_raw")
    return out


EMB_BF16_TABLE = os.environ.get("MEANT_EMB_BF16_TABLE", "1") == "1"


EMB_PRESORT = os.environ.get("MEANT_EMB_PRESORT", "1") == "1"
_aux_streams = {}
_aux_override = {}


def set_index_stream(device, stream) -> None:
    _aux_override[(device.type, device.index)] = stream


def _aux_stream(device):
    key = (device.type, device.index)
    if _aux_override.get(key) is not None:
        return _aux_override[key]
    st = _aux_streams.get(key)
    if st is None:
        st = _aux_streams[key] = torch.cuda.Stream(device=device)
    return st


def _emb_sorted_bwd_ok(n: int, d: int) -> bool:
    return d <= 1024 and d % 8 == 0 and (n >= 4096 or bool(_lib_option("deterministic")))


def _emb_seg_bwd_ok(n: int, d: int) -> bool:
    return d % 8 == 0 and (n >= 4096 or bool(_lib_option("deterministic")))


def _emb_bwd_route(n: int, d: int) -> str:
    if _emb_seg_bwd_ok(n, d) and d > 1024:
        return "seg"
    return "sorted" if _emb_sorted_bwd_ok(n, d) else "atomic"


def _sort_ids(ids_flat: torch.Tensor, V: int):
    n = ids_flat.numel()
    sorted_ids, order = torch.empty_like(ids_flat), torch.empty_like(ids_flat)
    wsb = lib.meant_sort_ids_ws(n, V)
    ws = torch.empty(wsb, device=ids_flat.device, dtype=torch.uint8)
    check(lib.meant_sort_ids(_p(ids_flat), n, V, _p(sorted_ids), _p(order), _p(ws), wsb, _stream()), "sort_ids")
    return sorted_ids, order


class _Embedding(torch.autograd.Function):

    @staticmethod
    def forward(ctx, ids, table, dtype):
        _need_gpu(ids, table)
        ids_c = _c(ids.long())
        V, d = table.shape
        n = ids_c.numel()
        out = torch.empty((*ids.shape, d), device=table.device, dtype=dtype)
        if dtype == torch.bfloat16 and EMB_BF16_TABLE and d % 8 == 0 and V < (1 << 31):
            tb = weights.get((table,), torch.bfloat16, False)
            idx = ids_c.view(-1).clamp(0, V - 1).to(torch.int32)
            check(lib.meant_gather_rows(_p(tb), _p(idx), None, _p(out), n, d, BF16, _stream()), "gather_rows")
        else:
            tf = _c(table.detach().float())
            check(lib.meant_embedding_fwd(_p(tf), _p(ids_c), _p(out), n, d, V, F32 if dtype == torch.float32 else BF16, _stream()),
                  "embedding_fwd")
        presort = None
        route = _emb_bwd_route(n, d)
        if EMB_PRESORT and ctx.needs_input_grad[1] and route != "atomic":
            main = torch.cuda.current_stream(ids_c.device)
            side = _aux_stream(ids_c.device)
            side.wait_stream(main)
            with torch.cuda.stream(side):
                sorted_ids, order = _sort_ids(ids_c.view(-1), V)
                ev = torch.cuda.Event()
                ev.record(side)
            presort = (sorted_ids, order, ev)
        ctx.save_for_backward(ids_c)
        ctx.presort = presort
        ctx.meta = (V, d)
        ctx.table = table
        _claim(table, "embedding")
        return out

    @staticmethod
    def backward(ctx, dout):
        (ids_c,) = ctx.saved_tensors
        V, d = ctx.meta
        dout = _c(dout)
        sink = _sink_of(ctx.table, "embedding") if grad_sinks else None
        if sink is not None and (sink.view.shape != (V, d) or not sink.view.is_contiguous()):
            sink = None
        dtab = sink.view if sink is not None else torch.zeros((V, d), device=dout.device, dtype=torch.float32)
        n = ids_c.numel()
        route = _emb_bwd_route(n, d)
        if route != "atomic":
            if ctx.presort is not None:
                sorted_ids, order, ev = ctx.presort
                cur = torch.cuda.current_stream(dout.device)
                cur.wait_event(ev)
                sorted_ids.record_stream(cur)
                order.record_stream(cur)
            else:
                sorted_ids, order = _sort_ids(ids_c.view(-1), V)
            nsl = sink.row_slices(ctx.table) if sink is not None else 1
            if route == "seg":
                wsb = lib.meant_embedding_bwd_seg_ws(n, d)
                ws = torch.empty(wsb, device=dout.device, dtype=torch.uint8)
                for c in range(nsl):
                    lo, hi = V * c // nsl, V * (c + 1) // nsl
                    check(lib.meant_embedding_bwd_seg(_p(dout), _p(sorted_ids), _p(order), _p(dtab), n, d, V, lo, hi, _dt(dout), _p(ws), wsb,
                                                      _stream()), "embedding_bwd_seg")
                    if nsl > 1:
                        sink.report_rows(ctx.table, lo, hi, c == nsl - 1)
                if nsl > 1:
                    return None, None, None
            elif nsl > 1:
                for c in range(nsl):
                    lo, hi = V * c // nsl, V * (c + 1) // nsl
                    check(lib.meant_embedding_bwd_sorted_range(_p(dout), _p(sorted_ids), _p(order), _p(dtab), n, d, V, lo, hi, _dt(dout),
                                                               _stream()), "embedding_bwd_sorted_range")
                    sink.report_rows(ctx.table, lo, hi, c == nsl - 1)
                return None, None, None
            else:
                check(lib.meant_embedding_bwd_sorted(_p(dout), _p(sorted_ids), _p(order), _p(dtab), n, d, V, _dt(dout), _stream()),
                      "embedding_bwd_sorted")
        else:
            check(lib.meant_embedding_bwd(_p(dout), _p(ids_c), _p(dtab), n, d, V, _dt(dout), _stream()), "embedding_bwd")
        if sink is not None:
            sink.report(ctx.table)
            return None, None, None
        return None, dtab, None


def embedding(ids, table, dtype):
    return _Embedding.apply(ids, table, dtype)


def cast(x: torch.Tensor, dtype: torch.dtype) -> torch.Tensor:
    _need_gpu(x)
    if x.dtype == dtype:
        return x
    x = _c(x)
    out = torch.empty_like(x, dtype=dtype)
    check(lib.meant_cast(_p(x), _dt(x), _p(out), F32 if dtype == torch.float32 else BF16, x.numel(), _stream()), "cast")
    return out


VOCAB_PAD = 256


class _SoftmaxCE(torch.autograd.Function):

    @staticmethod
    def forward(ctx, logits_pad, target, V, ignore_index):
        _need_gpu(logits_pad, target)
        logits_pad = _c(logits_pad)
        T, ld = logits_pad.shape
        assert ld % 8 == 0 and V <= ld
        tgt = _c(target.long())
        row_loss = torch.empty(T, device=logits_pad.device, dtype=torch.float32)
        lse = torch.empty(T, device=logits_pad.device, dtype=torch.float32)
        check(lib.meant_softmax_ce_fwd(_p(logits_pad), ld, _p(tgt), T, V, int(ignore_index), _p(row_loss), _p(lse), _dt(logits_pad),
                                       _stream()), "softmax_ce_fwd")
        nvalid = ((tgt != ignore_index) & (tgt >= 0) & (tgt < V)).sum().clamp_(min=1).float()
        ctx.save_for_backward(logits_pad, tgt, lse, nvalid)
        ctx.V, ctx.ignore_index = int(V), int(ignore_index)
        return row_loss.sum() / nvalid

    @staticmethod
    def backward(ctx, dloss):
        logits_pad, tgt, lse, nvalid = ctx.saved_tensors
        T, ld = logits_pad.shape
        g = (dloss.float() / nvalid).reshape(1).contiguous()
        dl = torch.empty_like(logits_pad)
        check(lib.meant_softmax_ce_bwd(_p(logits_pad), ld, _p(tgt), _p(lse), T, ctx.V, ctx.ignore_index, _p(g), _p(dl), _dt(logits_pad),
                                       _stream()), "softmax_ce_bwd")
        return dl, None, None, None


class _VocabLinear(torch.autograd.Function):

    @staticmethod
    def forward(ctx, x, weight, bias):
        _need_gpu(x, weight)
        V, d = weight.shape
        Vp = (V + VOCAB_PAD - 1) // VOCAB_PAD * VOCAB_PAD
        shp = x.shape
        x2 = _c(x).view(-1, d)
        w_c = weights.get((weight,), x.dtype, False, Vp - V)
        bias_f = None
        if bias is not None:
            bias_f = _c(torch.nn.functional.pad(bias.detach().float(), (0, Vp - V)))
        y, _ = _linear_fwd_raw(x2, w_c, bias_f, None, EPI_NONE, False)
        ctx.weight, ctx.bias, ctx.has_bias, ctx.in_shape, ctx.V = weight, bias, bias is not None, shp, V
        _claim(weight, "vocab"); _claim(bias, "vocab")
        ctx.save_for_backward(x2)
        return y.view(*shp[:-1], Vp)

    @staticmethod
    def backward(ctx, dy):
        (x2,) = ctx.saved_tensors
        V = ctx.V
        Vp = dy.shape[-1]
        dy2 = _c(dy).view(-1, Vp)
        dx, dw, db = _linear_bwd_raw(dy2, x2, (ctx.weight,), ctx.needs_input_grad[0], ctx.has_bias, pad_rows=Vp - V,
                                     bias_param=ctx.bias, site="vocab")
        return ((dx.view(ctx.in_shape) if dx is not None else None), (dw[:V] if dw is not None else None),
                (db[:V] if db is not None else None))


def _vocab_logits_padded(x, weight, bias):
    return _VocabLinear.apply(x, weight, bias)


def vocab_linear(x, weight, bias=None):
    return _vocab_logits_padded(x, weight, bias)[..., :weight.shape[0]]


def vocab_linear_cross_entropy(x, weight, bias, target, ignore_index: int = -100, rows: str = "all"):
    if rows not in ("all", "labelled"):
        raise ValueError(f"vocab_linear_cross_entropy: rows must be 'all' or 'labelled', got {rows!r}")
    V = weight.shape[0]
    if rows == "labelled":
        sel = select_rows(target.reshape(-1), V, ignore_index)
        m = padded_rows(sel.n)
        if m < sel.idx.numel():
            x = take_rows(x.reshape(-1, x.shape[-1]), sel.idx, sel.inv, m)
            target = sel.target_sel[:m]
    lp = _vocab_logits_padded(x, weight, bias)
    return _SoftmaxCE.apply(lp.reshape(-1, lp.shape[-1]), target.reshape(-1), V, ignore_index)


ROW_PAD_SMALL, ROW_PAD_STREAM, ROW_STREAM_MIN = 8, 256, 1024


def padded_rows(n: int) -> int:
    g = ROW_PAD_STREAM if n >= ROW_STREAM_MIN else ROW_PAD_SMALL
    return max((int(n) + g - 1) // g * g, g)


class SelectedRows(NamedTuple):
    idx: torch.Tensor
    inv: torch.Tensor
    target_sel: torch.Tensor
    count: torch.Tensor
    n: int


def select_rows(target, V: int, ignore_index: int = -100) -> SelectedRows:
    tgt = target.reshape(-1)
    if tgt.dtype != torch.int64:
        tgt = tgt.long()
    n_host = None
    if not tgt.is_cuda:
        n_host = int(((tgt != ignore_index) & (tgt >= 0) & (tgt < V)).sum())
        tgt = tgt.to(torch.device("cuda", torch.cuda.current_device()))
    _need_gpu(tgt)
    tgt = _c(tgt)
    T = tgt.numel()
    dev = tgt.device
    idx = torch.empty(T, device=dev, dtype=torch.int32)
    inv = torch.empty(T, device=dev, dtype=torch.int32)
    tsel = torch.empty(T, device=dev, dtype=torch.int64)
    count = torch.empty(1, device=dev, dtype=torch.int32)
    wsb = lib.meant_select_rows_ws(T)
    ws = torch.empty(max(wsb, 16), device=dev, dtype=torch.uint8)
    check(lib.meant_select_rows(_p(tgt), T, int(V), int(ignore_index), _p(idx), _p(inv), _p(tsel), _p(count), _p(ws), wsb, _stream()),
          "select_rows")
    if n_host is None:
        n_host = int(count.item())
    return SelectedRows(idx, inv, tsel, count, n_host)


class _TakeRows(torch.autograd.Function):

    @staticmethod
    def forward(ctx, x2d, idx, inv, m):
        ctx.save_for_backward(inv)
        return gather_rows(x2d, idx[:m])

    @staticmethod
    def backward(ctx, dy):
        (inv,) = ctx.saved_tensors
        return gather_rows(dy, inv), None, None, None


def take_rows(x2d, idx, inv, m: int):
    if x2d.dim() != 2 or x2d.shape[0] != idx.numel() or inv.numel() != idx.numel() or not 0 < m <= idx.numel():
        raise ValueError(f"take_rows: x2d {tuple(x2d.shape)}, idx [{idx.numel()}], inv [{inv.numel()}], m = {m}")
    if x2d.shape[1] % 8:
        raise ValueError(f"take_rows: row width {x2d.shape[1]} must be a multiple of 8")
    return _TakeRows.apply(x2d, idx, inv, int(m))


def softmax_cross_entropy(logits, target, ignore_index: int = -100):
    V = logits.shape[-1]
    l2 = logits.reshape(-1, V)
    Vp = (V + 7) // 8 * 8
    if Vp != V or not l2.is_contiguous():
        l2 = torch.nn.functional.pad(l2, (0, Vp - V))
    return _SoftmaxCE.apply(l2, target.reshape(-1), V, ignore_index)


class _AttentionCore(torch.autograd.Function):

    @staticmethod
    def forward(ctx, qkv, tables, G, S, H, scale, causal, key_mask):
        _need_gpu(qkv)
        dt = _dt(qkv)
        D3 = qkv.shape[-1]
        D = D3 // 3
        Dh = D // H
        qa, qb, ka, kb = tables if tables is not None else (None, None, None, None)
        R = qa.shape[1] if qa is not None else 0
        q2 = qkv.reshape(G * S, D3)
        if qa is not None:
            q2 = q2.clone() if q2.data_ptr() == qkv.data_ptr() else q2
            check(lib.meant_rotary_qk(_p(q2), G * S, S, H, Dh, R, _p(qa), _p(qb), _p(ka), _p(kb), 0, dt, _stream()), "rotary_qk")
        else:
            q2 = _c(q2)
        o = torch.empty((G * S, D), device=qkv.device, dtype=qkv.dtype)
        lse = torch.empty((G, H, S, 2), device=qkv.device, dtype=torch.float32)
        km = _c(key_mask.float()) if key_mask is not None else None
        wsb = lib.meant_attn_fwd_ws(G, S, H, Dh, dt)
        ws = torch.empty(max(wsb, 16), device=qkv.device, dtype=torch.uint8)
        check(lib.meant_attn_fwd(_p(q2), _p(o), _p(lse), _p(km), G, S, H, Dh, float(scale), int(causal), dt, _p(ws), wsb, _stream()), "attn_fwd")
        ctx.save_for_backward(q2, o, lse, km)
        ctx.tables, ctx.meta, ctx.in_shape = tables, (G, S, H, Dh, float(scale), int(causal)), qkv.shape
        return o

    @staticmethod
    def backward(ctx, do):
        q2, o, lse, km = ctx.saved_tensors
        G, S, H, Dh, scale, causal = ctx.meta
        do2 = _c(do)
        dt = _dt(do2)
        dqkv = torch.empty_like(q2)
        wsb = lib.meant_attn_ws(G, S, H, Dh, dt)
        ws = torch.empty(max(wsb, 16), device=do2.device, dtype=torch.uint8)
        qa, qb, ka, kb = ctx.tables if ctx.tables is not None else (None, None, None, None)
        R = qa.shape[1] if qa is not None else 0
        check(lib.meant_attn_bwd(_p(q2), _p(o), _p(do2), _p(lse), _p(km), _p(dqkv), G, S, H, Dh, scale, causal,
                                 _p(qa), _p(qb), _p(ka), _p(kb), R, dt, _p(ws), wsb, _stream()), "attn_bwd")
        return dqkv.view(ctx.in_shape), None, None, None, None, None, None, None


class _AttentionCoreScoreDropout(torch.autograd.Function):

    @staticmethod
    def forward(ctx, qkv, tables, G, S, H, scale, causal, key_mask, drop_p, seed):
        _need_gpu(qkv)
        dt = _dt(qkv)
        D3 = qkv.shape[-1]
        D = D3 // 3
        Dh = D // H
        qa, qb, ka, kb = tables if tables is not None else (None, None, None, None)
        R = qa.shape[1] if qa is not None else 0
        q2 = qkv.reshape(G * S, D3)
        if qa is not None:
            q2 = q2.clone() if q2.data_ptr() == qkv.data_ptr() else q2
            check(lib.meant_rotary_qk(_p(q2), G * S, S, H, Dh, R, _p(qa), _p(qb), _p(ka), _p(kb), 0, dt, _stream()), "rotary_qk")
        else:
            q2 = _c(q2)
        o = torch.empty((G * S, D), device=qkv.device, dtype=qkv.dtype)
        lse = torch.empty((G, H, S, 2), device=qkv.device, dtype=torch.float32)
        km = _c(key_mask.float()) if key_mask is not None else None
        wsb = lib.meant_attn_drop_ws(G, S, H, Dh, dt)
        ws = torch.empty(max(wsb, 16), device=qkv.device, dtype=torch.uint8)
        check(lib.meant_attn_drop_fwd(_p(q2), _p(o), _p(lse), _p(km), G, S, H, Dh, float(scale), int(causal), float(drop_p), int(seed), dt,
                                      _p(ws), wsb, _stream()), "attn_drop_fwd")
        ctx.save_for_backward(q2, o, lse, km)
        ctx.tables, ctx.meta, ctx.in_shape = tables, (G, S, H, Dh, float(scale), int(causal), float(drop_p), int(seed)), qkv.shape
        return o

    @staticmethod
    def backward(ctx, do):
        q2, o, lse, km = ctx.saved_tensors
        G, S, H, Dh, scale, causal, drop_p, seed = ctx.meta
        do2 = _c(do)
        dt = _dt(do2)
        dqkv = torch.empty_like(q2)
        wsb = lib.meant_attn_drop_ws(G, S, H, Dh, dt)
        ws = torch.empty(max(wsb, 16), device=do2.device, dtype=torch.uint8)
        check(lib.meant_attn_drop_bwd(_p(q2), _p(o), _p(do2), _p(lse), _p(km), _p(dqkv), G, S, H, Dh, scale, causal, drop_p, seed, dt,
                                      _p(ws), wsb, _stream()), "attn_drop_bwd")
        if ctx.tables is not None:
            qa, qb, ka, kb = ctx.tables
            check(lib.meant_rotary_qk(_p(dqkv), G * S, S, H, Dh, qa.shape[1], _p(qa), _p(qb), _p(ka), _p(kb), 1, dt, _stream()), "rotary_qk^T")
        return dqkv.view(ctx.in_shape), None, None, None, None, None, None, None, None, None


def attention_core_score_dropout(qkv, G, S, H, scale, drop_p, seed, tables=None, causal=False, key_mask=None):
    return _AttentionCoreScoreDropout.apply(qkv, tables, int(G), int(S), int(H), float(scale), bool(causal), key_mask, float(drop_p), int(seed))


def attention_core(qkv, G, S, H, scale, tables=None, causal=False, key_mask=None):
    return _AttentionCore.apply(qkv, tables, int(G), int(S), int(H), float(scale), bool(causal), key_mask)


class _GEGLU(torch.autograd.Function):

    @staticmethod
    def forward(ctx, h):
        _need_gpu(h)
        h2 = _c(h).view(-1, h.shape[-1])
        rows, w2 = h2.shape
        y = torch.empty((rows, w2 // 2), device=h.device, dtype=h.dtype)
        check(lib.meant_geglu_fwd(_p(h2), _p(y), rows, w2 // 2, _dt(h2), _stream()), "geglu_fwd")
        ctx.save_for_backward(h2)
        ctx.shape = h.shape
        return y.view(*h.shape[:-1], w2 // 2)

    @staticmethod
    def backward(ctx, dy):
        (h2,) = ctx.saved_tensors
        rows, w2 = h2.shape
        d2 = _c(dy).view(rows, w2 // 2)
        dh = torch.empty_like(h2)
        check(lib.meant_geglu_bwd(_p(h2), _p(d2), _p(dh), rows, w2 // 2, _dt(h2), _stream()), "geglu_bwd")
        return dh.view(ctx.shape)


def geglu(h):
    return _GEGLU.apply(h)


def gather_rows(src2d, idx, fill=None):
    _need_gpu(src2d, idx)
    src2d = _c(src2d)
    n, W = idx.numel(), src2d.shape[1]
    dst = torch.empty((n, W), device=src2d.device, dtype=src2d.dtype)
    check(lib.meant_gather_rows(_p(src2d), _p(idx), _p(fill), _p(dst), n, W, _dt(src2d), _stream()), "gather_rows")
    return dst


class _DividedAttention(torch.autograd.Function):

    @staticmethod
    def forward(ctx, qkv, plan, tables, H, scale, group_mask, cls_mask):
        _need_gpu(qkv)
# ... 122 lines not shown
```

Baseline: 3420 samples/s.

## Fuse token embedding gather with first encoder RMSNorm forward and backward

Adds HIP kernels that gather embedding rows and compute the first language encoder's RMSNorm in one pass, emitting both the residual stream and the normalized output. The backward folds the RMSNorm gradient into the sorted embedding scatter and also produces the gain gradient. The model routes through this path when the first encoder starts with a plain RMSNorm. The aim is to skip one full read/write of the token activations and a separate norm launch in each direction, at the cost of heavier, more register-hungry backward kernels and extra model-side routing for tuple inputs.

```diff
diff --git a/include/meant_hip.h b/include/meant_hip.h
--- a/include/meant_hip.h
+++ b/include/meant_hip.h
@@ -181,6 +181,14 @@
                             int64_t d, int64_t V, int64_t id_lo, int64_t id_hi, int dtype, void* workspace,
                             size_t workspace_bytes, void* stream);
 
+int meant_embedding_rmsnorm_fwd(const void* table, int table_dtype, const int64_t* ids, const float* gain, void* x, void* n_out,
+                                float* rinv, int64_t n, int64_t d, int64_t V, float eps, int dtype, void* stream);
+size_t meant_embedding_rmsnorm_bwd_sorted_ws(int64_t n, int64_t d);
+int meant_embedding_rmsnorm_bwd_sorted(const void* dn, const void* dres, const void* x, const float* rinv, const float* gain,
+                                       const int64_t* sorted_ids, const int64_t* order, float* dtable, float* dgain, int64_t n,
+                                       int64_t d, int64_t V, float eps, int64_t id_lo, int64_t id_hi, int accumulate_dgain, int dtype,
+                                       void* workspace, size_t workspace_bytes, void* stream);
+
 int meant_ce_probs(const float* probs, const int64_t* target, float* loss_accum, float* dprobs, int64_t B, int C,
                    void* stream);
 int meant_softmax_ce_fwd(const void* logits, int64_t ld, const int64_t* target, int64_t T, int64_t V, int64_t ignore_index,
diff --git a/meant_amd/_lib.py b/meant_amd/_lib.py
--- a/meant_amd/_lib.py
+++ b/meant_amd/_lib.py
@@ -83,6 +83,9 @@
     "meant_sort_ids": (_i, [_p, _i64, _i64, _p, _p, _p, _sz, _p]),
     "meant_embedding_bwd_seg_ws": (_sz, [_i64, _i64]),
     "meant_embedding_bwd_seg": (_i, [_p, _p, _p, _p, _i64, _i64, _i64, _i64, _i64, _i, _p, _sz, _p]),
+    "meant_embedding_rmsnorm_fwd": (_i, [_p, _i, _p, _p, _p, _p, _p, _i64, _i64, _i64, _f, _i, _p]),
+    "meant_embedding_rmsnorm_bwd_sorted_ws": (_sz, [_i64, _i64]),
+    "meant_embedding_rmsnorm_bwd_sorted": (_i, [_p, _p, _p, _p, _p, _p, _p, _p, _p, _i64, _i64, _i64, _f, _i64, _i64, _i, _i, _p, _sz, _p]),
     "meant_rmsnorm_partial_fwd": (_i, [_p, _p, _p, _p, _p, _i64, _i64, _i64, _f, _i, _p]),
     "meant_rmsnorm_partial_bwd": (_i, [_p, _p, _p, _p, _p, _p, _p, _i64, _i64, _i64, _f, _i, _p, _sz, _p]),
     "meant_rmsnorm_stats": (_i, [_p, _p, _i64, _i64, _f, _i, _p]),
diff --git a/meant_amd/csrc/common.h b/meant_amd/csrc/common.h
--- a/meant_amd/csrc/common.h
+++ b/meant_amd/csrc/common.h
@@ -55,6 +55,7 @@
   ROUTE_ATTN_BWD_D128, ROUTE_ATTN_BWD_D96, ROUTE_ATTN_GENERIC, ROUTE_ATTN_CLS, ROUTE_ATTN_SHORT, ROUTE_NT_OVERLAP, ROUTE_ATTN_BWD1,
   ROUTE_ATTN_FWD_D160, ROUTE_ATTN_FWD_D192, ROUTE_ATTN_FWD_D256, ROUTE_ATTN_BWD_D160, ROUTE_ATTN_BWD_D192, ROUTE_ATTN_BWD_D256, ROUTE_TEMPORAL_LONG,
   ROUTE_EMB_SEG, ROUTE_SORT_IDS, ROUTE_NT128K, ROUTE_NT256K, ROUTE_SELECT_ROWS, ROUTE_ROTARY_QK, ROUTE_ROTARY_PAIRS, ROUTE_NT_ROT,
+  ROUTE_EMB_NORM_FWD, ROUTE_EMB_NORM_BWD,
   MEANT_ROUTE_COUNT
 };
 void meant_route_hit(int route);
diff --git a/meant_amd/csrc/core.hip b/meant_amd/csrc/core.hip
--- a/meant_amd/csrc/core.hip
+++ b/meant_amd/csrc/core.hip
@@ -126,6 +126,7 @@
     "temporal_long", "emb_seg", "sort_ids", "nt128k", "nt256k", "select_rows",
     "rotary_qk", "rotary_pairs",
     "nt_rot",
+    "emb_norm_fwd", "emb_norm_bwd",
 };
 std::atomic<long long> g_route[MEANT_ROUTE_COUNT];
 }
diff --git a/meant_amd/csrc/embedding.hip b/meant_amd/csrc/embedding.hip
--- a/meant_amd/csrc/embedding.hip
+++ b/meant_amd/csrc/embedding.hip
@@ -1,4 +1,5 @@
-#include "common.h"
+#include <type_traits>
+#include "internal.h"
 
 #define EMB_REQ(c, ...) MEANT_REQUIRE(c, MEANT_ERR_ARG, __VA_ARGS__)
 
@@ -448,6 +449,255 @@
     }
   }
   flush(cur, !det && (shared || (j1 < n && sorted_ids[j1] == cur)));
+}
+
+template <typename TT, typename T>
+__device__ __forceinline__ Vec8<T> emb_chunk(const TT* p) {
+  const Vec8<TT> v = load8<TT>(p);
+  if constexpr (std::is_same<TT, T>::value) return v;
+  else {
+    Vec8<T> o;
+#pragma unroll
+    for (int k = 0; k < 8; ++k) o.set(k, v.get(k));
+    return o;
+  }
+}
+__device__ __forceinline__ int64_t emb_clamp(int64_t id, int64_t V) { return id < 0 ? 0 : (id >= V ? V - 1 : id); }
+
+template <typename TT, typename T, int C>
+__global__ __launch_bounds__(256) void emb_norm_fwd_packed_kernel(const TT* __restrict__ table, const int64_t* __restrict__ ids,
+                                                                   const float* __restrict__ scale, T* __restrict__ x, T* __restrict__ y,
+                                                                   float* __restrict__ rinv_out, int64_t rows, int d, int64_t V, int R,
+                                                                   float eps) {
+  const int lane = threadIdx.x & 63, wave = threadIdx.x >> 6;
+  const int nchunk = d >> 3;
+  const float inv_sqrt_d = rsqrtf((float)d);
+  int rsel[C], col[C];
+  f32x4 g0[C], g1[C];
+#pragma unroll
+  for (int c = 0; c < C; ++c) {
+    const int k = lane + 64 * c;
+    rsel[c] = k / nchunk;
+    col[c] = (k - rsel[c] * nchunk) * 8;
+    g0[c] = *reinterpret_cast<const f32x4*>(scale + col[c]);
+    g1[c] = *reinterpret_cast<const f32x4*>(scale + col[c] + 4);
+  }
+  const int64_t ngroups = rows / R;
+  for (int64_t grp = (int64_t)blockIdx.x * 4 + wave; grp < ngroups; grp += (int64_t)gridDim.x * 4) {
+    const int64_t row0 = grp * R;
+    Vec8<T> v[C];
+    float ss[C];
+#pragma unroll
+    for (int c = 0; c < C; ++c) v[c] = emb_chunk<TT, T>(table + emb_clamp(ids[row0 + rsel[c]], V) * d + col[c]);
+    T* xr = x + row0 * d;
+#pragma unroll
+    for (int c = 0; c < C; ++c) store8s<T>(xr + (lane + 64 * c) * 8, v[c]);
+#pragma unroll
+    for (int c = 0; c < C; ++c) {
+      ss[c] = 0.f;
+#pragma unroll
+      for (int i = 0; i < 8; ++i) { const float f = v[c].get(i); ss[c] += f * f; }
+    }
+    float rr[C];
+#pragma unroll
+    for (int c = 0; c < C; ++c) rr[c] = 0.f;
+    for (int r = 0; r < R; ++r) {
+      float s = 0.f;
+#pragma unroll
+      for (int c = 0; c < C; ++c) s += rsel[c] == r ? ss[c] : 0.f;
+      s = wave_sum_dpp(s);
+      const float rv = rms_rinv(s, inv_sqrt_d, eps);
+      if (lane == 0) rinv_out[row0 + r] = rv;
+#pragma unroll
+      for (int c = 0; c < C; ++c) rr[c] = rsel[c] == r ? rv : rr[c];
+    }
+    T* yr = y + row0 * d;
+#pragma unroll
+    for (int c = 0; c < C; ++c) {
+      Vec8<T> o;
+#pragma unroll
+      for (int i = 0; i < 8; ++i) o.set(i, (i < 4 ? g0[c][i] : g1[c][i - 4]) * (v[c].get(i) * rr[c]));
+      store8s<T>(yr + (lane + 64 * c) * 8, o);
+    }
+  }
+}
+
+template <typename TT, typename T>
+__global__ __launch_bounds__(256) void emb_norm_fwd_row_kernel(const TT* __restrict__ table, const int64_t* __restrict__ ids,
+                                                                const float* __restrict__ scale, T* __restrict__ x, T* __restrict__ y,
+                                                                float* __restrict__ rinv_out, int64_t rows, int d, int64_t V, float eps,
+                                                                int d_part, const float* __restrict__ offset) {
+  const int lane = threadIdx.x & 63, wave = threadIdx.x >> 6;
+  const int nchunk = d >> 3;
+  const float inv_sqrt_d = rsqrtf((float)d_part);
+  for (int64_t row = (int64_t)blockIdx.x * 4 + wave; row < rows; row += (int64_t)gridDim.x * 4) {
+    const TT* src = table + emb_clamp(ids[row], V) * d;
+    T* xr = x + row * d;
+    Vec8<T> v[2];
+    float ss = 0.f;
+#pragma unroll
+    for (int c = 0; c < 2; ++c) {
+      const int ch = lane + c * 64;
+      if (ch < nchunk) {
+        v[c] = emb_chunk<TT, T>(src + ch * 8);
+        store8s<T>(xr + ch * 8, v[c]);
+#pragma unroll
+        for (int i = 0; i < 8; ++i) { const float f = v[c].get(i); ss += ch * 8 + i < d_part ? f * f : 0.f; }
+      }
+    }
+    ss = wave_sum(ss);
+    const float r = 1.0f / (sqrtf(ss) * inv_sqrt_d + eps);
+    if (lane == 0) rinv_out[row] = r;
+    T* yr = y + row * d;
+#pragma unroll
+    for (int c = 0; c < 2; ++c) {
+      const int ch = lane + c * 64;
+      if (ch < nchunk) {
+        const f32x4 g0 = *reinterpret_cast<const f32x4*>(scale + ch * 8);
+        const f32x4 g1 = *reinterpret_cast<const f32x4*>(scale + ch * 8 + 4);
+        Vec8<T> o;
+#pragma unroll
+        for (int i = 0; i < 8; ++i) o.set(i, (i < 4 ? g0[i] : g1[i - 4]) * (v[c].get(i) * r) + (offset ? offset[ch * 8 + i] : 0.f));
+        store8<T>(yr + ch * 8, o);
+      }
+    }
+  }
+}
+
+constexpr int EMB_MAX_D = 1024;
+__device__ __forceinline__ long long readlane64(long long v, int l) {
+  const unsigned lo = (unsigned)__builtin_amdgcn_readlane((int)(unsigned long long)v, l);
+  const unsigned hi = (unsigned)__builtin_amdgcn_readlane((int)((unsigned long long)v >> 32), l);
+  return (long long)(((unsigned long long)hi << 32) | lo);
+}
+template <typename T>
+__global__ __launch_bounds__(256) void emb_norm_bwd_sorted_kernel(const T* __restrict__ dn, const T* __restrict__ dres, const T* __restrict__ x,
+                                                                   const float* __restrict__ rinv, const float* __restrict__ gain,
+                                                                   const int64_t* __restrict__ sorted_ids, const int64_t* __restrict__ order,
+                                                                   float* __restrict__ dtable, float* __restrict__ partial, int64_t n, int d,
+                                                                   int64_t V, float eps, int64_t id_lo, int64_t id_hi) {
+  __shared__ float red[4][EMB_MAX_D];
+  const int lane = threadIdx.x & 63, wave = __builtin_amdgcn_readfirstlane(threadIdx.x >> 6);
+  const int64_t j0 = ((int64_t)blockIdx.x * 4 + wave) * EMB_SEG;
+  const int64_t j1 = j0 + EMB_SEG < n ? j0 + EMB_SEG : n;
+  const bool active = j0 < n && !(sorted_ids[j1 - 1] < id_lo || sorted_ids[j0] >= id_hi);
+  const int nch = d >> 3;
+  const bool has1 = lane + 64 < nch, has0 = lane < nch;
+  float gq0[8], gq1[8];
+#pragma unroll
+  for (int e = 0; e < 8; ++e) gq0[e] = gq1[e] = 0.f;
+  if (active) {
+    float a0[8], a1[8], b0[8], b1[8];
+#pragma unroll
+    for (int e = 0; e < 8; ++e) a0[e] = a1[e] = b0[e] = b1[e] = 0.f;
+    int64_t cur = sorted_ids[j0];
+    long long cur_ord = order[j0];
+    bool shared = j0 > 0 && sorted_ids[j0 - 1] == cur;
+
+    auto flush = [&](int64_t id, long long ord, bool atomic) {
+      if (id < 0 || id >= V || id < id_lo || id >= id_hi) return;
+      if (ord < 0 || ord >= n) return;
+      const T* xr = x + ord * d;
+      const float r = rinv[ord];
+      Vec8<T> x0{}, x1{};
+      Vec8<float> ga0{}, ga1{};
+      if (has0) { x0 = load8<T>(xr + lane * 8); ga0 = load8<float>(gain + lane * 8); }
+      if (has1) { x1 = load8<T>(xr + (lane + 64) * 8); ga1 = load8<float>(gain + (lane + 64) * 8); }
+      float dot = 0.f;
+#pragma unroll
+      for (int e = 0; e < 8; ++e) {
+        const float xe0 = x0.get(e), xe1 = x1.get(e);
+        gq0[e] += a0[e] * xe0 * r;
+        gq1[e] += a1[e] * xe1 * r;
+        a0[e] = ga0.get(e) * a0[e];
+        a1[e] = ga1.get(e) * a1[e];
+        dot += a0[e] * xe0;
+        dot += a1[e] * xe1;
+      }
+      dot = wave_sum_dpp(dot);
+      const float nsd = (__builtin_amdgcn_rcpf(r) - eps) * (float)d;
+      const float kk = nsd > 0.f ? dot * r * r * __builtin_amdgcn_rcpf(nsd) : 0.f;
+#pragma unroll
+      for (int e = 0; e < 8; ++e) {
+        a0[e] = r * a0[e] - kk * x0.get(e) + b0[e];
+        a1[e] = r * a1[e] - kk * x1.get(e) + b1[e];
+      }
+      float* row = dtable + id * d;
+      if (atomic) {
+#pragma unroll
+        for (int e = 0; e < 8; ++e) {
+          if (has0) atomicAdd(row + lane * 8 + e, a0[e]);
+          if (has1) atomicAdd(row + (lane + 64) * 8 + e, a1[e]);
+        }
+      } else {
+        if (has0) {
+          Vec8<float> v = load8<float>(row + lane * 8);
+#pragma unroll
+          for (int e = 0; e < 8; ++e) v.set(e, v.get(e) + a0[e]);
+          store8<float>(row + lane * 8, v);
+        }
+        if (has1) {
+          Vec8<float> v = load8<float>(row + (lane + 64) * 8);
+#pragma unroll
+          for (int e = 0; e < 8; ++e) v.set(e, v.get(e) + a1[e]);
+          store8<float>(row + (lane + 64) * 8, v);
+        }
+      }
+    };
+
+    for (int64_t jb = j0; jb < j1; jb += 64) {
+      const int64_t jl = jb + lane < j1 ? jb + lane : j1 - 1;
+      const long long my_id = sorted_ids[jl], my_ord = order[jl];
+      const int cnt = (int)(j1 - jb < 64 ? j1 - jb : 64);
+      for (int t0 = 0; t0 < cnt; t0 += 4) {
+        Vec8<T> r0[4], r1[4], s0[4], s1[4];
+        long long ids4[4], ord4[4];
+#pragma unroll
+        for (int u = 0; u < 4; ++u) {
+          const int t = t0 + u < cnt ? t0 + u : cnt - 1;
+          ids4[u] = readlane64(my_id, t);
+          ord4[u] = readlane64(my_ord, t);
+          const bool row_ok = ord4[u] >= 0 && ord4[u] < n;
+          const int64_t off = (row_ok ? ord4[u] : 0) * d;
+          r0[u] = Vec8<T>{}; r1[u] = Vec8<T>{}; s0[u] = Vec8<T>{}; s1[u] = Vec8<T>{};
+          if (has0 && row_ok) r0[u] = load8s<T>(dn + off + lane * 8);
+          if (has1 && row_ok) r1[u] = load8s<T>(dn + off + (lane + 64) * 8);
+          if (dres) {
+            if (has0 && row_ok) s0[u] = load8s<T>(dres + off + lane * 8);
+            if (has1 && row_ok) s1[u] = load8s<T>(dres + off + (lane + 64) * 8);
+          }
+        }
+#pragma unroll
+        for (int u = 0; u < 4; ++u) {
+          if (t0 + u >= cnt) break;
+          const int64_t id = ids4[u];
+          if (id != cur) {
+            flush(cur, cur_ord, shared);
+#pragma unroll
+            for (int e = 0; e < 8; ++e) a0[e] = a1[e] = b0[e] = b1[e] = 0.f;
+            cur = id;
+            cur_ord = ord4[u];
+            shared = false;
+          }
+#pragma unroll
+          for (int e = 0; e < 8; ++e) {
+            a0[e] += r0[u].get(e);
+            a1[e] += r1[u].get(e);
+            b0[e] += s0[u].get(e);
+            b1[e] += s1[u].get(e);
+          }
+        }
+      }
+    }
+    flush(cur, cur_ord, shared || (j1 < n && sorted_ids[j1] == cur));
+  }
+#pragma unroll
+  for (int e = 0; e < 8; ++e) {
+    if (has0) red[wave][lane * 8 + e] = gq0[e];
+    if (has1) red[wave][(lane + 64) * 8 + e] = gq1[e];
+  }
+  __syncthreads();
+  for (int j = threadIdx.x; j < d; j += 256) partial[(int64_t)blockIdx.x * d + j] = (red[0][j] + red[1][j]) + (red[2][j] + red[3][j]);
 }
 
 }
@@ -590,3 +840,75 @@
   MEANT_LAUNCH_CHECK("embedding_bwd");
   return MEANT_OK;
 }
+
+extern "C" int meant_embedding_rmsnorm_fwd(const void* table, int table_dtype, const int64_t* ids, const float* gain, void* x, void* n_out,
+                                           float* rinv, int64_t n, int64_t d, int64_t V, float eps, int dtype, void* stream) {
+  EMB_REQ(table && ids && gain && x && n_out && rinv && n > 0 && d > 0 && V > 0, "embedding_rmsnorm_fwd: bad argument");
+  MEANT_REQUIRE(d <= EMB_MAX_D && d % 8 == 0, MEANT_ERR_UNSUPPORTED, "embedding_rmsnorm_fwd: d=%lld must be a multiple of 8 and <= 1024", (long long)d);
+  MEANT_REQUIRE((table_dtype == MEANT_F32 || table_dtype == MEANT_BF16) && (dtype == MEANT_F32 || dtype == MEANT_BF16) &&
+                    !(table_dtype == MEANT_BF16 && dtype == MEANT_F32),
+                MEANT_ERR_UNSUPPORTED, "embedding_rmsnorm_fwd: table dtype %d with output dtype %d (a bf16 image serves the bf16 tier only)", table_dtype, dtype);
+  EMB_REQ(meant_aligned16(table) && meant_aligned16(gain) && meant_aligned16(x) && meant_aligned16(n_out), "embedding_rmsnorm_fwd: 16-byte alignment");
+  hipStream_t st = (hipStream_t)stream;
+  const NormPacking pk = rmsnorm_packing(n, d);
+#define EMB_NORM_FWD(TT, T)                                                                                                              \
+  do {                                                                                                                                   \
+    if (pk.R == 0) {                                                                                                                     \
+      int64_t nb = ceil_div(n, 4); if (nb > 1024) nb = 1024;                                                                             \
+      hipLaunchKernelGGL((emb_norm_fwd_row_kernel<TT, T>), dim3((unsigned)nb), dim3(256), 0, st, (const TT*)table, ids, gain, (T*)x,    \
+                         (T*)n_out, rinv, n, (int)d, V, eps, (int)d, (const float*)nullptr);                                             \
+    } else {                                                                                                                             \
+      int64_t nb = ceil_div(n / pk.R, 4); if (nb > 2048) nb = 2048;                                                                      \
+      if (pk.C == 1) hipLaunchKernelGGL((emb_norm_fwd_packed_kernel<TT, T, 1>), dim3((unsigned)nb), dim3(256), 0, st, (const TT*)table, \
+                                        ids, gain, (T*)x, (T*)n_out, rinv, n, (int)d, V, pk.R, eps);                                     \
+      else if (pk.C == 2) hipLaunchKernelGGL((emb_norm_fwd_packed_kernel<TT, T, 2>), dim3((unsigned)nb), dim3(256), 0, st,              \
+                                             (const TT*)table, ids, gain, (T*)x, (T*)n_out, rinv, n, (int)d, V, pk.R, eps);              \
+      else hipLaunchKernelGGL((emb_norm_fwd_packed_kernel<TT, T, 3>), dim3((unsigned)nb), dim3(256), 0, st, (const TT*)table, ids,      \
+                              gain, (T*)x, (T*)n_out, rinv, n, (int)d, V, pk.R, eps);                                                    \
+    }                                                                                                                                    \
+  } while (0)
+  if (table_dtype == MEANT_BF16) EMB_NORM_FWD(bf16, bf16);
+  else if (dtype == MEANT_BF16) EMB_NORM_FWD(float, bf16);
+  else EMB_NORM_FWD(float, float);
+#undef EMB_NORM_FWD
+  MEANT_LAUNCH_CHECK("embedding_rmsnorm_fwd");
+  meant_route_hit(ROUTE_EMB_NORM_FWD);
+  return MEANT_OK;
+}
+
+extern "C" size_t meant_embedding_rmsnorm_bwd_sorted_ws(int64_t n, int64_t d) {
+  if (n <= 0 || d <= 0) return 0;
+  return (size_t)ceil_div(n, 4 * EMB_SEG) * (size_t)d * sizeof(float);
+}
+
+extern "C" int meant_embedding_rmsnorm_bwd_sorted(const void* dn, const void* dres, const void* x, const float* rinv, const float* gain,
+                                                  const int64_t* sorted_ids, const int64_t* order, float* dtable, float* dgain, int64_t n,
+                                                  int64_t d, int64_t V, float eps, int64_t id_lo, int64_t id_hi, int accumulate_dgain,
+                                                  int dtype, void* workspace, size_t workspace_bytes, void* stream) {
+  EMB_REQ(dn && x && rinv && gain && sorted_ids && order && dtable && dgain && n > 0 && d > 0 && V > 0 && 0 <= id_lo && id_lo <= id_hi &&
+              id_hi <= V,
+          "embedding_rmsnorm_bwd_sorted: bad argument");
+  MEANT_REQUIRE(d <= EMB_MAX_D && d % 8 == 0, MEANT_ERR_UNSUPPORTED, "embedding_rmsnorm_bwd_sorted: d=%lld must be a multiple of 8 and <= 1024", (long long)d);
+  MEANT_REQUIRE(!meant_opt(MEANT_OPT_DETERMINISTIC), MEANT_ERR_UNSUPPORTED,
+                "embedding_rmsnorm_bwd_sorted: float atomics for the runs that cross a stretch; option deterministic takes the separate kernels");
+  const size_t need = meant_embedding_rmsnorm_bwd_sorted_ws(n, d);
+  MEANT_REQUIRE(workspace && workspace_bytes >= need, MEANT_ERR_WORKSPACE, "embedding_rmsnorm_bwd_sorted: workspace of %zu bytes needed, %zu given", need, workspace_bytes);
+  EMB_REQ(meant_aligned16(dn) && (!dres || meant_aligned16(dres)) && meant_aligned16(x) && meant_aligned16(gain) && meant_aligned16(dtable) &&
+              meant_aligned16(workspace),
+          "embedding_rmsnorm_bwd_sorted: 16-byte alignment");
+  hipStream_t st = (hipStream_t)stream;
+  if (id_lo == id_hi) {
+    if (!accumulate_dgain) {
+      const hipError_t e = hipMemsetAsync(dgain, 0, (size_t)d * sizeof(float), st);
+      MEANT_REQUIRE(e == hipSuccess, MEANT_ERR_LAUNCH, "embedding_rmsnorm_bwd_sorted: clearing dgain failed: %s", hipGetErrorString(e));
+    }
+    return MEANT_OK;
+  }
+  const int64_t nb = ceil_div(n, 4 * EMB_SEG);
+  DISPATCH_DTYPE(dtype, T,
+                 hipLaunchKernelGGL(emb_norm_bwd_sorted_kernel<T>, dim3((unsigned)nb), dim3(256), 0, st, (const T*)dn, (const T*)dres,
+                                    (const T*)x, rinv, gain, sorted_ids, order, dtable, (float*)workspace, n, (int)d, V, eps, id_lo, id_hi));
+  MEANT_LAUNCH_CHECK("embedding_rmsnorm_bwd_sorted");
+  meant_route_hit(ROUTE_EMB_NORM_BWD);
+  return colsum_launch(workspace, d, dgain, nb, d, MEANT_F32, accumulate_dgain, st);
+}
diff --git a/meant_amd/csrc/internal.h b/meant_amd/csrc/internal.h
--- a/meant_amd/csrc/internal.h
+++ b/meant_amd/csrc/internal.h
@@ -43,6 +43,9 @@
 
 int colsum_launch(const void* x, int64_t ldx, float* out, int64_t M, int64_t N, int dtype, int accumulate, hipStream_t stream);
 
+struct NormPacking { int R, C; };
+NormPacking rmsnorm_packing(int64_t rows, int64_t d);
+
 int attn_f32_fwd(const float* qkv, float* o, float* lse, const float* key_mask, int64_t G, int64_t S, int H, int Dh,
                  float scale, int causal, void* ws, size_t ws_bytes, hipStream_t stream, float drop_p = 0.f, uint64_t seed = 0);
 int attn_f32_bwd(const float* qkv, const float* o, const float* dout, const float* lse, const float* key_mask, float* dqkv,
diff --git a/meant_amd/csrc/norm.hip b/meant_amd/csrc/norm.hip
--- a/meant_amd/csrc/norm.hip
+++ b/meant_amd/csrc/norm.hip
@@ -1198,6 +1198,11 @@
   return rc ? rc : norm_colsums(part1, nb, d, dscale, doffset, 0, stream);
 }
 
+}
+
+NormPacking rmsnorm_packing(int64_t rows, int64_t d) {
+  const NormRoute nr = norm_route(rows, d);
+  return nr.kind == NORM_PACKED ? NormPacking{nr.R, nr.C} : NormPacking{0, 0};
 }
 
 extern "C" size_t meant_rmsnorm_bwd_ws(int64_t rows, int64_t d) {
diff --git a/meant_amd/modules.py b/meant_amd/modules.py
--- a/meant_amd/modules.py
+++ b/meant_amd/modules.py
@@ -334,7 +334,10 @@
         e, e2 = self.encode, self.encode2
         p1 = e[4].p if self.training else 0.0
         p2 = e2[4].p if self.training else 0.0
-        n, res = ops.rmsnorm_fork(input, e[0].scale, e[0].eps)
+        if isinstance(input, tuple):
+            n, res = input
+        else:
+            n, res = ops.rmsnorm_fork(input, e[0].scale, e[0].eps)
         if COMPOSE_PRE_LINEAR and e[1].bias is not None:
             h = e[2].multi_mad(e[2].core(n, attention_mask, pre=e[1]))
         else:
@@ -415,7 +418,8 @@
 
 def _run_stack(encoders, x, *args, checkpoint=False):
     n = len(encoders)
-    fold = ops.stack_fold(n, x.numel() // x.shape[-1], x.shape[-1])
+    x0 = _tokens(x)
+    fold = ops.stack_fold(n, x0.numel() // x0.shape[-1], x0.shape[-1])
     for i, enc in enumerate(encoders):
         ck = checkpoint if isinstance(checkpoint, bool) else i < checkpoint
         last = enc.encode2[-1]
@@ -452,10 +456,36 @@
     return ops.pooled_linear_cat([st], compute_dtype)
 
 
-def _embed(mods, ids, dtype):
+def _plain_embedding(mod, x) -> bool:
+    return isinstance(mod, nn.Embedding) and mod.max_norm is None and not mod.sparse and x.dtype in (torch.int64, torch.int32)
+
+
+def _tokens(x):
+    return x[1] if isinstance(x, tuple) else x
+
+
+def _emb_norm_fused(mods, ids, encoders, checkpoint) -> bool:
+    if encoders is None or len(encoders) == 0 or len(mods) != 1 or checkpoint:
+        return False
+    mod, enc = mods[0], encoders[0]
+    if not _plain_embedding(mod, ids) or not isinstance(enc, languageEncoder):
+        return False
+    norm = enc.encode[0]
+    d = mod.weight.shape[1]
+    if type(norm) is not RMSNorm or norm.bias or 0. <= norm.p <= 1. or norm.d != d:
+        return False
+    if torch.is_grad_enabled() and norm.scale.requires_grad and not mod.weight.requires_grad:
+        return False
+    return ops.emb_norm_fuse_ok(ids.numel(), d)
+
+
+def _embed(mods, ids, dtype, encoders=None, checkpoint=False):
+    if ids.is_cuda and _emb_norm_fused(mods, ids, encoders, checkpoint):
+        norm = encoders[0].encode[0]
+        return ops.embedding_rmsnorm_fork(ids, mods[0].weight, norm.scale, norm.eps, dtype)
     x = ids
     for mod in mods:
-        if isinstance(mod, nn.Embedding) and mod.max_norm is None and not mod.sparse and x.dtype in (torch.int64, torch.int32):
+        if _plain_embedding(mod, x):
             x = ops.embedding(x, mod.weight, dtype)
         else:
             x = mod(x)
@@ -500,10 +530,10 @@
         B = images.shape[0]
         if images.is_cuda and TWO_STREAMS:
             ops.set_index_stream(images.device, _side_stream(images.device))
-        words = _embed(self.embedding, tweets.reshape(B * self.lag, tweets.shape[2]), dt)
+        ck = _ckpt_setting(self)
+        words = _embed(self.embedding, tweets.reshape(B * self.lag, tweets.shape[2]), dt, self.languageEncoders, ck)
         if attention_mask is not None:
             attention_mask = attention_mask.reshape(B * self.lag, attention_mask.shape[2])
-        ck = _ckpt_setting(self)
         side = _side_stream(images.device) if (TWO_STREAMS and images.is_cuda and not ck) else None
         if side is not None:
             main = torch.cuda.current_stream()
@@ -585,7 +615,7 @@
     def forward(self, tweets, attention_mask=None):
         dt = resolve_compute_dtype(self, None)
         B = tweets.shape[0]
-        words = _embed(self.embedding, tweets.reshape(B * self.lag, tweets.shape[2]), dt)
+        words = _embed(self.embedding, tweets.reshape(B * self.lag, tweets.shape[2]), dt, self.languageEncoders)
         attention_mask = attention_mask.reshape(B * self.lag, attention_mask.shape[2])
         words = _run_stack(self.languageEncoders, words, attention_mask)
         fused = _pool_parts(dt, words).view(B, self.lag, self.dim)
@@ -616,7 +646,7 @@
 
     def forward(self, tweets, images, attention_mask=None):
         dt = resolve_compute_dtype(self, images)
-        words = _embed(self.embedding, tweets, dt)
+        words = _embed(self.embedding, tweets, dt, self.languageEncoders)
         words = _run_stack(self.languageEncoders, words, attention_mask)
         img = self.patchEmbed(images, dt)
         img = _run_stack(self.visionEncoders, img)
@@ -648,8 +678,9 @@
 
     def _encode(self, words, attention_mask):
         dt = resolve_compute_dtype(self, None)
-        x = _embed(self.embedding, words, dt)
-        fold = ops.stack_fold(len(self.languageEncoders), x.numel() // x.shape[-1], x.shape[-1])
+        x = _embed(self.embedding, words, dt, self.languageEncoders)
+        x0 = _tokens(x)
+        fold = ops.stack_fold(len(self.languageEncoders), x0.numel() // x0.shape[-1], x0.shape[-1])
         for enc in self.languageEncoders:
             x = enc(x, attention_mask=attention_mask, fold=fold)
         return x
diff --git a/meant_amd/ops.py b/meant_amd/ops.py
--- a/meant_amd/ops.py
+++ b/meant_amd/ops.py
@@ -1278,6 +1278,91 @@
     return _Embedding.apply(ids, table, dtype)
 
 
+def emb_norm_fuse_ok(n: int, d: int) -> bool:
+    return (os.environ.get("MEANT_EMB_NORM_FUSE", "1") != "0" and not _lib_option("deterministic")
+            and _emb_bwd_route(n, d) == "sorted")
+
+
+class _EmbeddingRMSNormFork(torch.autograd.Function):
+
+    @staticmethod
+    def forward(ctx, ids, table, gain, eps, dtype):
+        _need_gpu(ids, table, gain)
+        ids_c = _c(ids.long())
+        V, d = table.shape
+        n = ids_c.numel()
+        x = torch.empty((*ids.shape, d), device=table.device, dtype=dtype)
+        y = torch.empty_like(x)
+        rinv = torch.empty(n, device=table.device, dtype=torch.float32)
+        sc = _c(gain.detach().float())
+        if dtype == torch.bfloat16 and EMB_BF16_TABLE and V < (1 << 31):
+            tb, tdt = weights.get((table,), torch.bfloat16, False), BF16
+        else:
+            tb, tdt = _c(table.detach().float()), F32
+        check(lib.meant_embedding_rmsnorm_fwd(_p(tb), tdt, _p(ids_c), _p(sc), _p(x), _p(y), _p(rinv), n, d, V, eps,
+                                              F32 if dtype == torch.float32 else BF16, _stream()), "embedding_rmsnorm_fwd")
+        presort = None
+        if EMB_PRESORT and ctx.needs_input_grad[1]:
+            main = torch.cuda.current_stream(ids_c.device)
+            side = _aux_stream(ids_c.device)
+            side.wait_stream(main)
+            with torch.cuda.stream(side):
+                sorted_ids, order = _sort_ids(ids_c.view(-1), V)
+                ev = torch.cuda.Event()
+                ev.record(side)
+            presort = (sorted_ids, order, ev)
+        ctx.save_for_backward(ids_c, x, sc, rinv)
+        ctx.presort = presort
+        ctx.meta = (V, d, eps)
+        ctx.table = table
+        _claim(table, "embedding")
+        return y, x
+
+    @staticmethod
+    def backward(ctx, dn, dres):
+        ids_c, x, sc, rinv = ctx.saved_tensors
+        V, d, eps = ctx.meta
+        if dn is None and dres is None:
+            return None, None, None, None, None
+        if dn is None:
+            dn = torch.zeros_like(x)
+        dn = _c(dn)
+        dres = _c(dres) if dres is not None else None
+        sink = _sink_of(ctx.table, "embedding") if grad_sinks else None
+        if sink is not None and (sink.view.shape != (V, d) or not sink.view.is_contiguous()):
+            sink = None
+        dtab = sink.view if sink is not None else torch.zeros((V, d), device=dn.device, dtype=torch.float32)
+        n = ids_c.numel()
+        if ctx.presort is not None:
+            sorted_ids, order, ev = ctx.presort
+            cur = torch.cuda.current_stream(dn.device)
+            cur.wait_event(ev)
+            sorted_ids.record_stream(cur)
+            order.record_stream(cur)
+        else:
+            sorted_ids, order = _sort_ids(ids_c.view(-1), V)
+        dgain = torch.empty(d, device=dn.device, dtype=torch.float32)
+        wsb = lib.meant_embedding_rmsnorm_bwd_sorted_ws(n, d)
+        ws = torch.empty(wsb, device=dn.device, dtype=torch.uint8)
+        nsl = sink.row_slices(ctx.table) if sink is not None else 1
+        for c in range(nsl):
+            lo, hi = V * c // nsl, V * (c + 1) // nsl
+            check(lib.meant_embedding_rmsnorm_bwd_sorted(_p(dn), _p(dres), _p(x), _p(rinv), _p(sc), _p(sorted_ids), _p(order), _p(dtab),
+                                                         _p(dgain), n, d, V, eps, lo, hi, int(c > 0), _dt(dn), _p(ws), wsb, _stream()),
+                  "embedding_rmsnorm_bwd_sorted")
+            if nsl > 1:
+                sink.report_rows(ctx.table, lo, hi, c == nsl - 1)
+        if sink is not None:
+            if nsl == 1:
+                sink.report(ctx.table)
+            return None, None, dgain, None, None
+        return None, dtab, dgain, None, None
+
+
+def embedding_rmsnorm_fork(ids, table, gain, eps, dtype):
+    return _EmbeddingRMSNormFork.apply(ids, table, gain, float(eps), dtype)
+
+
 def cast(x: torch.Tensor, dtype: torch.dtype) -> torch.Tensor:
     _need_gpu(x)
     if x.dtype == dtype:
```

Result: faster. 3497 samples/s, median of 5 (+2.2%).
